# rizar/attention-lvcsr

Measured on AMD Instinct MI355X. Metric: encoder+attention+decoder training frames/sec (whole node), higher is better.
Workload: dtype f32; 1 GPU; wsj_base: B=16 utterances x T=800 frames x F=40 fbank per GPU, L=100 labels; 256x256x256x256 BiGRU subsample [1, 1, 2, 2], content_and_conv attention, 256-unit GRU decoder; global_batch=16, per_gpu_batch=16, ragged=False, parallelism=dp1, optimizer=clip100+adadelta+maxnorm1, hip_graph=True, priming_steps=2, encoder_kernels=persistent clusters, full=False

## Files before the change

attention-lvcsr_amd/csrc/encoder_persist.hip:

```cpp
#include "common.h"
#include "graph_cache.h"
#include "lvsr_hip.h"
#include "persist.h"

typedef lvsr_bigru_fwd_args EncFwd;
typedef lvsr_bigru_bwd_args EncBwd0;

template <int NG, bool PRIV, int NTH = 256>
struct Sweep {
    static constexpr int NT = PRIV ? 64 : NTH;
    static constexpr int N = (NG + NT - 1) / NT;
    u64 w[N];
    __device__ __forceinline__ void issue(const u64* g, unsigned epoch) {
        const int tid = PRIV ? (int)(threadIdx.x & 63) : (int)threadIdx.x;
#pragma unroll
        for (int i = 0; i < N; ++i) {
            const int idx = tid + NT * i;
            if (NG % NT == 0 || idx < NG) w[i] = __hip_atomic_load(g + idx, __ATOMIC_RELAXED, __HIP_MEMORY_SCOPE_AGENT);
            else w[i] = (u64)epoch << 32;
        }
    }
    __device__ __forceinline__ bool complete(unsigned epoch) const {
        bool ok = true;
#pragma unroll
// ... 353 lines not shown
        const size_t jo = (size_t)b0 * 2 * H + dir * H + min(jj, H - 1);
        const long long row = (long long)B * 2 * H, sgn = dir == 0 ? -1 : 1;
        const float* p0 = (hi ? a.c : a.u) + jo;
        const float* p1 = (hi ? a.y : a.r) + jo;
        const float h0v = a.h0[dir][min(jj, H - 1)];
        const float* p2 = hi ? a.dy + (size_t)b0 * 2 * H + dir * H + min(jj, H - 1) : (a.mask ? a.mask + b0 : a.h0[dir]);
        const long long row2 = hi ? row : (a.mask ? (long long)B : 0);
        auto issue = [&](int ns, float (&dst)[3]) {
            const int nsc = min(ns, T - 1), t = dir == 0 ? T - 1 - nsc : nsc, tp = t + (int)sgn, tpc = min(max(tp, 0), T - 1);
            const bool edge = tp != tpc, dy_here = !edge && (tp % a.sub) == 0;
            const float v0 = p0[(long long)t * row];
            const float v1 = p1[(long long)(hi ? tpc : t) * row];
            const float v2 = p2[(long long)(hi ? tpc / a.sub : t) * row2];
            dst[0] = live ? v0 : 0.f;
            dst[1] = live ? ((hi && edge) ? h0v : v1) : 0.f;
            dst[2] = hi ? ((live && dy_here) ? v2 : 0.f) : ((live && a.mask) ? v2 : 1.f);
        };
        float pa[3], pb[3];
        auto hand = [&](int n, const float (&v)[3]) {
            if (n + 1 < T) { opnd9[lane] = v[0]; opnd9[64 + lane] = v[1]; opnd9[128 + lane] = v[2]; }
            __syncthreads();
            __syncthreads();
        };
        issue(1, pa);
        for (int n = 0; n < T; n += 2) {
            issue(n + 2, pb);
            hand(n, pa);
            if (n + 1 < T) {
                issue(n + 3, pa);
                hand(n + 1, pb);
            }
        }
        return;
    }
    const int tid = threadIdx.x, q = tid % KSPLIT, j = p * UNITS + tid / KSPLIT, k0 = q * KS;
    const bool junit = j < H;
    f32x2 wa[KS / 2], wbu[KS / 2], wbr[KS / 2];
    {
        const float* Whg = a.WhgT_p[dir];
        const float* Whh = a.WhhT_p[dir];
        const size_t jc = (size_t)min(j, H - 1);
#pragma unroll
        for (int x = 0; x < KS / 2; ++x) {
            float v[6];
#pragma unroll
            for (int e = 0; e < 2; ++e) {
                const int k = k0 + 2 * x + e;
                const float keep = (junit && k < H) ? 1.f : 0.f;
                const size_t kc = (size_t)min(k, H - 1);
                v[e] = Whh[jc * H + kc] * keep;
                v[2 + e] = Whg[jc * 2 * H + kc] * keep;
                v[4 + e] = Whg[jc * 2 * H + H + kc] * keep;
            }
            wa[x] = (f32x2){v[0], v[1]}; wbu[x] = (f32x2){v[2], v[3]}; wbr[x] = (f32x2){v[4], v[5]};
        }
    }
    u64* gc = planes + (size_t)cl * 4 * NG;
    u64* gu = gc + NG;
    u64* gr = gc + 2 * NG;
    const int t_first = dir == 0 ? T - 1 : 0;
    float dh[NR], n_u[NR], n_c[NR], n_r[NR], n_hp[NR], n_m[NR], n_dy[NR];
    bool rvalid[NR];
    auto prefetch = [&](int t, int i) {
        const int b = b0 + q + i * KSPLIT;
        const int tp = dir == 0 ? t - 1 : t + 1;
        const size_t o = ((size_t)t * B + b) * 2 * H + dir * H + j;
        n_u[i] = a.u[o]; n_c[i] = a.c[o]; n_r[i] = a.r[o];
        n_hp[i] = (tp < 0 || tp >= T) ? a.h0[dir][j] : a.y[((size_t)tp * B + b) * 2 * H + dir * H + j];
        n_m[i] = a.mask ? a.mask[(size_t)t * B + b] : 1.f;
        n_dy[i] = pb_dy_at(a, tp, b, dir, j);
    };
#pragma unroll
    for (int i = 0; i < NR; ++i) {
        const int r = q + i * KSPLIT;
        rvalid[i] = junit && r < RB && b0 + r < B;
        dh[i] = rvalid[i] ? pb_dy_at(a, t_first, b0 + r, dir, j) : 0.f;
        n_u[i] = n_c[i] = n_r[i] = n_hp[i] = n_dy[i] = 0.f; n_m[i] = 1.f;
        if (rvalid[i]) prefetch(t_first, i);
    }
    for (int n = 0; n < T; ++n) {
        const int t = dir == 0 ? T - 1 - n : n;
        float uu[NR], cc[NR], rr[NR], hp[NR], part[NR];
#pragma unroll
        for (int i = 0; i < NR; ++i) {
            const int r = q + i * KSPLIT;
            uu[i] = n_u[i]; cc[i] = n_c[i]; rr[i] = n_r[i]; hp[i] = n_hp[i];
            if (r < RB) {
                const float dhn = n_m[i] * dh[i];
                const float dpc = rvalid[i] ? dhn * uu[i] * (1.f - cc[i] * cc[i]) : 0.f;
                const float dpu = rvalid[i] ? dhn * (cc[i] - hp[i]) * uu[i] * (1.f - uu[i]) : 0.f;
                if (P == 1) {
                    lds_publish<KS, LDH, KSPLIT>(vbuf[0], r, j, dpc);
                    lds_publish<KS, LDH, KSPLIT>(vbuf[1], r, j, dpu);
                } else {
                    granule_store(gc + (size_t)r * HP + j, (unsigned)(n + 1), dpc, plain);
                    granule_store(gu + (size_t)r * HP + j, (unsigned)(n + 1), dpu, plain);
                }
                part[i] = dhn * (1.f - uu[i]) + (1.f - n_m[i]) * dh[i] + n_dy[i];
                if (rvalid[i] && save) {
                    float* dx = a.dxg + ((size_t)t * B + b0 + r) * 6 * H + dir * 3 * H;
                    dx[j] = dpc; dx[H + j] = dpu;
                }
            }
        }
        if (!LD9 && n + 1 < T && !(flags & PF_NOPREFETCH)) {
#pragma unroll
            for (int i = 0; i < NR; ++i)
                if (rvalid[i]) prefetch(dir == 0 ? t - 1 : t + 1, i);
        }
        if (P > 1 && !gather_plane<NG, HP, KS, LDH, KSPLIT, PRIV, 2, NBUF * RB * KSPLIT * LDH, NTH>(gc, (unsigned)(n + 1), vbuf[0], abort_word)) return;
        gather_fence<PRIV>();
        if (LD9 && n + 1 < T && rvalid[0]) {
            const int ju = tid / KSPLIT;
            n_u[0] = opnd9[ju]; n_c[0] = opnd9[32 + ju]; n_r[0] = opnd9[64 + ju]; n_hp[0] = opnd9[96 + ju];
            n_m[0] = opnd9[128 + ju]; n_dy[0] = opnd9[160 + ju];
        }
        float s[RB], vu[RB];
        slice_dot<KS, RB, LDH, KSPLIT>(wa, vbuf[0], q, s);
#pragma unroll
        for (int i = 0; i < NR; ++i) {
            const int r = q + i * KSPLIT;
            if (r < RB) {
                const float drh = pick_row<RB, KSPLIT>(s, q, i);
                const float dpr = rvalid[i] ? drh * hp[i] * rr[i] * (1.f - rr[i]) : 0.f;
                if (P == 1) lds_publish<KS, LDH, KSPLIT>(vbuf[2], r, j, dpr);
                else granule_store(gr + (size_t)r * HP + j, (unsigned)(n + 1), dpr, plain);
                part[i] += drh * rr[i];
                if (rvalid[i] && save) a.dxg[((size_t)t * B + b0 + r) * 6 * H + dir * 3 * H + 2 * H + j] = dpr;
            }
        }
        slice_dot<KS, RB, LDH, KSPLIT>(wbu, vbuf[1], q, vu);
        if (P > 1 && !gather_plane<NG, HP, KS, LDH, KSPLIT, PRIV, 1, 0, NTH>(gr, (unsigned)(n + 1), vbuf[2], abort_word)) return;
        gather_fence<PRIV>();
        slice_dot<KS, RB, LDH, KSPLIT>(wbr, vbuf[2], q, s);
#pragma unroll
        for (int i = 0; i < NR; ++i) {
            const int r = q + i * KSPLIT;
            if (r < RB) dh[i] = rvalid[i] ? part[i] + pick_row<RB, KSPLIT>(vu, q, i) + pick_row<RB, KSPLIT>(s, q, i) : 0.f;
        }
    }
#pragma unroll
    for (int i = 0; i < NR; ++i)
        if (rvalid[i]) dh_out[((size_t)dir * Bp + b0 + q + i * KSPLIT) * H + j] = dh[i];
}

__global__ __launch_bounds__(256) void enc_pbwd_h0_kernel(const float* dh, int Bp, int B, int H, float* out_f, float* out_b) {
    const int dir = blockIdx.z;
    const int j = blockIdx.x * 256 + threadIdx.x;
    if (j >= H) return;
    float s = 0.f;
    for (int b = 0; b < B; ++b) s += dh[((size_t)dir * Bp + b) * H + j];
    (dir == 0 ? out_f : out_b)[j] = s;
}

template <int KS, int U>
__device__ __forceinline__ void ub_dot(const f32x2 (&w)[U][KS / 2], const float* buf, int q, float (&out)[U]) {
    const float4* hv = (const float4*)(buf + q * (KS + 4));
    f32x2 acc[U];
#pragma unroll
    for (int u = 0; u < U; ++u) acc[u] = (f32x2){0.f, 0.f};
#pragma unroll
    for (int x = 0; x < KS / 4; ++x) {
        const float4 h4 = hv[x];
        const f32x2 lo = {h4.x, h4.y}, hi = {h4.z, h4.w};
#pragma unroll
        for (int u = 0; u < U; ++u) {
            acc[u] = w[u][2 * x] * lo + acc[u];
            acc[u] = w[u][2 * x + 1] * hi + acc[u];
        }
    }
#pragma unroll
    for (int u = 0; u < U; ++u) out[u] = acc[u].x + acc[u].y;
}
template <int U>
__device__ __forceinline__ float ub_fold(const float (&v)[U], int q) {
    float r;
    if (U == 4) {
        const bool up = (q & 32) != 0;
        const float a0 = (up ? v[2] : v[0]) + __shfl_xor(up ? v[0] : v[2], 32, 64);
        const float a1 = (up ? v[3] : v[1]) + __shfl_xor(up ? v[1] : v[3], 32, 64);
        const bool up2 = (q & 16) != 0;
        r = (up2 ? a1 : a0) + __shfl_xor(up2 ? a0 : a1, 16, 64);
    } else if (U == 2) {
        const bool up = (q & 16) != 0;
        r = (up ? v[1] : v[0]) + __shfl_xor(up ? v[0] : v[1], 16, 64);
    } else {
        r = v[0];
    }
    return group_sum<16>(r);
}

template <int KS, int U, int NTH>
__global__ __launch_bounds__(NTH) void enc_pfwd_ub_kernel(EncFwd a, u64* planes, u64* hello, int* abort_word, int flags) {
    constexpr int G = 16 * U, HP = KS * G, UNITS = NTH / G * U, P = HP / UNITS, LDH = KS + 4, NG = HP;
    __shared__ __attribute__((aligned(16))) float hbuf[2][G * LDH];
    const int H = a.H, B = a.B, T = a.T;
    int cl, p;
    if (!cluster_of_block(P, 2 * B, flags, cl, p)) return;
    const bool save = !(flags & PF_NOSAVE);
    const bool plain = cluster_shares_xcd(hello + (size_t)cl * P, P, p, abort_word) && !(flags & PF_SC1);
    const int dir = cl / B, b = cl % B;
    const int tid = threadIdx.x, q = tid % G, jb = p * UNITS + (tid / G) * U, k0 = q * KS;
    f32x2 wr[U][KS / 2], wu[U][KS / 2], wc[U][KS / 2];
    {
        const float* Whg = a.Whg_p[dir];
        const float* Whh = a.Whh_p[dir];
#pragma unroll
        for (int u = 0; u < U; ++u) {
            const int j = jb + u;
            const size_t jc = (size_t)min(j, H - 1);
#pragma unroll
            for (int x = 0; x < KS / 2; ++x) {
                float v[6];
#pragma unroll
                for (int e = 0; e < 2; ++e) {
                    const int k = k0 + 2 * x + e;
                    const float keep = (j < H && k < H) ? 1.f : 0.f;
                    const size_t kc = (size_t)min(k, H - 1);
                    v[e] = Whg[kc * 2 * H + jc] * keep;
                    v[2 + e] = Whg[kc * 2 * H + H + jc] * keep;
                    v[4 + e] = Whh[kc * H + jc] * keep;
                }
                wu[u][x] = (f32x2){v[0], v[1]}; wr[u][x] = (f32x2){v[2], v[3]}; wc[u][x] = (f32x2){v[4], v[5]};
            }
        }
    }
    u64* gh = planes + (size_t)cl * 2 * NG;
    u64* grh = gh + NG;
    const int j = jb + (q >> 4);
    const bool own = (q & 15) == 0 && j < H;
    float hown = own ? a.h0[dir][j] : 0.f, n_xin = 0.f, n_gu = 0.f, n_gr = 0.f, n_m = 1.f;
    auto fetch = [&](int t) {
        const size_t row = (size_t)t * B + b;
        const float* xr = a.xg + row * 6 * H + dir * 3 * H;
        n_xin = xr[j]; n_gu = xr[H + j]; n_gr = xr[2 * H + j];
        if (a.mask) n_m = a.mask[row];
    };
    if (own) fetch(dir == 0 ? 0 : T - 1);
    for (int k = tid; k < HP; k += NTH) hbuf[0][(k / KS) * LDH + (k % KS)] = k < H ? a.h0[dir][k] : 0.f;
    for (int n = 0; n < T; ++n) {
        const int t = dir == 0 ? n : T - 1 - n;
        const float xin = n_xin, gu = n_gu, gr = n_gr, m = n_m;
        if (n > 0 && !gather_plane<NG, HP, KS, LDH, G, false, 1, 0, NTH>(gh, (unsigned)n, hbuf[0], abort_word, flags)) return;
        __syncthreads();
        float s[U];
        ub_dot<KS, U>(wr, hbuf[0], q, s);
        const float rr = sigmoid_fast(ub_fold<U>(s, q) + gr);
        const float rh = own ? rr * hown : 0.f;
        if ((q & 15) == 0) granule_store(grh + min(j, HP - 1), (unsigned)(n + 1), rh, plain);
        if (own && save) {
            const size_t o = ((size_t)t * B + b) * 2 * H + dir * H + j;
            a.r[o] = rr; a.rh[o] = rh;
        }
        ub_dot<KS, U>(wu, hbuf[0], q, s);
        const float uu = sigmoid_fast(ub_fold<U>(s, q) + gu);
        if (own && save) a.u[((size_t)t * B + b) * 2 * H + dir * H + j] = uu;
        if (!gather_plane<NG, HP, KS, LDH, G, false, 1, 0, NTH>(grh, (unsigned)(n + 1), hbuf[1], abort_word, flags)) return;
        __syncthreads();
        ub_dot<KS, U>(wc, hbuf[1], q, s);
        const float cand = tanh_fast(ub_fold<U>(s, q) + xin);
        float hn = cand * uu + hown * (1.f - uu);
        hn = m * hn + (1.f - m) * hown;
        if (!own) hn = 0.f;
        if ((q & 15) == 0 && n + 1 < T) granule_store(gh + min(j, HP - 1), (unsigned)(n + 1), hn, plain);
        if (own) {
            const size_t o = ((size_t)t * B + b) * 2 * H + dir * H + j;
            if (save) a.c[o] = cand;
            a.y[o] = hn;
            if (a.ysub && (t % a.sub) == 0) a.ysub[((size_t)(t / a.sub) * B + b) * 2 * H + dir * H + j] = hn;
        }
        hown = hn;
        if (own && n + 1 < T && !(flags & PF_NOPREFETCH)) fetch(dir == 0 ? n + 1 : T - 2 - n);
    }
}

static int wide_cluster_capacity() {
    static int occ_cached = -1;
    if (occ_cached < 0) {
        int occ = 1 << 20, n = 0;
        const bool ok = hipOccupancyMaxActiveBlocksPerMultiprocessor(&n, enc_pfwd_kernel<16, 16, 1, false, 512>, 512, 0) == hipSuccess && (occ = min(occ, n)) >= 0 &&
                        hipOccupancyMaxActiveBlocksPerMultiprocessor(&n, enc_pfwd_kernel<16, 16, 2, false, 512>, 512, 0) == hipSuccess && (occ = min(occ, n)) >= 0 &&
                        hipOccupancyMaxActiveBlocksPerMultiprocessor(&n, enc_pbwd_kernel<16, 16, 1, false, 512>, 512, 0) == hipSuccess && (occ = min(occ, n)) >= 0 &&
                        hipOccupancyMaxActiveBlocksPerMultiprocessor(&n, enc_pbwd_kernel<16, 16, 2, false, 512>, 512, 0) == hipSuccess && (occ = min(occ, n)) >= 0;
        if (!ok) { (void)hipGetLastError(); occ = 0; }
        occ_cached = min(occ, 2);
    }
    return occ_cached * lvsr_max_cluster_wgs();
}

static int persist_flags() { return lvsr_knob(LVSR_KNOB_PERSIST_FLAGS); }

extern "C" int lvsr_bigru_persist_rows(int B, int H) {
    PersistGeom g;
    if (B <= 0 || H <= 0 || !persist_geom(B, H, g)) return 0;
    return g.RB;
}

extern "C" long long lvsr_bigru_persist_ws_bytes(int B, int H) {
    PersistGeom g;
    if (B <= 0 || H <= 0) return 0;
    if (!persist_geom(B, H, g)) return 0;
    const long long hello = (long long)cluster_grid(2 * B, 16, 0) * 8;
    return 256 + (long long)2 * (B + 16) * 4 * g.HP * 8 + (hello > 8 * 1024 ? hello : 8 * 1024);
}

template <int KS, int KSPLIT>
static void launch_fwd(hipStream_t s, const EncFwd& a, const PersistGeom& g, u64* planes, u64* hello, int* ab, int flags) {
    if (g.NTH == 512 && g.RB == 1 && g.HP == 512 && !(flags & PF_NOUB)) {
        hipLaunchKernelGGL((enc_pfwd_ub_kernel<8, 4, 512>), dim3(g.grid), dim3(512), 0, s, a, planes, hello, ab, flags);
        return;
    }
    if (g.NTH == 512) {
        if (g.P == 8 && g.KS == 16 && g.RB == 1 && !(flags & (PF_NOLD9F | PF_NOSTAGE)) && g.grid <= lvsr_max_cluster_wgs())
            hipLaunchKernelGGL((enc_pfwd_kernel<16, 16, 1, false, 512, true>), dim3(g.grid), dim3(576), 0, s, a, planes, hello, ab, flags);
        else if (g.P == 8 && g.KS == 16 && g.RB == 1) hipLaunchKernelGGL((enc_pfwd_kernel<16, 16, 1, false, 512>), dim3(g.grid), dim3(512), 0, s, a, planes, hello, ab, flags);
        else if (g.P == 8 && g.KS == 16) hipLaunchKernelGGL((enc_pfwd_kernel<16, 16, 2, false, 512>), dim3(g.grid), dim3(512), 0, s, a, planes, hello, ab, flags);
        else if (g.RB == 1) hipLaunchKernelGGL((enc_pfwd_kernel<KS / 2, KSPLIT * 2, 1, false, 512>), dim3(g.grid), dim3(512), 0, s, a, planes, hello, ab, flags);
        else hipLaunchKernelGGL((enc_pfwd_kernel<KS / 2, KSPLIT * 2, 2, false, 512>), dim3(g.grid), dim3(512), 0, s, a, planes, hello, ab, flags);
        return;
    }
    switch (g.RB) {
        case 1:
            if (!(flags & PF_PRIVATE)) hipLaunchKernelGGL((enc_pfwd_kernel<KS, KSPLIT, 1, false>), dim3(g.grid), dim3(256), 0, s, a, planes, hello, ab, flags);
            else hipLaunchKernelGGL((enc_pfwd_kernel<KS, KSPLIT, 1, true>), dim3(g.grid), dim3(256), 0, s, a, planes, hello, ab, flags);
            break;
        case 2: hipLaunchKernelGGL((enc_pfwd_kernel<KS, KSPLIT, 2, false>), dim3(g.grid), dim3(256), 0, s, a, planes, hello, ab, flags); break;
        case 4: hipLaunchKernelGGL((enc_pfwd_kernel<KS, KSPLIT, 4, false>), dim3(g.grid), dim3(256), 0, s, a, planes, hello, ab, flags); break;
        default: hipLaunchKernelGGL((enc_pfwd_kernel<KS, KSPLIT, 8, false>), dim3(g.grid), dim3(256), 0, s, a, planes, hello, ab, flags); break;
    }
}
template <int KS, int KSPLIT>
static void launch_bwd(hipStream_t s, const EncBwd0& a, const PersistGeom& g, u64* planes, u64* hello, int* ab, float* dh, int Bp, int flags) {
    if (g.NTH == 512) {
        if (g.P == 8 && g.KS == 16 && g.RB == 1 && !(flags & PF_NOLD9) && g.grid <= lvsr_max_cluster_wgs())
            hipLaunchKernelGGL((enc_pbwd_kernel<16, 16, 1, false, 512, true>), dim3(g.grid), dim3(576), 0, s, a, planes, hello, ab, dh, Bp, flags);
        else if (g.P == 8 && g.KS == 16 && g.RB == 1) hipLaunchKernelGGL((enc_pbwd_kernel<16, 16, 1, false, 512>), dim3(g.grid), dim3(512), 0, s, a, planes, hello, ab, dh, Bp, flags);
        else if (g.P == 8 && g.KS == 16) hipLaunchKernelGGL((enc_pbwd_kernel<16, 16, 2, false, 512>), dim3(g.grid), dim3(512), 0, s, a, planes, hello, ab, dh, Bp, flags);
        else if (g.RB == 1) {
            if constexpr (KSPLIT == 8) {
                if (!(flags & PF_NOLD9) && g.grid <= lvsr_max_cluster_wgs()) {
                    hipLaunchKernelGGL((enc_pbwd_kernel<KS / 2, KSPLIT * 2, 1, false, 512, true>), dim3(g.grid), dim3(576), 0, s, a, planes, hello, ab, dh, Bp, flags);
                    return;
                }
            }
            hipLaunchKernelGGL((enc_pbwd_kernel<KS / 2, KSPLIT * 2, 1, false, 512>), dim3(g.grid), dim3(512), 0, s, a, planes, hello, ab, dh, Bp, flags);
        }
        else hipLaunchKernelGGL((enc_pbwd_kernel<KS / 2, KSPLIT * 2, 2, false, 512>), dim3(g.grid), dim3(512), 0, s, a, planes, hello, ab, dh, Bp, flags);
        return;
    }
    switch (g.RB) {
        case 1:
            if (!(flags & PF_PRIVATE)) hipLaunchKernelGGL((enc_pbwd_kernel<KS, KSPLIT, 1, false>), dim3(g.grid), dim3(256), 0, s, a, planes, hello, ab, dh, Bp, flags);
            else hipLaunchKernelGGL((enc_pbwd_kernel<KS, KSPLIT, 1, true>), dim3(g.grid), dim3(256), 0, s, a, planes, hello, ab, dh, Bp, flags);
            break;
        case 2: hipLaunchKernelGGL((enc_pbwd_kernel<KS, KSPLIT, 2, false>), dim3(g.grid), dim3(256), 0, s, a, planes, hello, ab, dh, Bp, flags); break;
        case 4: hipLaunchKernelGGL((enc_pbwd_kernel<KS, KSPLIT, 4, false>), dim3(g.grid), dim3(256), 0, s, a, planes, hello, ab, dh, Bp, flags); break;
        default: hipLaunchKernelGGL((enc_pbwd_kernel<KS, KSPLIT, 8, false>), dim3(g.grid), dim3(256), 0, s, a, planes, hello, ab, dh, Bp, flags); break;
    }
}

int lvsr_bigru_fwd_persistent(hipStream_t s, const EncFwd& a0, int use_graph) {
    EncFwd a = a0;
    PersistGeom g;
    LVSR_REQUIRE(persist_geom(a.B, a.H, g) && a.sync_ws, "lvsr_bigru_fwd: persistent mode not available for B=%d H=%d", a.B, a.H);
    int* ab = (int*)a.sync_ws;
    u64* planes = (u64*)((char*)a.sync_ws + 256);
    u64* hello = planes + (size_t)2 * g.rt * 2 * g.plane;
    const size_t bytes = (size_t)2 * g.rt * 2 * g.plane * 8 + (size_t)g.grid * 8;
    if (a.sub == 1) a.ysub = nullptr;
    const int flags = persist_flags();
    auto enqueue = [&]() {
        (void)hipMemsetAsync(planes, 0, bytes, s);
        switch (g.KSPLIT / (g.NTH / 256)) {
            case 2: launch_fwd<64, 2>(s, a, g, planes, hello, ab, flags); break;
            case 4: launch_fwd<64, 4>(s, a, g, planes, hello, ab, flags); break;
            default: launch_fwd<64, 8>(s, a, g, planes, hello, ab, flags); break;
        }
    };
    GraphKey key("bigru_pfwd");
    key.add(&a, sizeof(a));
    key.add(&g.RB, sizeof(g.RB));
    key.add(&g.NTH, sizeof(g.NTH));
    key.add(&flags, sizeof(flags));
    return lvsr_run_graph(s, use_graph, key, enqueue, "lvsr_bigru_fwd(persistent)");
}

int lvsr_bigru_bwd_persistent(hipStream_t s, const EncBwd0& a, int use_graph) {
    PersistGeom g;
    LVSR_REQUIRE(persist_geom(a.B, a.H, g) && a.sync_ws, "lvsr_bigru_bwd: persistent mode not available for B=%d H=%d", a.B, a.H);
    int* ab = (int*)a.sync_ws;
    u64* planes = (u64*)((char*)a.sync_ws + 256);
    u64* hello = planes + (size_t)2 * g.rt * 4 * g.plane;
    const size_t bytes = (size_t)2 * g.rt * 4 * g.plane * 8 + (size_t)g.grid * 8;
    const int Bp = ((a.B + 15) / 16) * 16;
    float* dh = a.dh_ws;
    const int flags = persist_flags();
    auto enqueue = [&]() {
        (void)hipMemsetAsync(planes, 0, bytes, s);
        switch (g.KSPLIT / (g.NTH / 256)) {
            case 2: launch_bwd<64, 2>(s, a, g, planes, hello, ab, dh, Bp, flags); break;
            case 4: launch_bwd<64, 4>(s, a, g, planes, hello, ab, dh, Bp, flags); break;
            default: launch_bwd<64, 8>(s, a, g, planes, hello, ab, dh, Bp, flags); break;
        }
        hipLaunchKernelGGL(enc_pbwd_h0_kernel, dim3((a.H + 255) / 256, 1, 2), dim3(256), 0, s, dh, Bp, a.B, a.H, a.dh0[0], a.dh0[1]);
    };
    GraphKey key("bigru_pbwd");
    key.add(&a, sizeof(a));
    key.add(&g.RB, sizeof(g.RB));
    key.add(&g.NTH, sizeof(g.NTH));
    key.add(&flags, sizeof(flags));
    return lvsr_run_graph(s, use_graph, key, enqueue, "lvsr_bigru_bwd(persistent)");
}
```

attention-lvcsr_amd/csrc/gemm.hip:

```cpp
#include "common.h"
#include "lvsr_hip.h"
#include "graph_cache.h"
#include <algorithm>
#include <vector>

#define BM 64
#define BN 64
#define BK 16
#define LDS_LD (BM + 4)

struct GemmArgs {
    const float* A; const float* B; float* C; const float* bias;
    int M, N, K, lda, ldb, ldc, transA, transB;
    float alpha, beta;
    int ksplit;
    int kchunk;
    float* part;
    int batch;
    long long sA, sB, sC;
};

__global__ __launch_bounds__(256) void lvsr_sgemm_kernel(GemmArgs g) {
    __shared__ float As[BK][LDS_LD];
    __shared__ float Bs[BK][LDS_LD];
// ... 424 lines not shown
        if ((int)blockIdx.x >= pk.d[x].fold0) p = x;
    const GroupDesc& d = pk.d[p];
    const size_t total = (size_t)d.M * d.N;
    const float* part = pk.part + d.part_off;
    const size_t base = (size_t)((int)blockIdx.x - d.fold0) * FOLD_ELEMS;
    const bool vec = (d.N & 3) == 0 && (d.ldc & 3) == 0 && (((size_t)d.C) & 15) == 0 && (((size_t)part) & 15) == 0;
    size_t idx[4];
    float s[4] = {0.f, 0.f, 0.f, 0.f};
#pragma unroll
    for (int e = 0; e < 4; ++e) idx[e] = vec ? base + 4 * threadIdx.x + e : base + threadIdx.x + 256 * e;
    int z = 0;
    if (vec) {
        if (idx[0] >= total) return;
        const float* q = part + idx[0];
        for (; z + 4 <= d.ksplit; z += 4) {
            float4 v[4];
#pragma unroll
            for (int c = 0; c < 4; ++c) v[c] = *(const float4*)(q + (size_t)(z + c) * total);
#pragma unroll
            for (int c = 0; c < 4; ++c) { s[0] += v[c].x; s[1] += v[c].y; s[2] += v[c].z; s[3] += v[c].w; }
        }
        for (; z < d.ksplit; ++z) {
            const float4 v = *(const float4*)(q + (size_t)z * total);
            s[0] += v.x; s[1] += v.y; s[2] += v.z; s[3] += v.w;
        }
        float* c = d.C + (idx[0] / d.N) * d.ldc + idx[0] % d.N;
        if (d.beta != 0.f) {
            const float4 o = *(const float4*)c;
            s[0] += d.beta * o.x; s[1] += d.beta * o.y; s[2] += d.beta * o.z; s[3] += d.beta * o.w;
        }
        *(float4*)c = make_float4(s[0], s[1], s[2], s[3]);
        return;
    }
    for (; z + 4 <= d.ksplit; z += 4) {
        float v[4][4];
#pragma unroll
        for (int c = 0; c < 4; ++c)
#pragma unroll
            for (int e = 0; e < 4; ++e) v[c][e] = idx[e] < total ? part[(size_t)(z + c) * total + idx[e]] : 0.f;
#pragma unroll
        for (int c = 0; c < 4; ++c)
#pragma unroll
            for (int e = 0; e < 4; ++e) s[e] += v[c][e];
    }
    for (; z < d.ksplit; ++z)
#pragma unroll
        for (int e = 0; e < 4; ++e) s[e] += idx[e] < total ? part[(size_t)z * total + idx[e]] : 0.f;
#pragma unroll
    for (int e = 0; e < 4; ++e) {
        if (idx[e] >= total) continue;
        float* c = d.C + (idx[e] / d.N) * d.ldc + idx[e] % d.N;
        float r = s[e];
        if (d.beta != 0.f) r += d.beta * *c;
        *c = r;
    }
}

__global__ __launch_bounds__(256) void lvsr_sgemm_splitk_reduce(GemmArgs g) {
    const size_t total = (size_t)g.M * g.N;
    for (size_t idx = (size_t)blockIdx.x * blockDim.x + threadIdx.x; idx < total; idx += (size_t)gridDim.x * blockDim.x) {
        const int m = (int)(idx / g.N), n = (int)(idx % g.N);
        float s = 0.f;
        for (int z = 0; z < g.ksplit; ++z) s += g.part[(size_t)z * total + idx];
        float v = g.alpha * s;
        if (g.beta != 0.f) v += g.beta * g.C[(size_t)m * g.ldc + n];
        if (g.bias) v += g.bias[n];
        g.C[(size_t)m * g.ldc + n] = v;
    }
}

__global__ __launch_bounds__(256) void lvsr_colsum_kernel(const float* X, int M, int N, int ldx, float* out, float beta,
                                                          int rows_per, float* part) {
    __shared__ float red[4][64];
    const int n = blockIdx.x * 64 + (threadIdx.x & 63);
    const int g = threadIdx.x >> 6;
    const int m0 = blockIdx.y * rows_per, m1 = min(M, m0 + rows_per);
    float s0 = 0.f, s1 = 0.f, s2 = 0.f, s3 = 0.f;
    if (n < N) {
        int m = m0 + g;
        for (; m + 12 < m1; m += 16) {
            s0 += X[(size_t)m * ldx + n];
            s1 += X[(size_t)(m + 4) * ldx + n];
            s2 += X[(size_t)(m + 8) * ldx + n];
            s3 += X[(size_t)(m + 12) * ldx + n];
        }
        for (; m < m1; m += 4) s0 += X[(size_t)m * ldx + n];
    }
    red[g][threadIdx.x & 63] = (s0 + s1) + (s2 + s3);
    __syncthreads();
    if (g == 0 && n < N) {
        const int c = threadIdx.x & 63;
        const float v = ((red[0][c] + red[1][c]) + red[2][c]) + red[3][c];
        if (part) part[(size_t)blockIdx.y * N + n] = v;
        else out[n] = (beta != 0.f ? beta * out[n] : 0.f) + v;
    }
}

#define COLSUM_MANY_MAX 32
struct ColsumMember { const float* X; float* out; float* part; int M, N, ldx, S, rows_per, nx, block0, fin0; float beta; };
struct ColsumPack { ColsumMember m[COLSUM_MANY_MAX]; int n; };
__global__ __launch_bounds__(256) void lvsr_colsum_many_kernel(ColsumPack pk) {
    __shared__ float red[4][64];
    int p = 0;
    for (int i = 1; i < pk.n; ++i)
        if ((int)blockIdx.x >= pk.m[i].block0) p = i;
    const ColsumMember& c = pk.m[p];
    const int local = blockIdx.x - c.block0, bx = local % c.nx, by = local / c.nx;
    const int n = bx * 64 + (threadIdx.x & 63);
    const int g = threadIdx.x >> 6;
    const int m0 = by * c.rows_per, m1 = min(c.M, m0 + c.rows_per);
    const float* X = c.X;
    const int ldx = c.ldx;
    float s0 = 0.f, s1 = 0.f, s2 = 0.f, s3 = 0.f;
    if (n < c.N) {
        int m = m0 + g;
        for (; m + 12 < m1; m += 16) {
            s0 += X[(size_t)m * ldx + n];
            s1 += X[(size_t)(m + 4) * ldx + n];
            s2 += X[(size_t)(m + 8) * ldx + n];
            s3 += X[(size_t)(m + 12) * ldx + n];
        }
        for (; m < m1; m += 4) s0 += X[(size_t)m * ldx + n];
    }
    red[g][threadIdx.x & 63] = (s0 + s1) + (s2 + s3);
    __syncthreads();
    if (g == 0 && n < c.N) {
        const int col = threadIdx.x & 63;
        const float v = ((red[0][col] + red[1][col]) + red[2][col]) + red[3][col];
        if (c.S > 1) c.part[(size_t)by * c.N + n] = v;
        else c.out[n] = (c.beta != 0.f ? c.beta * c.out[n] : 0.f) + v;
    }
}
__global__ __launch_bounds__(256) void lvsr_colsum_many_finish(ColsumPack pk) {
    int p = 0;
    for (int i = 1; i < pk.n; ++i)
        if ((int)blockIdx.x >= pk.m[i].fin0) p = i;
    const ColsumMember& c = pk.m[p];
    if (c.S <= 1) return;
    const int n = ((int)blockIdx.x - c.fin0) * 256 + threadIdx.x;
    if (n >= c.N) return;
    float v = 0.f;
    for (int s = 0; s < c.S; ++s) v += c.part[(size_t)s * c.N + n];
    c.out[n] = (c.beta != 0.f ? c.beta * c.out[n] : 0.f) + v;
}

__global__ __launch_bounds__(256) void lvsr_colsum_finish(const float* part, int S, int N, float* out, float beta) {
    const int n = blockIdx.x * 256 + threadIdx.x;
    if (n >= N) return;
    float v = 0.f;
    for (int s = 0; s < S; ++s) v += part[(size_t)s * N + n];
    out[n] = (beta != 0.f ? beta * out[n] : 0.f) + v;
}

#define COPY_MANY_MAX 32
struct CopyPack { lvsr_copy_desc d[COPY_MANY_MAX]; int n; };
__global__ __launch_bounds__(256) void lvsr_copy2d_many_kernel(CopyPack pk) {
    const lvsr_copy_desc& d = pk.d[blockIdx.y];
    const bool vec = ((d.cols | d.lds | d.ldd) & 3) == 0 && ((((size_t)d.src) | ((size_t)d.dst)) & 15) == 0;
    if (d.rows == 1) {
        for (int c = blockIdx.x * 256 + threadIdx.x; c < d.cols; c += gridDim.x * 256)
            d.dst[c] = d.beta != 0.f ? d.src[c] + d.beta * d.dst[c] : d.src[c];
        return;
    }
    for (int r = blockIdx.x; r < d.rows; r += gridDim.x) {
        const float* s = d.src + (size_t)r * d.lds;
        float* o = d.dst + (size_t)r * d.ldd;
        if (d.beta != 0.f) {
            for (int c = threadIdx.x; c < d.cols; c += 256) o[c] = s[c] + d.beta * o[c];
        } else if (vec) {
            for (int c = threadIdx.x * 4; c < d.cols; c += 1024) *(float4*)(o + c) = *(const float4*)(s + c);
        } else {
            for (int c = threadIdx.x; c < d.cols; c += 256) o[c] = s[c];
        }
    }
}

__global__ __launch_bounds__(256) void lvsr_transpose_kernel(const float* in, int rows, int cols, float* out) {
    __shared__ float tile[32][33];
    const int tx = threadIdx.x & 31, ty = threadIdx.x >> 5;
    const int r0 = blockIdx.y * 32, c0 = blockIdx.x * 32;
    for (int j = ty; j < 32; j += 8) {
        const int r = r0 + j, c = c0 + tx;
        tile[j][tx] = (r < rows && c < cols) ? in[(size_t)r * cols + c] : 0.f;
    }
    __syncthreads();
    for (int j = ty; j < 32; j += 8) {
        const int c = c0 + j, r = r0 + tx;
        if (r < rows && c < cols) out[(size_t)c * rows + r] = tile[tx][j];
    }
}

__global__ __launch_bounds__(256) void lvsr_pack_b_kernel(const float* W, int ldw, int K, int N, int trans, float* P,
                                                          int Kw, int NQ, long long total) {
    for (long long idx = (long long)blockIdx.x * 256 + threadIdx.x; idx < total; idx += (long long)gridDim.x * 256) {
        const int r = (int)(idx & 3), lane = (int)((idx >> 2) & 63);
        const long long g = idx >> 8;
        const int q = (int)(g % NQ), wave = (int)((g / NQ) & 3), tile = (int)(g / NQ / 4);
        const int k = wave * Kw + (lane >> 4) * (Kw >> 2) + 4 * q + r, col = tile * 16 + (lane & 15);
        float v = 0.f;
        if (k < K && col < N) v = trans ? W[(size_t)col * ldw + k] : W[(size_t)k * ldw + col];
        P[idx] = v;
    }
}

static bool operands_aligned(const float* A, int lda, const float* B, int ldb) {
    return (lda & 3) == 0 && (ldb & 3) == 0 && (((size_t)A) & 15) == 0 && (((size_t)B) & 15) == 0;
}

static int colsum_split(int M, int N, bool have_ws, long long ws_bytes) {
    if (!have_ws || M < 512) return 1;
    const int nx = (N + 63) / 64;
    int S = (M + 255) / 256;
    const int want = (1024 + nx - 1) / nx;
    if (S > want) S = want;
    while (S > 1 && (long long)S * N * 4 > ws_bytes) --S;
    return S;
}

extern "C" {

static int sgemm_launch(void* stream, int transA, int transB, int M, int N, int K, float alpha, const float* A, int lda,
                        const float* B, int ldb, float beta, float* C, int ldc, const float* bias, float* ws,
                        long long ws_bytes, int batch, long long sA, long long sB, long long sC) {
    LVSR_REQUIRE(M >= 0 && N >= 0 && K >= 0 && batch >= 1, "lvsr_sgemm: negative dimension");
    if (M == 0 || N == 0) return LVSR_OK;
    GemmArgs g;
    g.batch = batch; g.sA = sA; g.sB = sB; g.sC = sC;
    if (batch > 1) ws = nullptr;
    g.A = A; g.B = B; g.C = C; g.bias = bias;
    g.M = M; g.N = N; g.K = K; g.lda = lda; g.ldb = ldb; g.ldc = ldc; g.transA = transA; g.transB = transB;
    g.alpha = alpha; g.beta = beta; g.ksplit = 1; g.kchunk = 0; g.part = nullptr;
    const bool big = (M >= 96 && N >= 96) || (min(M, N) >= 32 && max(M, N) >= 256 && K >= 2048);
    int tm = big ? GM : BM, tn = big ? GN : BN;
    const int tk = big ? GK : BK;
    int tiles = ((M + tm - 1) / tm) * ((N + tn - 1) / tn);
    const int mid_max = lvsr_knob(LVSR_KNOB_GEMM_MID_TILES) > 0 ? lvsr_knob(LVSR_KNOB_GEMM_MID_TILES) : 2048;
    const bool mid = big && batch == 1 && (tiles < 256 || (tiles < mid_max && K <= 2048));
    if (mid) { tm = 64; tn = 64; tiles = ((M + 63) / 64) * ((N + 63) / 64); }
    g.kchunk = ((K + tk - 1) / tk) * tk;
    if (g.kchunk == 0) g.kchunk = tk;
    const int slots = mid ? 1024 : 512;
    if (ws && 2 * tiles <= slots && K >= 1024) {
        int want = (slots + tiles - 1) / tiles;
        int maxk = K / 256;
        if (want > maxk) want = maxk;
        long long need = (long long)want * M * N * 4;
        while (want > 1 && need > ws_bytes) { --want; need = (long long)want * M * N * 4; }
        if (want > 1) {
            int chunk = (K + want - 1) / want;
            chunk = ((chunk + tk - 1) / tk) * tk;
            g.ksplit = (K + chunk - 1) / chunk;
            g.kchunk = chunk;
            g.part = ws;
        }
    }
    dim3 grid((N + tn - 1) / tn, (M + tm - 1) / tm, batch > 1 ? batch : g.ksplit);
    hipStream_t st = (hipStream_t)stream;
    if (!big) {
        hipLaunchKernelGGL(lvsr_sgemm_kernel, grid, dim3(256), 0, st, g);
    } else {
        const bool fast = operands_aligned(A, lda, B, ldb) && (batch == 1 || ((sA & 3) == 0 && (sB & 3) == 0));
        lvsr_dispatch<0, 1, 2, 3, 4, 5, 6, 7>((transA ? 4 : 0) | (transB ? 2 : 0) | (fast ? 1 : 0), [&](auto v) {
            constexpr bool TA = (decltype(v)::value & 4) != 0, TB = (decltype(v)::value & 2) != 0, FAST = (decltype(v)::value & 1) != 0;
            if (mid) hipLaunchKernelGGL((lvsr_sgemm64_kernel<TA, TB, FAST>), grid, dim3(256), 0, st, g);
            else hipLaunchKernelGGL((lvsr_sgemm128_kernel<TA, TB, FAST>), grid, dim3(256), 0, st, g);
        });
    }
    if (g.ksplit > 1) {
        int nb = (int)(((size_t)M * N + 255) / 256);
        if (nb > 2048) nb = 2048;
        hipLaunchKernelGGL(lvsr_sgemm_splitk_reduce, dim3(nb), dim3(256), 0, st, g);
    }
    return lvsr_check_launch("lvsr_sgemm");
}

int lvsr_sgemm(void* stream, int transA, int transB, int M, int N, int K, float alpha, const float* A, int lda,
               const float* B, int ldb, float beta, float* C, int ldc, const float* bias, float* ws,
               long long ws_bytes) {
    return sgemm_launch(stream, transA, transB, M, N, K, alpha, A, lda, B, ldb, beta, C, ldc, bias, ws, ws_bytes, 1, 0, 0, 0);
}

int lvsr_sgemm_batched(void* stream, int transA, int transB, int M, int N, int K, float alpha, const float* A, int lda,
                       long long strideA, const float* B, int ldb, long long strideB, float beta, float* C, int ldc,
                       long long strideC, int batch) {
    LVSR_REQUIRE(batch >= 0, "lvsr_sgemm_batched: negative batch");
    if (batch == 0) return LVSR_OK;
    return sgemm_launch(stream, transA, transB, M, N, K, alpha, A, lda, B, ldb, beta, C, ldc, nullptr, nullptr, 0, batch,
                        strideA, strideB, strideC);
}

static bool group_aligned(const lvsr_gemm_desc& s) { return operands_aligned(s.A, s.lda, s.B, s.ldb); }
static void group_cut(const lvsr_gemm_desc* s, int n, long long ws_bytes, int* ksplit, int* kchunk) {
    int target = 1024;
    if (ws_bytes > 0) {
        for (;; target += 512) {
            long long need = 0;
            bool splits = false;
            for (int i = 0; i < n; ++i) {
                const int want = (s[i].K + target - 1) / target;
                if (want > 1) { need += ((long long)want * s[i].M * s[i].N + 3) / 4 * 4; splits = true; }
            }
            if (!splits || need * 4 <= ws_bytes) break;
        }
    }
    for (int i = 0; i < n; ++i) {
        const int want = ws_bytes > 0 ? (s[i].K + target - 1) / target : 1;
        int chunk = (s[i].K + want - 1) / want;
        chunk = ((chunk + GK - 1) / GK) * GK;
        kchunk[i] = chunk;
        ksplit[i] = (s[i].K + chunk - 1) / chunk;
    }
}
static void group_order(const lvsr_gemm_desc* s, const int* kchunk, int n, int* order) {
    for (int i = 0; i < n; ++i) order[i] = i;
    auto cost = [&](int i) { return (kchunk[i] < s[i].K ? kchunk[i] : s[i].K) * (group_aligned(s[i]) ? 1 : 2); };
    std::stable_sort(order, order + n, [&](int a, int b) { return cost(a) > cost(b); });
}

int lvsr_sgemm_tn_grouped_plan(const lvsr_gemm_desc* descs, int n, long long ws_bytes, int* ksplit, int* kchunk) {
    LVSR_REQUIRE(n >= 0 && (n == 0 || (descs && ksplit && kchunk)), "lvsr_sgemm_tn_grouped_plan: bad arguments");
    for (int i = 0; i < n; ++i)
        LVSR_REQUIRE(descs[i].M > 0 && descs[i].N > 0 && descs[i].K > 0, "lvsr_sgemm_tn_grouped_plan: bad descriptor %d", i);
    group_cut(descs, n, ws_bytes, ksplit, kchunk);
    return LVSR_OK;
}

int lvsr_sgemm_tn_grouped(void* stream, const lvsr_gemm_desc* descs, int n, float* ws, long long ws_bytes) {
    LVSR_REQUIRE(n >= 0 && (n == 0 || descs), "lvsr_sgemm_tn_grouped: bad arguments");
    hipStream_t st = (hipStream_t)stream;
    for (int i = 0; i < n; ++i)
        LVSR_REQUIRE(descs[i].A && descs[i].B && descs[i].C && descs[i].M > 0 && descs[i].N > 0 && descs[i].K > 0,
                     "lvsr_sgemm_tn_grouped: bad descriptor %d", i);
    if (!ws || ws_bytes < 0) ws_bytes = 0;
    std::vector<int> ksplit(n), kchunk(n);
    group_cut(descs, n, ws_bytes, ksplit.data(), kchunk.data());
    long long off = 0;
    for (int i0 = 0; i0 < n; i0 += GROUP_MAX) {
        const int cnt = n - i0 < GROUP_MAX ? n - i0 : GROUP_MAX;
        int order[GROUP_MAX];
        group_order(descs + i0, kchunk.data() + i0, cnt, order);
        GroupPack pk;
        pk.n = cnt; pk.part = ws;
        int units = 0, nfold = 0;
        for (int o = 0; o < cnt; ++o) {
            const int i = i0 + order[o];
            const lvsr_gemm_desc& s = descs[i];
            GroupDesc& d = pk.d[o];
            d.A = s.A; d.B = s.B; d.C = s.C; d.M = s.M; d.N = s.N; d.K = s.K; d.lda = s.lda; d.ldb = s.ldb; d.ldc = s.ldc; d.beta = s.beta;
            d.gx = (s.N + GN - 1) / GN; d.gy = (s.M + GM - 1) / GM;
            d.ksplit = ksplit[i]; d.kchunk = kchunk[i];
            d.fast = group_aligned(s) ? 1 : 0;
            d.unit0 = units;
            units += d.gx * d.gy * d.ksplit;
            d.fold0 = nfold;
            d.part_off = off;
            if (d.ksplit > 1) {
                const long long mn = (long long)s.M * s.N;
                off += (d.ksplit * mn + 3) / 4 * 4;
                nfold += (int)((mn + FOLD_ELEMS - 1) / FOLD_ELEMS);
            }
        }
        LVSR_REQUIRE(off * 4 <= ws_bytes, "lvsr_sgemm_tn_grouped: partials exceed the workspace");
        pk.total = units;
        hipLaunchKernelGGL(lvsr_sgemm128_grouped_tn_kernel, dim3(units), dim3(256), 0, st, pk);
        if (nfold) hipLaunchKernelGGL(lvsr_sgemm_grouped_reduce, dim3(nfold), dim3(256), 0, st, pk);
    }
    return lvsr_check_launch("lvsr_sgemm_tn_grouped");
}

int lvsr_colsum(void* stream, const float* X, int M, int N, int ldx, float* out, float beta, float* ws,
                long long ws_bytes) {
    if (N <= 0) return LVSR_OK;
    const int nx = (N + 63) / 64;
    const int S = colsum_split(M, N, ws != nullptr, ws_bytes);
    const int rows_per = (M + S - 1) / S;
    hipLaunchKernelGGL(lvsr_colsum_kernel, dim3(nx, S), dim3(256), 0, (hipStream_t)stream, X, M, N, ldx, out, beta, rows_per,
                       S > 1 ? ws : nullptr);
    if (S > 1)
        hipLaunchKernelGGL(lvsr_colsum_finish, dim3((N + 255) / 256), dim3(256), 0, (hipStream_t)stream, ws, S, N, out, beta);
    return lvsr_check_launch("lvsr_colsum");
}

int lvsr_colsum_many(void* stream, const lvsr_colsum_desc* descs, int n, float* ws, long long ws_bytes, long long split_ws_bytes) {
    LVSR_REQUIRE(n >= 0 && (n == 0 || descs), "lvsr_colsum_many: bad arguments");
    for (int i = 0; i < n; ++i)
        LVSR_REQUIRE(descs[i].X && descs[i].out && descs[i].M >= 0 && descs[i].N > 0, "lvsr_colsum_many: bad descriptor %d", i);
    for (int i0 = 0; i0 < n; i0 += COLSUM_MANY_MAX) {
        ColsumPack pk;
        pk.n = n - i0 < COLSUM_MANY_MAX ? n - i0 : COLSUM_MANY_MAX;
        int blocks = 0, fin = 0;
        long long off = 0;
        bool any_split = false;
        for (int i = 0; i < pk.n; ++i) {
            const lvsr_colsum_desc& d = descs[i0 + i];
            ColsumMember& c = pk.m[i];
            c.X = d.X; c.out = d.out; c.M = d.M; c.N = d.N; c.ldx = d.ldx; c.beta = d.beta;
            c.nx = (d.N + 63) / 64;
            const int S = colsum_split(d.M, d.N, ws != nullptr, split_ws_bytes);
            c.S = S;
            c.rows_per = (d.M + S - 1) / S;
            c.part = ws ? ws + off : nullptr;
            if (S > 1) { off += (long long)S * d.N; any_split = true; }
            c.block0 = blocks; blocks += c.nx * S;
            c.fin0 = fin; fin += (d.N + 255) / 256;
        }
        LVSR_REQUIRE(off * 4 <= ws_bytes, "lvsr_colsum_many: workspace too small for the partial sums (%lld bytes needed)", off * 4);
        if (blocks > 0) hipLaunchKernelGGL(lvsr_colsum_many_kernel, dim3(blocks), dim3(256), 0, (hipStream_t)stream, pk);
        if (any_split) hipLaunchKernelGGL(lvsr_colsum_many_finish, dim3(fin), dim3(256), 0, (hipStream_t)stream, pk);
        LVSR_REQUIRE(i0 + COLSUM_MANY_MAX >= n || !any_split, "lvsr_colsum_many: more than %d members with row splits", COLSUM_MANY_MAX);
    }
    return lvsr_check_launch("lvsr_colsum_many");
}

int lvsr_copy2d_many(void* stream, const lvsr_copy_desc* descs, int n) {
    LVSR_REQUIRE(n >= 0 && (n == 0 || descs), "lvsr_copy2d_many: bad arguments");
    for (int i = 0; i < n; ++i)
        LVSR_REQUIRE(descs[i].rows >= 0 && descs[i].cols >= 0 && descs[i].src && descs[i].dst, "lvsr_copy2d_many: bad descriptor %d", i);
    for (int i0 = 0; i0 < n; i0 += COPY_MANY_MAX) {
        CopyPack pk;
        pk.n = n - i0 < COPY_MANY_MAX ? n - i0 : COPY_MANY_MAX;
        for (int i = 0; i < pk.n; ++i) pk.d[i] = descs[i0 + i];
        hipLaunchKernelGGL(lvsr_copy2d_many_kernel, dim3(128, pk.n), dim3(256), 0, (hipStream_t)stream, pk);
    }
    return lvsr_check_launch("lvsr_copy2d_many");
}

int lvsr_transpose(void* stream, const float* in, int rows, int cols, float* out) {
    if (rows <= 0 || cols <= 0) return LVSR_OK;
    hipLaunchKernelGGL(lvsr_transpose_kernel, dim3((cols + 31) / 32, (rows + 31) / 32), dim3(256), 0, (hipStream_t)stream,
                       in, rows, cols, out);
    return lvsr_check_launch("lvsr_transpose");
}

long long lvsr_pack_size(int K, int N) {
    if (K <= 0 || N <= 0) return 0;
    return (long long)((N + 15) / 16) * 16 * 4 * lvsr_pack_kw(K);
}

int lvsr_pack_b(void* stream, const float* W, int ldw, int K, int N, int trans, float* packed) {
    LVSR_REQUIRE(K > 0 && N > 0 && W && packed, "lvsr_pack_b: bad arguments K=%d N=%d", K, N);
    const int Kw = lvsr_pack_kw(K), NQ = Kw / 16;
    const long long total = lvsr_pack_size(K, N);
    int nb = (int)((total + 255) / 256);
    if (nb > 4096) nb = 4096;
    hipLaunchKernelGGL(lvsr_pack_b_kernel, dim3(nb), dim3(256), 0, (hipStream_t)stream, W, ldw, K, N, trans, packed, Kw,
                       NQ, total);
    return lvsr_check_launch("lvsr_pack_b");
}

int lvsr_pack_b_many(void* stream, const lvsr_pack_desc* descs, int n, int use_graph) {
    LVSR_REQUIRE(n >= 0 && (n == 0 || descs), "lvsr_pack_b_many: bad arguments");
    if (n == 0) return LVSR_OK;
    for (int i = 0; i < n; ++i)
        LVSR_REQUIRE(descs[i].K > 0 && descs[i].N > 0 && descs[i].W && descs[i].packed, "lvsr_pack_b_many: bad descriptor %d", i);
    hipStream_t s = (hipStream_t)stream;
    auto enqueue = [&]() {
        for (int i = 0; i < n; ++i) {
            const lvsr_pack_desc& d = descs[i];
            const int Kw = lvsr_pack_kw(d.K), NQ = Kw / 16;
            const long long total = lvsr_pack_size(d.K, d.N);
            int nb = (int)((total + 255) / 256);
            if (nb > 4096) nb = 4096;
            hipLaunchKernelGGL(lvsr_pack_b_kernel, dim3(nb), dim3(256), 0, s, d.W, d.ldw, d.K, d.N, d.trans, d.packed, Kw, NQ, total);
        }
    };
    GraphKey key("pack_many");
    key.add(descs, sizeof(lvsr_pack_desc) * (size_t)n);
    return lvsr_run_graph(s, use_graph, key, enqueue, "lvsr_pack_b_many");
}

}
```

attention-lvcsr_amd/csrc/optimizer.hip:

```cpp
#include "common.h"
#include "lvsr_hip.h"
#include <string.h>

typedef lvsr_opt_args Opt;

__device__ __forceinline__ float blk_sum256(float v, float* red) {
    v = wave_sum(v);
    __syncthreads();
    if ((threadIdx.x & 63) == 0) red[threadIdx.x >> 6] = v;
    __syncthreads();
    return (red[0] + red[1]) + (red[2] + red[3]);
}

__global__ __launch_bounds__(256) void opt_sqnorm_kernel(Opt o) {
    __shared__ float red[4];
    float s = 0.f;
    for (long long i = (long long)blockIdx.x * 256 + threadIdx.x; i < o.n; i += (long long)gridDim.x * 256) {
        const float g = o.grad[i] * o.grad_scale;
        s += g * g;
    }
    s = blk_sum256(s, red);
    if (threadIdx.x == 0) o.scratch[2 + blockIdx.x] = s;
}

__global__ __launch_bounds__(256) void opt_norm_kernel(Opt o, int nparts) {
    __shared__ float red[4];
    float s = 0.f;
    for (int i = threadIdx.x; i < nparts; i += 256) s += o.scratch[2 + i];
    s = blk_sum256(s, red);
    if (threadIdx.x == 0) {
        const float norm = sqrtf(s);
        const bool skip = o.guard && o.guard[0] != 0.f;
        o.scratch[3] = skip ? 1.f : 0.f;
        double* cs = skip ? nullptr : o.clip_state;
        const float thr = cs ? (float)cs[0] : o.clip_threshold;
        o.scratch[0] = norm;
        o.scratch[1] = (thr > 0.f && !(norm < thr)) ? thr / norm : 1.f;
        float burn = 0.f;
        if (cs) {
            if (cs[4] > 0.0) { burn = 1.f; cs[4] -= 1.0; }
            if (o.adaptive_clipping && norm > 0.f && norm - norm == 0.f) {
                const double d = (double)o.adaptive_decay, init = (double)o.clip_threshold, bp = (double)o.adaptive_burnin;
                const double ln = log((double)norm);
                cs[3] += 1.0;
                cs[1] = d * cs[1] + (1.0 - d) * ln;
                cs[2] = d * cs[2] + (1.0 - d) * ln * ln;
                const double var = cs[2] - cs[1] * cs[1];
                double t = exp(cs[1] + sqrt(var > 0.0 ? var : 0.0));
                const double conf = (cs[3] < bp ? cs[3] : bp) / bp;
                t = conf * t + (1.0 - conf) * init;
                cs[0] = t < 5.0 * init ? t : 5.0 * init;
            }
        }
        o.scratch[2] = burn;
    }
}

__global__ __launch_bounds__(256) void opt_rules_kernel(Opt o) {
    if (o.scratch[3] != 0.f) return;
    const float mult = o.scratch[1];
    if (blockIdx.x == 0)
        for (int sgi = threadIdx.x; sgi < o.nseg; sgi += 256) o.segflag[sgi] = 0;
    for (long long i = (long long)blockIdx.x * 256 + threadIdx.x; i < o.n; i += (long long)gridDim.x * 256) {
        float s = o.grad[i] * o.grad_scale * mult;
        if (o.use_momentum) {
            s = o.learning_rate * s;
            s = o.momentum * o.velocity[i] + s;
            o.velocity[i] = s;
        }
        if (o.use_adadelta) {
            const float ms = o.decay_rate * o.ms_step[i] + (1.f - o.decay_rate) * s * s;
            const float dx = sqrtf(o.ms_dx[i] + o.epsilon) / sqrtf(ms + o.epsilon) * s;
            o.ms_step[i] = ms;
            o.ms_dx[i] = o.decay_rate * o.ms_dx[i] + (1.f - o.decay_rate) * dx * dx;
            s = dx;
        }
        o.step[i] = s;
    }
}

#define MAXNORM_GROUPS 16
__global__ __launch_bounds__(64 * MAXNORM_GROUPS) void opt_maxnorm_kernel(Opt o) {
    __shared__ float red[MAXNORM_GROUPS][64];
    const long long* seg = o.segments + 4 * (long long)blockIdx.y;
    const long long off = seg[0], rows = seg[1], cols = seg[2], flags = seg[3];
    if (!(flags & 1) || o.scratch[3] != 0.f) return;
    const long long j = (long long)blockIdx.x * 64 + (threadIdx.x & 63);
    if ((long long)blockIdx.x * 64 >= cols) return;
    const int g = threadIdx.x >> 6;
    float s = 0.f;
    if (j < cols)
        for (long long r = g; r < rows; r += MAXNORM_GROUPS) {
            const float v = o.param[off + r * cols + j] - o.step[off + r * cols + j];
            s += v * v;
        }
    red[g][threadIdx.x & 63] = s;
    __syncthreads();
    const int c = threadIdx.x & 63;
    float tot = 0.f;
#pragma unroll
    for (int gg = 0; gg < MAXNORM_GROUPS; ++gg) tot += red[gg][c];
    const float norm = sqrtf(tot);
    if (j < cols && norm > o.max_norm) {
        const float k = o.max_norm / norm;
        for (long long r = g; r < rows; r += MAXNORM_GROUPS) {
            const long long x = off + r * cols + j;
            o.step[x] = o.param[x] - k * (o.param[x] - o.step[x]);
        }
    }
}

__global__ __launch_bounds__(256) void opt_finite_kernel(Opt o) {
    __shared__ float red[4];
    const long long* seg = o.segments + 4 * (long long)blockIdx.y;
    const long long off = seg[0], n = seg[1] * seg[2];
    if (o.scratch[3] != 0.f) return;
    float s = 0.f;
    for (long long i = (long long)blockIdx.x * 256 + threadIdx.x; i < n; i += (long long)gridDim.x * 256) s += o.step[off + i];
    s = blk_sum256(s, red);
    if (threadIdx.x == 0 && (s != s || s - s != 0.f)) o.segflag[blockIdx.y] = 1;
}

__global__ __launch_bounds__(256) void opt_apply_kernel(Opt o) {
    const long long* seg = o.segments + 4 * (long long)blockIdx.y;
    const long long off = seg[0], n = seg[1] * seg[2];
    const int bad = o.remove_not_finite ? o.segflag[blockIdx.y] : 0;
    if (o.scratch[3] != 0.f) return;
    if (o.clip_state && o.scratch[2] != 0.f) return;
    for (long long i = (long long)blockIdx.x * 256 + threadIdx.x; i < n; i += (long long)gridDim.x * 256) {
        const float p = o.param[off + i];
        const float s = bad ? (1.f - o.nonfinite_scaler) * p : o.step[off + i];
        o.param[off + i] = p - s;
    }
}

struct GuardPack { const int* w[64]; int n; };
__global__ void guard_collect_kernel(GuardPack pk, float* out) {
    if (threadIdx.x == 0) {
        int bad = 0;
        for (int i = 0; i < pk.n; ++i)
            if (pk.w[i] && __hip_atomic_load(pk.w[i], __ATOMIC_RELAXED, __HIP_MEMORY_SCOPE_AGENT) != 0) ++bad;
        out[0] = (float)bad;
    }
}

extern "C" int lvsr_guard_collect(void* stream, const int* const* words, int n, float* out) {
    LVSR_REQUIRE(n >= 0 && n <= 64 && out && (n == 0 || words), "lvsr_guard_collect: at most 64 words");
    GuardPack pk;
    pk.n = n;
    for (int i = 0; i < 64; ++i) pk.w[i] = i < n ? words[i] : nullptr;
    hipLaunchKernelGGL(guard_collect_kernel, dim3(1), dim3(64), 0, (hipStream_t)stream, pk, out);
    return lvsr_check_launch("lvsr_guard_collect");
}

extern "C" int lvsr_opt_step(void* stream, const lvsr_opt_args* args) {
    LVSR_REQUIRE(args != nullptr, "lvsr_opt_step: null args");
    Opt o;
    memcpy(&o, args, sizeof(o));
    LVSR_REQUIRE(o.n > 0 && o.nseg > 0 && o.param && o.grad && o.step && o.segments && o.scratch && o.segflag,
                 "lvsr_opt_step: missing buffers");
    LVSR_REQUIRE(!o.use_momentum || o.velocity, "lvsr_opt_step: momentum needs a velocity buffer");
    LVSR_REQUIRE(!o.use_adadelta || (o.ms_step && o.ms_dx), "lvsr_opt_step: AdaDelta needs its two accumulators");
    LVSR_REQUIRE(!o.adaptive_clipping || (o.clip_state && o.clip_threshold > 0.f && o.adaptive_burnin > 0),
                 "lvsr_opt_step: adaptive clipping needs clip_state, an initial threshold and a burn-in period");
    hipStream_t s = (hipStream_t)stream;
    const int nparts = 256;
    int nb = (int)((o.n + 255) / 256);
    if (nb > 2048) nb = 2048;
    hipLaunchKernelGGL(opt_sqnorm_kernel, dim3(nparts), dim3(256), 0, s, o);
    hipLaunchKernelGGL(opt_norm_kernel, dim3(1), dim3(256), 0, s, o, nparts);
    hipLaunchKernelGGL(opt_rules_kernel, dim3(nb), dim3(256), 0, s, o);
    if (o.max_norm > 0.f)
        hipLaunchKernelGGL(opt_maxnorm_kernel, dim3((o.max_cols + 63) / 64, o.nseg), dim3(64 * MAXNORM_GROUPS), 0, s, o);
    if (o.remove_not_finite)
        hipLaunchKernelGGL(opt_finite_kernel, dim3(16, o.nseg), dim3(256), 0, s, o);
    hipLaunchKernelGGL(opt_apply_kernel, dim3(16, o.nseg), dim3(256), 0, s, o);
    return lvsr_check_launch("lvsr_opt_step");
}
```

attention-lvcsr_amd/csrc/readout.hip:

```cpp
#include "common.h"
#include "lvsr_hip.h"

__global__ __launch_bounds__(256) void gather_rows_kernel(const float* table, int ldt, const long long* idx, int n,
                                                          int nrows, int width, const float* bias, float* out, int ldo) {
    const int r = blockIdx.y;
    const int c = blockIdx.x * 256 + threadIdx.x;
    if (r >= n || c >= width) return;
    long long v = idx[r];
    float x = 0.f;
    if (v >= 0 && v < nrows) x = table[(size_t)v * ldt + c];
    if (bias) x += bias[c];
    out[(size_t)r * ldo + c] = x;
}

#define SCATTER_CHUNK 2048
__global__ __launch_bounds__(256) void scatter_add_rows_kernel(const float* src, int lds, const long long* idx, int n,
                                                               int width, float* dst, int ldd, float beta) {
    __shared__ int hit[SCATTER_CHUNK];
    __shared__ int nhit;
    const int v = blockIdx.y;
    const int c = blockIdx.x * 256 + threadIdx.x;
    float s = 0.f;
    for (int r0 = 0; r0 < n; r0 += SCATTER_CHUNK) {
        const int m = min(SCATTER_CHUNK, n - r0);
        __syncthreads();
        if (threadIdx.x == 0) nhit = 0;
        const int per = (m + 255) / 256, x0 = min(m, (int)threadIdx.x * per), x1 = min(m, x0 + per);
        int mine = 0;
        for (int x = x0; x < x1; ++x) mine += idx[r0 + x] == v;
        __shared__ int cnt[256];
        cnt[threadIdx.x] = mine;
        __syncthreads();
        if (threadIdx.x == 0) {
            int run = 0;
            for (int t = 0; t < 256; ++t) { const int k = cnt[t]; cnt[t] = run; run += k; }
            nhit = run;
        }
        __syncthreads();
        int o = cnt[threadIdx.x];
        for (int x = x0; x < x1; ++x)
            if (idx[r0 + x] == v) hit[o++] = r0 + x;
        __syncthreads();
        if (c < width)
            for (int h = 0; h < nhit; ++h) s += src[(size_t)hit[h] * lds + c];
    }
    if (c < width) {
        float* d = dst + (size_t)v * ldd + c;
        *d = (beta != 0.f ? beta * *d : 0.f) + s;
    }
}

__global__ __launch_bounds__(256) void act_fwd_kernel(int kind, const float* x, int ldx, int n, int P, float* y, int ldy) {
    const int Pout = kind == 1 ? P / 2 : P;
    const size_t total = (size_t)n * Pout;
    for (size_t idx = (size_t)blockIdx.x * 256 + threadIdx.x; idx < total; idx += (size_t)gridDim.x * 256) {
        const int r = (int)(idx / Pout), j = (int)(idx % Pout);
        const float* xr = x + (size_t)r * ldx;
        float v;
        if (kind == 1) v = fmaxf(xr[2 * j], xr[2 * j + 1]);
        else if (kind == 2) v = xr[j] > 0.f ? xr[j] : 0.f;
        else if (kind == 3) v = tanhf(xr[j]);
        else v = xr[j];
        y[(size_t)r * ldy + j] = v;
    }
}

__global__ __launch_bounds__(256) void act_bwd_kernel(int kind, const float* x, int ldx, const float* dy, int lddy, int n,
                                                      int P, float* dx, int lddx) {
    const int Pout = kind == 1 ? P / 2 : P;
    const size_t total = (size_t)n * Pout;
    for (size_t idx = (size_t)blockIdx.x * 256 + threadIdx.x; idx < total; idx += (size_t)gridDim.x * 256) {
        const int r = (int)(idx / Pout), j = (int)(idx % Pout);
        const float* xr = x + (size_t)r * ldx;
        float* dr = dx + (size_t)r * lddx;
        const float g = dy[(size_t)r * lddy + j];
        if (kind == 1) {
            const float a = xr[2 * j], b = xr[2 * j + 1], m = fmaxf(a, b);
            dr[2 * j] = a == m ? g : 0.f;
            dr[2 * j + 1] = b == m ? g : 0.f;
        } else if (kind == 2) {
            dr[j] = xr[j] > 0.f ? g : 0.f;
        } else if (kind == 3) {
            const float t = tanhf(xr[j]);
            dr[j] = g * (1.f - t * t);
        } else {
            dr[j] = g;
        }
    }
}

__global__ __launch_bounds__(256) void softmax_nll_kernel(const float* logits, int ld, const long long* labels,
                                                          const float* mask, int n, int V, float* cost, float* dlogits,
                                                          int ldd, float scale, float* neglogp, int ldn) {
    const int r = blockIdx.x * 4 + (threadIdx.x >> 6), lane = threadIdx.x & 63;
    if (r >= n) return;
    const float* x = logits + (size_t)r * ld;
    float mx = -3.0e38f;
    for (int v = lane; v < V; v += 64) mx = fmaxf(mx, x[v]);
    mx = wave_max(mx);
    float s = 0.f;
    for (int v = lane; v < V; v += 64) s += expf(x[v] - mx);
    s = wave_sum(s);
    const float lse = logf(s);
    const float m = mask ? mask[r] : 1.f;
    const long long y = labels ? labels[r] : -1;
    if (cost && lane == 0) cost[r] = (y >= 0 && y < V) ? -((x[y] - mx) - lse) * m : 0.f;
    for (int v = lane; v < V; v += 64) {
        const float lp = (x[v] - mx) - lse;
        if (neglogp) neglogp[(size_t)r * ldn + v] = -lp;
        if (dlogits) dlogits[(size_t)r * ldd + v] = (expf(lp) - (v == y ? 1.f : 0.f)) * m * scale;
    }
}

__device__ __forceinline__ float row_lse(const float* x, int V, float scale, int lane) {
    float mx = -3.0e38f;
    for (int v = lane; v < V; v += 64) mx = fmaxf(mx, scale * x[v]);
    mx = wave_max(mx);
    float s = 0.f;
    for (int v = lane; v < V; v += 64) s += expf(scale * x[v] - mx);
    s = wave_sum(s);
    return mx + logf(s);
}
__global__ __launch_bounds__(256) void shallow_fusion_kernel(const float* am, int ld, const float* lm_add, int n, int V,
                                                             float am_beta, float lm_weight, int norm_am, int norm_lm,
                                                             int norm_tot, float out_scale, float* out) {
    const int r = blockIdx.x * 4 + (threadIdx.x >> 6), lane = threadIdx.x & 63;
    if (r >= n) return;
    const float* a = am + (size_t)r * ld;
    const float* l = lm_add + (size_t)r * V;
    float* o = out + (size_t)r * V;
    const float lse_a = norm_am ? row_lse(a, V, am_beta, lane) : 0.f;
    const float lse_l = norm_lm ? row_lse(l, V, -1.f, lane) : 0.f;
    float lse_t = 0.f;
    if (norm_tot) {
        float mx = -3.0e38f;
        for (int v = lane; v < V; v += 64) mx = fmaxf(mx, (am_beta * a[v] - lse_a) + lm_weight * (-l[v] - lse_l));
        mx = wave_max(mx);
        float s = 0.f;
        for (int v = lane; v < V; v += 64) s += expf(((am_beta * a[v] - lse_a) + lm_weight * (-l[v] - lse_l)) - mx);
        s = wave_sum(s);
        lse_t = mx + logf(s);
    }
    for (int v = lane; v < V; v += 64) o[v] = out_scale * (((am_beta * a[v] - lse_a) + lm_weight * (-l[v] - lse_l)) - lse_t);
}

__global__ __launch_bounds__(256) void select_cost_kernel(const float* x, int ld, const long long* labels, const float* mask, int n, int V,
                                                          float scale, float* cost) {
    const int r = blockIdx.x * 256 + threadIdx.x;
    if (r >= n) return;
    const long long y = labels[r];
    const float v = (y >= 0 && y < V) ? x[(size_t)r * ld + y] : 0.f;
    cost[r] = scale * v * (mask ? mask[r] : 1.f);
}

__device__ __forceinline__ float row_lse(const float* x, int V, float scale, int lane);
#define RS_MAX_IN 4096
#define RS_MAX_P 2048
#define RS_MAX_V 2048

__device__ void wg_matvec(const float* x, int K, const float* W, int N, const float* bias, float* out, float* part ) {
    const bool vec = (N % 4 == 0) && ((((size_t)W) & 15) == 0);
    const int cols = vec ? N / 4 : N;
    int CP = 1;
    while (CP < cols && CP < 256) CP <<= 1;
    const int G = 256 / CP, jl = threadIdx.x % CP, g = threadIdx.x / CP;
    const int per = (K + G - 1) / G, k0 = g * per, k1 = min(K, k0 + per);
    for (int j0 = 0; j0 < cols; j0 += CP) {
        const int j = j0 + jl;
        float a0 = 0.f, a1 = 0.f, a2 = 0.f, a3 = 0.f;
        if (j < cols) {
            if (vec) {
                const float4* w = (const float4*)W + j;
                const int N4 = N / 4;
                int k = k0;
                for (; k + 7 < k1; k += 8) {
                    float4 wv[8];
#pragma unroll
                    for (int u = 0; u < 8; ++u) wv[u] = w[(size_t)(k + u) * N4];
#pragma unroll
                    for (int u = 0; u < 8; ++u) {
                        const float xv = x[k + u];
                        a0 += xv * wv[u].x; a1 += xv * wv[u].y; a2 += xv * wv[u].z; a3 += xv * wv[u].w;
                    }
                }
                for (; k < k1; ++k) {
                    const float4 wv = w[(size_t)k * N4];
                    const float xv = x[k];
                    a0 += xv * wv.x; a1 += xv * wv.y; a2 += xv * wv.z; a3 += xv * wv.w;
                }
            } else {
                const float* w = W + j;
                int k = k0;
                for (; k + 3 < k1; k += 4) {
                    a0 += x[k] * w[(size_t)k * N];
                    a1 += x[k + 1] * w[(size_t)(k + 1) * N];
                    a2 += x[k + 2] * w[(size_t)(k + 2) * N];
                    a3 += x[k + 3] * w[(size_t)(k + 3) * N];
                }
                for (; k < k1; ++k) a0 += x[k] * w[(size_t)k * N];
            }
        }
        __syncthreads();
// ... 86 lines not shown
    if (a.emitter == 1) {
        if (w0) {
            float bv = -3.0e38f;
            int bi = V;
            for (int v = lane; v < V; v += 64) {
                const float x = logits[v];
                if (a.neglogp) a.neglogp[(size_t)r * V + v] = -x;
                if (bi == V || x > bv) { bv = x; bi = v; }
            }
#pragma unroll
            for (int o = 32; o > 0; o >>= 1) {
                const float ov = __shfl_xor(bv, o, 64);
                const int oi = __shfl_xor(bi, o, 64);
                if (oi < V && (bi == V || ov > bv || (ov == bv && oi < bi))) { bv = ov; bi = oi; }
            }
            if (a.outputs && lane == 0) {
                a.outputs[r] = bi;
                if (a.costs) a.costs[r] = bv;
            }
        }
        return;
    }
    if (w0) {
        float lse_a = 0.f, lse_l = 0.f, lse_t = 0.f, mx0 = 0.f;
        if (!l) {
            mx0 = -3.0e38f;
            for (int v = lane; v < V; v += 64) mx0 = fmaxf(mx0, logits[v]);
            mx0 = wave_max(mx0);
            float s0 = 0.f;
            for (int v = lane; v < V; v += 64) s0 += expf(logits[v] - mx0);
            lse_a = logf(wave_sum(s0));
        } else {
            lse_a = a.norm_am ? row_lse(logits, V, a.am_beta, lane) : 0.f;
            lse_l = a.norm_lm ? row_lse(l, V, -1.f, lane) : 0.f;
            if (a.norm_tot) {
                float mx = -3.0e38f;
                for (int v = lane; v < V; v += 64) mx = fmaxf(mx, (a.am_beta * logits[v] - lse_a) + a.lm_weight * (-l[v] - lse_l));
                mx = wave_max(mx);
                float s = 0.f;
                for (int v = lane; v < V; v += 64) s += expf(((a.am_beta * logits[v] - lse_a) + a.lm_weight * (-l[v] - lse_l)) - mx);
                s = wave_sum(s);
                lse_t = mx + logf(s);
            }
        }
        for (int v = lane; v < V; v += 64) {
            const float lp = l ? ((a.am_beta * logits[v] - lse_a) + a.lm_weight * (-l[v] - lse_l)) - lse_t : (logits[v] - mx0) - lse_a;
            xin[v] = lp;
            if (a.neglogp) a.neglogp[(size_t)r * V + v] = -lp;
        }
    }
    __syncthreads();
    if (a.uniforms && tid == 0) {
        const float u = a.uniforms[r];
        float cum = 0.f;
        int pick = 0;
        bool hit = false;
        for (int v = 0; v < V; ++v) {
            cum += expf(xin[v]);
            if (!hit && cum > u) { pick = v; hit = true; }
        }
        a.outputs[r] = pick;
        if (a.costs) a.costs[r] = -xin[pick];
    }
}

__global__ __launch_bounds__(256) void softmax_emit_kernel(const float* logits, int ld, const float* uniforms, int n, int V,
                                                           long long* outputs, float* costs) {
    const int r = blockIdx.x * 4 + (threadIdx.x >> 6), lane = threadIdx.x & 63;
    if (r >= n) return;
    const float* x = logits + (size_t)r * ld;
    float mx = -3.0e38f;
    for (int v = lane; v < V; v += 64) mx = fmaxf(mx, x[v]);
    mx = wave_max(mx);
    float s = 0.f;
    for (int v = lane; v < V; v += 64) s += expf(x[v] - mx);
    const float lse = logf(wave_sum(s));
    if (lane == 0) {
        const float u = uniforms[r];
        float cum = 0.f;
        int pick = 0;
        bool hit = false;
        for (int v = 0; v < V; ++v) {
            cum += expf((x[v] - mx) - lse);
            if (!hit && cum > u) { pick = v; hit = true; }
        }
        outputs[r] = pick;
        if (costs) costs[r] = -((x[pick] - mx) - lse);
    }
}

#define GRID_Y_MAX 65535

extern "C" {

int lvsr_softmax_emit(void* stream, const float* logits, int ld, const float* uniforms, int n, int V, long long* outputs,
                      float* costs) {
    LVSR_REQUIRE(logits && uniforms && outputs && V > 0, "lvsr_softmax_emit: bad arguments");
    if (n <= 0) return LVSR_OK;
    hipLaunchKernelGGL(softmax_emit_kernel, dim3((n + 3) / 4), dim3(256), 0, (hipStream_t)stream, logits, ld, uniforms, n, V, outputs,
                       costs);
    return lvsr_check_launch("lvsr_softmax_emit");
}

int lvsr_readout_step(void* stream, const lvsr_readout_step_args* args) {
    LVSR_REQUIRE(args != nullptr, "lvsr_readout_step: null args");
    const lvsr_readout_step_args& a = *args;
    LVSR_REQUIRE(a.n > 0 && a.E > 0 && a.P > 0 && a.V > 0 && a.WA && a.Wmw, "lvsr_readout_step: bad arguments");
    LVSR_REQUIRE(a.D + a.E <= RS_MAX_IN && a.P <= RS_MAX_P && a.V <= RS_MAX_V && (!a.Wms || a.P <= RS_MAX_V),
                 "lvsr_readout_step: sizes exceed the LDS budget (D+E <= %d, P <= %d, V <= %d)", RS_MAX_IN, RS_MAX_P, RS_MAX_V);
    LVSR_REQUIRE(a.Wout != nullptr || a.P == a.V, "lvsr_readout_step: without a post-merge layer the merge width must be V");
    LVSR_REQUIRE(a.act >= 0 && a.act <= 3 && (a.act != 1 || a.P % 2 == 0), "lvsr_readout_step: bad activation");
    LVSR_REQUIRE(!a.uniforms || a.outputs, "lvsr_readout_step: emit needs an output buffer");
    LVSR_REQUIRE(a.emitter == 0 || (a.emitter == 1 && !a.lm_add),
                 "lvsr_readout_step: emitter must be 0 (softmax) or 1 (reward regression, without a language model)");
    LVSR_REQUIRE(a.n_hidden >= 0 && a.n_hidden <= 3 && (a.n_hidden == 0 || (a.Wout && (a.act == 2 || a.act == 3))),
                 "lvsr_readout_step: further post-merge layers need a one-piece activation and an output layer");
    for (int h = 0; h < a.n_hidden; ++h)
        LVSR_REQUIRE(a.Wh[h] && a.bh[h] && a.dimh[h] > 0 && a.dimh[h] <= RS_MAX_P && a.dimh[h] <= RS_MAX_V,
                     "lvsr_readout_step: bad post-merge layer %d", h);
    hipLaunchKernelGGL(readout_step_kernel, dim3(a.n), dim3(256), 0, (hipStream_t)stream, a);
    return lvsr_check_launch("lvsr_readout_step");
}

int lvsr_readout_merge(void* stream, const float* S, int lds, const float* WA, int ldwa, int n, int D, int E, int P,
                       const float* Wms_p, const float* Wmw_p, const float* bias1, float* R1, int ldr1) {
    LVSR_REQUIRE(WA && Wmw_p && R1 && n > 0 && E > 0 && P > 0 && ldwa >= E && ldr1 >= P && (!Wms_p || (S && D > 0 && lds >= D)),
                 "lvsr_readout_merge: bad arguments");
    hipLaunchKernelGGL(readout_merge_kernel, dim3((P + 15) / 16, (n + 15) / 16), dim3(256), 0, (hipStream_t)stream, S, lds, WA, ldwa, n,
                       D, E, P, Wms_p, Wmw_p, bias1, R1, ldr1);
    return lvsr_check_launch("lvsr_readout_merge");
}

int lvsr_gather_rows(void* stream, const float* table, int ldt, const long long* idx, int n, int nrows, int width,
                     const float* bias, float* out, int ldo) {
    if (n <= 0 || width <= 0) return LVSR_OK;
    LVSR_REQUIRE(n <= GRID_Y_MAX, "lvsr_gather_rows: n = %d rows exceed the %d of one launch (one work-group row per output row)", n,
                 GRID_Y_MAX);
    hipLaunchKernelGGL(gather_rows_kernel, dim3((width + 255) / 256, n), dim3(256), 0, (hipStream_t)stream, table, ldt, idx, n,
                       nrows, width, bias, out, ldo);
    return lvsr_check_launch("lvsr_gather_rows");
}

int lvsr_scatter_add_rows(void* stream, const float* src, int lds, const long long* idx, int n, int nrows, int width,
                          float* dst, int ldd, float beta) {
    if (nrows <= 0 || width <= 0) return LVSR_OK;
    LVSR_REQUIRE(nrows <= GRID_Y_MAX,
                 "lvsr_scatter_add_rows: nrows = %d rows exceed the %d of one launch (one work-group row per destination row)", nrows,
                 GRID_Y_MAX);
    hipLaunchKernelGGL(scatter_add_rows_kernel, dim3((width + 255) / 256, nrows), dim3(256), 0, (hipStream_t)stream, src, lds,
                       idx, n, width, dst, ldd, beta);
    return lvsr_check_launch("lvsr_scatter_add_rows");
}

int lvsr_act_fwd(void* stream, int kind, const float* x, int ldx, int n, int P, float* y, int ldy) {
    LVSR_REQUIRE(kind >= 0 && kind <= 3 && (kind != 1 || P % 2 == 0), "lvsr_act_fwd: bad activation %d / P=%d", kind, P);
    if (n <= 0 || P <= 0) return LVSR_OK;
    size_t total = (size_t)n * P;
    int nb = (int)((total + 255) / 256);
    if (nb > 4096) nb = 4096;
    hipLaunchKernelGGL(act_fwd_kernel, dim3(nb), dim3(256), 0, (hipStream_t)stream, kind, x, ldx, n, P, y, ldy);
    return lvsr_check_launch("lvsr_act_fwd");
}

int lvsr_act_bwd(void* stream, int kind, const float* x, int ldx, const float* dy, int lddy, int n, int P, float* dx,
                 int lddx) {
    LVSR_REQUIRE(kind >= 0 && kind <= 3 && (kind != 1 || P % 2 == 0), "lvsr_act_bwd: bad activation %d / P=%d", kind, P);
    if (n <= 0 || P <= 0) return LVSR_OK;
    size_t total = (size_t)n * P;
    int nb = (int)((total + 255) / 256);
    if (nb > 4096) nb = 4096;
    hipLaunchKernelGGL(act_bwd_kernel, dim3(nb), dim3(256), 0, (hipStream_t)stream, kind, x, ldx, dy, lddy, n, P, dx, lddx);
    return lvsr_check_launch("lvsr_act_bwd");
}

int lvsr_softmax_nll(void* stream, const float* logits, int ld, const long long* labels, const float* mask, int n, int V,
                     float* cost, float* dlogits, int ldd, float scale, float* neglogp, int ldn) {
    if (n <= 0 || V <= 0) return LVSR_OK;
    hipLaunchKernelGGL(softmax_nll_kernel, dim3((n + 3) / 4), dim3(256), 0, (hipStream_t)stream, logits, ld, labels, mask, n, V,
                       cost, dlogits, ldd, scale, neglogp, ldn);
    return lvsr_check_launch("lvsr_softmax_nll");
}

int lvsr_select_cost(void* stream, const float* x, int ld, const long long* labels, const float* mask, int n, int V, float scale,
                     float* cost) {
    LVSR_REQUIRE(x && labels && cost, "lvsr_select_cost: null argument");
    if (n <= 0) return LVSR_OK;
    hipLaunchKernelGGL(select_cost_kernel, dim3((n + 255) / 256), dim3(256), 0, (hipStream_t)stream, x, ld, labels, mask, n, V, scale, cost);
    return lvsr_check_launch("lvsr_select_cost");
}

int lvsr_shallow_fusion(void* stream, const float* am, int ld, const float* lm_add, int n, int V, float am_beta,
                        float lm_weight, int norm_am, int norm_lm, int norm_tot, float out_scale, float* out) {
    if (n <= 0 || V <= 0) return LVSR_OK;
    hipLaunchKernelGGL(shallow_fusion_kernel, dim3((n + 3) / 4), dim3(256), 0, (hipStream_t)stream, am, ld, lm_add, n, V,
                       am_beta, lm_weight, norm_am, norm_lm, norm_tot, out_scale, out);
    return lvsr_check_launch("lvsr_shallow_fusion");
}

}
```

attention-lvcsr_amd/lvsr_amd/bricks/__init__.py:

```python
import contextlib

import torch


class SpeechBottom(object):
    ACT = {"identity": 0, "rectifier": 2, "tanh": 3}

    def __init__(self, dims, store, lib, workspace):
        self.d, self.store, self.lib, self.ws = dims, store, lib, workspace
        self._saved = None

    def apply(self, recordings, save_for_backward=True):
        d, p, lib, ws = self.d, self.store.p, self.lib, self.ws
        if not d.bottom_dims:
            return recordings
        T, B = int(recordings.shape[0]), int(recordings.shape[1])
        x = recordings.contiguous().view(T * B, d.F)
        saved = []
        for j, o in enumerate(d.bottom_dims):
            z = ws.get("bottom%d.z" % j, (T * B, o))
            lib.sgemm(x, p["/recognizer/bottom/bottom/linear_%d.W" % j], z, bias=p["/recognizer/bottom/bottom/linear_%d.b" % j])
            a = ws.get("bottom%d.a" % j, (T * B, o))
            lib.call("lvsr_act_fwd", lib.stream_for(a), self.ACT[d.bottom_act], native_ptr(z), o, T * B, o, native_ptr(a), o)
            saved.append((x, z))
            x = a
        if save_for_backward:
            self._saved = saved
        return x.view(T, B, d.bottom_dims[-1])

    def backward(self, d_out):
        d, p, g, lib, ws = self.d, self.store.p, self.store.g, self.lib, self.ws
        if not d.bottom_dims:
            return
        gws = ws.get("gemm_ws", (1 << 22,))
        da = d_out.contiguous().view(-1, d.bottom_dims[-1])
        n = int(da.shape[0])
        for j in reversed(range(len(d.bottom_dims))):
            x, z = self._saved[j]
            o = d.bottom_dims[j]
            dz = ws.get("bottom%d.dz" % j, (n, o))
            lib.call("lvsr_act_bwd", lib.stream_for(dz), self.ACT[d.bottom_act], native_ptr(z), o, native_ptr(da), o, n, o,
                     native_ptr(dz), o)
            W = "/recognizer/bottom/bottom/linear_%d.W" % j
            lib.sgemm(x, dz, g[W], transA=True, ws=gws)
            lib.colsum(dz, g["/recognizer/bottom/bottom/linear_%d.b" % j], ws=gws)
            if j > 0:
                dx = ws.get("bottom%d.dx" % j, (n, int(x.shape[1])))
                lib.sgemm(dz, p[W], dx, transB=True)
                da = dx


def native_ptr(t):
    from ..native import ptr
    return ptr(t)


class Encoder(object):
    PERSIST_MAX_ROWS = 2

    PASS_ROWS = 64

    def __init__(self, dims, store, lib, workspace, use_graph=True, use_persistent=None, pfx="enc"):
        can = not lib.is_emulator or lib.emulates_concurrency()
        self.persist_auto = use_persistent is None
        self.use_persistent = can and (not lib.is_emulator if use_persistent is None else bool(use_persistent))
        self.d = dims
        self.store = store
        self.lib = lib
        self.ws = workspace
        self.use_graph = use_graph
        self.pfx = pfx
        self._passes = []
        self.force_passes = False
        self._pass_cols = None
        self._saved = None
        self._packs = {}
        self._cats = {}
        self._pack_cache = {}
        self.overlap = False
        self._side = None
        self._side_pending = False

    def _n(self, i, what):
        return "%s%d.%s" % (self.pfx, i, what)

    def _names(self, i, direction):
        base = "/recognizer/encoder/bidir%d/%s" % (i, direction)
        return dict(Wi=base + "/fork/fork_inputs.W", bi=base + "/fork/fork_inputs.b",
                    Wg=base + "/fork/fork_gate_inputs.W", bg=base + "/fork/fork_gate_inputs.b",
                    Whh=base + "/gatedrecurrent.state_to_state", Whg=base + "/gatedrecurrent.state_to_gates",
                    h0=base + "/gatedrecurrent.initial_state")

    def _packed(self, i):
        if self._packs.get("version") != self.store.version or self.lib.capturing:
            p, lib, ws = self.store.p, self.lib, self.ws
            packs, jobs = dict(version=self.store.version), []
            for li in range(self.d.n_layers):
                H = self.d.Hs[li]
                ent = dict(Whh=[], Whg=[], WhhT=[], WhgT=[])
                for di, direction in enumerate(("forward", "backward")):
                    n = self._names(li, direction)
                    for key, W, trans in (("Whh", p[n["Whh"]], False), ("Whg", p[n["Whg"]], False), ("WhhT", p[n["Whh"]], True)):
                        K, N = (W.shape[1], W.shape[0]) if trans else (W.shape[0], W.shape[1])
                        buf = ws.get("enc%d.%d.%s_p" % (li, di, key), (lib.pack_size(K, N),))
                        jobs.append((W, buf, trans))
                        ent[key].append(buf)
                    sz = lib.pack_size(H, H)
                    buf = ws.get("enc%d.%d.WhgT_p" % (li, di), (2 * sz,))
                    Wg = p[n["Whg"]]
                    jobs.append((Wg[:, :H], buf[:sz], True))
                    jobs.append((Wg[:, H:], buf[sz:], True))
                    ent["WhgT"].append(buf)
                packs[li] = ent
            lib.pack_many(jobs, use_graph=self.use_graph, cache=self._pack_cache)
            self._packs = packs
        return self._packs[i]

    def _fork_cat(self, i):
        ent = self._cats.get(i)
        if ent is None or ent["version"] != self.store.version or self.lib.capturing:
            p, ws = self.store.p, self.ws
            H, I = self.d.Hs[i], self.d.layer_input_dim(i)
            W = ws.get("enc%d.Wcat" % i, (I, 6 * H))
            b = ws.get("enc%d.bcat" % i, (6 * H,))
            pairs = []
            for di, direction in enumerate(("forward", "backward")):
                n = self._names(i, direction)
                o = di * 3 * H
                pairs += [(p[n["Wi"]], W[:, o: o + H]), (p[n["Wg"]], W[:, o + H: o + 3 * H]),
                          (p[n["bi"]], b[o: o + H]), (p[n["bg"]], b[o + H: o + 3 * H])]
            self.lib.copy_many(pairs)
            ent = dict(version=self.store.version, W=W, b=b)
            self._cats[i] = ent
        return ent["W"], ent["b"]

    @contextlib.contextmanager
    def _side_stream(self):
        if not self.overlap or self.lib.is_emulator or not torch.cuda.is_available():
            yield self.ws.get("gemm_ws", (1 << 22,))
            return
        cur = torch.cuda.current_stream()
        if self._side is None:
            self._side = torch.cuda.Stream(cur.device)
        self._side.wait_stream(cur)
        with torch.cuda.stream(self._side):
            yield self.ws.get("gemm_ws.side", (1 << 22,))
        self._side_pending = True

    def join_side_stream(self):
        if self._side is not None and self._side_pending:
            torch.cuda.current_stream().wait_stream(self._side)
            self._side_pending = False

    def _sync_ws(self, i, B, H):
        if not self.use_persistent:
            return None
        nbytes = int(self.lib._lvsr_bigru_persist_ws_bytes(int(B), int(H)))
        if nbytes <= 0:
            return None
        if self.persist_auto and int(self.lib._lvsr_bigru_persist_rows(int(B), int(H))) > self.PERSIST_MAX_ROWS:
            return None
        return self.ws.get(self._n(i, "sync"), ((nbytes + 3) // 4,), torch.int32)

    def check_persistent(self):
        for k, t in self.ws._bufs.items():
            if k[0].startswith("enc") and k[0].endswith(".sync") and int(t[0]) != 0:
                t[:64].zero_()
                raise RuntimeError("persistent BiGRU kernel aborted (a work-group of the cluster was not scheduled); results since "
                                   "the last check are invalid")

    def _pass_columns(self, B):
        if B <= self.PASS_ROWS or self.pfx != "enc":
            return None
        if not self.force_passes:
            if not (self.persist_auto and self.use_persistent):
                return None
            H = max(self.d.Hs)
            if int(self.lib._lvsr_bigru_persist_ws_bytes(int(B), int(H))) > 0 and \
                    int(self.lib._lvsr_bigru_persist_rows(int(B), int(H))) <= self.PERSIST_MAX_ROWS:
                return None
        n = (B + self.PASS_ROWS - 1) // self.PASS_ROWS
        per = (B + n - 1) // n
        return [(lo, min(B, lo + per)) for lo in range(0, B, per)]

    def _pass_encoder(self, k):
        while len(self._passes) <= k:
            child = Encoder(self.d, self.store, self.lib, self.ws, use_graph=self.use_graph, use_persistent=None,
                            pfx="enc.p%d_" % len(self._passes))
            child._cats = self._cats
            self._passes.append(child)
        return self._passes[k]

    @staticmethod
    def _cols2d(t, lo, hi):
        T, B = int(t.shape[0]), int(t.shape[1])
        F = int(t.numel() // max(1, T * B))
        return t.view(T, B * F)[:, lo * F: hi * F]

    def _apply_in_passes(self, cols, input_, mask, save_for_backward):
        d, lib, ws = self.d, self.lib, self.ws
        T, B = int(input_.shape[0]), int(input_.shape[1])
        F = int(input_.shape[2])
        x = input_.contiguous()
        m = None if mask is None else mask.contiguous()
        enc = msk = None
        for k, (lo, hi) in enumerate(cols):
            child = self._pass_encoder(k)
            xk = ws.get(child.pfx + ".x", (T, hi - lo, F))
            pairs = [(self._cols2d(x, lo, hi), xk.view(T, (hi - lo) * F))]
            mk = None
            if m is not None:
                mk = ws.get(child.pfx + ".m", (T, hi - lo))
                pairs.append((self._cols2d(m, lo, hi), mk))
            lib.copy_many(pairs)
            ek, emk = child.apply(xk, mk, save_for_backward=save_for_backward)
            if enc is None:
                Te, E = int(ek.shape[0]), int(ek.shape[2])
                enc = ws.get("enc.passes.encoded", (Te, B, E))
                msk = ws.get("enc.passes.mask", (Te, B))
            lib.copy_many([(ek.view(Te, (hi - lo) * E), self._cols2d(enc, lo, hi)), (emk, self._cols2d(msk, lo, hi))])
        if save_for_backward:
            self._pass_cols = cols
            self._saved = None
        return enc, msk

    def _encoder_gradient_range(self):
        offs = self.store.offsets
        mine = [(o, n) for k, (o, n) in offs.items() if k.startswith("/recognizer/encoder/")]
        lo, hi = min(o for o, n in mine), max(o + (n + 3) // 4 * 4 for o, n in mine)
        assert all(k.startswith("/recognizer/encoder/") == (lo <= o < hi) for k, (o, n) in offs.items()), "encoder parameters are not one range"
        return lo, min(hi, self.store.grad.numel()) - lo

    def _backward_in_passes(self, cols, d_encoded, need_input_grad, group=None):
        d, lib, ws = self.d, self.lib, self.ws
        dy = d_encoded.contiguous()
        Te, B, E = int(dy.shape[0]), int(dy.shape[1]), int(dy.shape[2])
        first, count = self._encoder_gradient_range()
        genc = self.store.grad[first: first + count]
        acc = ws.get("enc.passes.gacc", (count,))
        dx = None
        if group is None:
            group = lib.group()
        for k, (lo, hi) in enumerate(cols):
            child = self._passes[k]
            dk = ws.get(child.pfx + ".dy", (Te, hi - lo, E))
            lib.copy_many([(self._cols2d(dy, lo, hi), dk.view(Te, (hi - lo) * E))])
            dxk = child.backward(dk, need_input_grad=need_input_grad, group=group)
            group.flush(ws.get("gemm_ws.grouped", (1 << 26,)))
            child.finish_backward()
            if need_input_grad:
                if dx is None:
                    dx = ws.get("enc.passes.dx", (int(dxk.shape[0]), B, int(dxk.shape[2])))
                lib.copy_many([(dxk.view(int(dxk.shape[0]), -1), self._cols2d(dx, lo, hi))])
            if k + 1 < len(cols):
                lib.copy_many([(genc, acc, 0.0 if k == 0 else 1.0)])
            else:
                lib.copy_many([(acc, genc, 1.0)])
        self._scatter = []
        return dx

    def apply(self, input_, mask=None, save_for_backward=True):
        d, p, lib, ws = self.d, self.store.p, self.lib, self.ws
        T, B = int(input_.shape[0]), int(input_.shape[1])
        cols = self._pass_columns(B)
        if cols is not None:
            return self._apply_in_passes(cols, input_, mask, save_for_backward)
        if save_for_backward:
            self._pass_cols = None
        x = input_.contiguous()
        m = None if mask is None else mask.contiguous()
        saved = []
        gemm_ws = ws.get("gemm_ws", (1 << 22,))
        for i, (H, s) in enumerate(zip(d.Hs, d.subsample)):
            I = d.layer_input_dim(i)
            Ts = (T + s - 1) // s
            xg = ws.get(self._n(i, "xg"), (T, B, 6 * H))
            y = ws.get(self._n(i, "y"), (T, B, 2 * H))
            ysub = y if s == 1 else ws.get(self._n(i, "ysub"), (Ts, B, 2 * H))
            u = ws.get(self._n(i, "u"), (T, B, 2 * H))
            r = ws.get(self._n(i, "r"), (T, B, 2 * H))
            c = ws.get(self._n(i, "c"), (T, B, 2 * H))
            rh = ws.get(self._n(i, "rh"), (T, B, 2 * H))
            x2, xg2 = x.view(T * B, I), xg.view(T * B, 6 * H)
            sync = self._sync_ws(i, B, H)
            pk = self._packed(i) if sync is None else None
            Wcat, bcat = self._fork_cat(i)
            lib.sgemm(x2, Wcat, xg2, bias=bcat)
            h0s = [p[self._names(i, direction)["h0"]] for direction in ("forward", "backward")]
            if sync is not None:
                nf, nb = self._names(i, "forward"), self._names(i, "backward")
                Whh, Whg = [p[nf["Whh"]], p[nb["Whh"]]], [p[nf["Whg"]], p[nb["Whg"]]]
            else:
                Whh, Whg = [pk["Whh"][0], pk["Whh"][1]], [pk["Whg"][0], pk["Whg"][1]]
            lib.run("lvsr_bigru_fwd", "lvsr_bigru_fwd_args", y, self.use_graph and sync is None, xg=xg, mask=m, Whh_p=Whh, Whg_p=Whg, h0=h0s,
                    y=y, ysub=(ysub if s > 1 else None), u=u, r=r, c=c, rh=rh, sub=s, T=T, B=B, H=H,
                    persistent=int(sync is not None), sync_ws=sync)
            saved.append(dict(x=x, mask=m, T=T, y=y, u=u, r=r, c=c, rh=rh))
            x = ysub
            if m is not None and s > 1:
                mm = ws.get(self._n(i, "msub"), (Ts, B))
                mm.copy_(m[::s])
                m = mm
            T = Ts
        if m is None:
            m = ws.get(self.pfx + ".ones_mask", (T, B))
            m.fill_(1.0)
        if save_for_backward:
            self._saved = saved
        return x, m

    def backward(self, d_encoded, need_input_grad=False, group=None):
        d, p, g, lib, ws = self.d, self.store.p, self.store.g, self.lib, self.ws
        if self._pass_cols is not None:
            return self._backward_in_passes(self._pass_cols, d_encoded, need_input_grad, group)
        assert self._saved is not None, "apply() must run first"
        gemm_ws = ws.get("gemm_ws", (1 << 22,))
        self._scatter = []
        dy = d_encoded.contiguous()
        B = int(dy.shape[1])
        for i in reversed(range(d.n_layers)):
            H, s, I = d.Hs[i], d.subsample[i], d.layer_input_dim(i)
            sv = self._saved[i]
            T = sv["T"]
            dxg = ws.get(self._n(i, "dxg"), (T, B, 6 * H))
            Bp = (B + 15) // 16 * 16
            dh_ws = ws.get(self._n(i, "dh"), (12 * Bp * H,))
            nf, nb = self._names(i, "forward"), self._names(i, "backward")
            sync = self._sync_ws(i, B, H)
            pk = self._packed(i) if sync is None else None
            if sync is not None:
                WhhT, WhgT = [p[nf["Whh"]], p[nb["Whh"]]], [p[nf["Whg"]], p[nb["Whg"]]]
            else:
                WhhT, WhgT = [pk["WhhT"][0], pk["WhhT"][1]], [pk["WhgT"][0], pk["WhgT"][1]]
            lib.run("lvsr_bigru_bwd", "lvsr_bigru_bwd_args", dxg, self.use_graph and sync is None, mask=sv["mask"], y=sv["y"],
                    u=sv["u"], r=sv["r"], c=sv["c"], WhhT_p=WhhT, WhgT_p=WhgT, h0=[p[nf["h0"]], p[nb["h0"]]], dy=dy,
                    dxg=dxg, dh_ws=dh_ws, dh0=[g[nf["h0"]], g[nb["h0"]]], sub=s, T=T, B=B, H=H,
                    persistent=int(sync is not None), sync_ws=sync)
            x2 = sv["x"].view(T * B, I)
            dxg2 = dxg.view(T * B, 6 * H)
            y2 = sv["y"].view(T * B, 2 * H)
            rh2 = sv["rh"].view(T * B, 2 * H)
            dx = None
            if i > 0 or need_input_grad:
                dx = ws.get(self._n(i, "dx"), (T, B, I))
            if dx is not None:
                lib.sgemm(dxg2, self._cats[i]["W"], dx.view(T * B, I), transB=True)
            with self._side_stream() as side_ws:
                wgrad, colsum = lib.weight_grad_calls(group, side_ws)
                for di, direction in enumerate(("forward", "backward")):
                    n = self._names(i, direction)
                    dc = dxg2[:, di * 3 * H: di * 3 * H + H]
                    dg = dxg2[:, di * 3 * H + H: di * 3 * H + 3 * H]
                    hcol = slice(di * H, (di + 1) * H)
                    wgrad(rh2[:, hcol], dc, g[n["Whh"]])
                    if T > 1:
                        if di == 0:
                            wgrad(y2[: (T - 1) * B, hcol], dg[B:], g[n["Whg"]])
                        else:
                            wgrad(y2[B:, hcol], dg[: (T - 1) * B], g[n["Whg"]])
                        beta = 1.0
                    else:
                        beta = 0.0
                    first = dg[:B] if di == 0 else dg[(T - 1) * B:]
                    if group is not None:
                        group.add_after(p[n["h0"]], first, g[n["Whg"]], beta=beta, M=H, K=B, lda=0)
                    else:
                        lib.sgemm(p[n["h0"]], first, g[n["Whg"]], transA=True, beta=beta, M=H, K=B, lda=0)
                gW = ws.get("enc%d.gWcat" % i, (I, 6 * H))
                gb = ws.get("enc%d.gbcat" % i, (6 * H,))
                lib.sgemm(x2, dxg2, gW, transA=True, ws=side_ws)
                colsum(dxg2, gb)
                for di, direction in enumerate(("forward", "backward")):
                    n = self._names(i, direction)
                    o = di * 3 * H
                    self._scatter += [(gW[:, o: o + H], g[n["Wi"]]), (gW[:, o + H: o + 3 * H], g[n["Wg"]]),
                                      (gb[o: o + H], g[n["bi"]]), (gb[o + H: o + 3 * H], g[n["bg"]])]
                if self.overlap and group is not None:
                    group.flush(ws.get("gemm_ws.grouped.side", (1 << 26,)))
            dy = dx
        self.join_side_stream()
        if group is None:
            self.finish_backward()
        return dy

    def finish_backward(self):
        self.lib.copy_many(self._scatter)
        self._scatter = []
```

attention-lvcsr_amd/lvsr_amd/bricks/generator.py:

```python
import ctypes

import numpy
import torch

from ..native import ptr
from .beam_state import BeamState

ACT_KIND = {"identity": 0, "maxout2": 1, "rectifier": 2, "tanh": 3}
NORMALIZER_KIND = {"softmax": 0, "logistic": 1, "relu": 2}
PRIOR_KIND = {"expanding": 0, "window_around_mean": 1, "window_around_median": 2}
ATT_MS = 32


def _f32(x):
    return float(numpy.float32(x))


class SequenceGenerator(object):
    language_model = None
    current_search = None

    def __init__(self, dims, store, lib, workspace, use_graph=True, use_persistent=None):
        self.d = dims
        self.store = store
# ... 8 lines not shown
        self.criterion = dims.cfg["criterion"]
        self.mse = self.criterion != "log_likelihood"
        self.min_reward = float(dims.cfg["min_reward"])
        g = "/recognizer/generator"
        att = g + "/att_trans/" + ("conv_att" if dims.conv else "cont_att")
        self.n = dict(
            Wpre=att + "/preprocess.W", bpre=att + "/preprocess.b", Ws=att + "/state_trans/transform_states.W",
            we=att + "/energy_comp/linear.W", eb=att + "/energy_comp/linear.b", filters=att + "/conv1d.filters", handler=att + "/handler.W",
            Wdi=g + "/att_trans/distribute/fork_inputs.W", Wdg=g + "/att_trans/distribute/fork_gate_inputs.W",
            Whh=g + "/att_trans/transition.state_to_state", Whg=g + "/att_trans/transition.state_to_gates",
            h0=g + "/att_trans/transition.initial_state",
            Wfi=g + "/fork/fork_inputs.W", bfi=g + "/fork/fork_inputs.b",
            Wfg=g + "/fork/fork_gate_inputs.W", bfg=g + "/fork/fork_gate_inputs.b",
            Wms=g + "/readout/merge/transform_states.W", Wmw=g + "/readout/merge/transform_weighted_averages.W",
            bpm=g + "/readout/post_merge/bias.b", Wout=g + "/readout/post_merge/mlp/linear_%d.W" % len(dims.pm_hidden),
            bout=g + "/readout/post_merge/mlp/linear_%d.b" % len(dims.pm_hidden), bro=g + "/readout/bias.b",
            table=g + "/readout/lookupfeedback/lookuptable.W")
        self.pm_hidden = [(g + "/readout/post_merge/mlp/linear_%d.W" % j, g + "/readout/post_merge/mlp/linear_%d.b" % j, w)
                          for j, w in enumerate(dims.pm_hidden)]

    def _state_width(self):
        return self.d.D

    def _merge_states_weight(self):
        return self.store.p[self.n["Wms"]]

    def _initial_state(self):
        return self.store.p[self.n["h0"]]

    def _AW(self, Tp, B):
        ld = (3 * self.d.D + 3) // 4 * 4
        return self.ws.get("gen.AW", (Tp * B, ld))[:, : 3 * self.d.D], ld

    def _merge_states_backward(self, S2, dR1, gws, group=None):
        d, p, g, n, lib, ws = self.d, self.store.p, self.store.g, self.n, self.lib, self.ws
        wgrad, _ = lib.weight_grad_calls(group, gws)
        wgrad(S2, dR1, g[n["Wms"]])
        dS_r = ws.get("gen.dS_r", (S2.shape[0], d.D))
        lib.sgemm(dR1, p[n["Wms"]], dS_r, transB=True)
        return dS_r

    def _packed(self, packs=True):
        if self._packs is not None and self._packs["version"] == self.store.version and not self.lib.capturing:
            if packs:
                self._ensure_packs(self._packs)
            return self._packs
        p, lib, ws, n, d = self.store.p, self.lib, self.ws, self.n, self.d
        ent = dict(version=self.store.version)
        jobs = []

        def pack(key, W, trans=False):
            K, N = (W.shape[1], W.shape[0]) if trans else (W.shape[0], W.shape[1])
            buf = ws.get("gen.%s_p" % key, (lib.pack_size(K, N),))
            jobs.append((W, buf, trans))
            ent[key] = buf
        pack("Ws", p[n["Ws"]]); pack("WsT", p[n["Ws"]], True)
        pack("Whg", p[n["Whg"]]); pack("WhgT", p[n["Whg"]], True)
        pack("Whh", p[n["Whh"]]); pack("WhhT", p[n["Whh"]], True)
        pack("Wdi", p[n["Wdi"]]); pack("Wdg", p[n["Wdg"]])
        wd = ws.get("gen.Wd_cat", (d.E, 3 * d.D))
        lib.copy_many([(p[n["Wdi"]], wd[:, : d.D]), (p[n["Wdg"]], wd[:, d.D:])])
        pack("WdT", wd, True)
        ent["_jobs"], ent["packed"] = jobs, False
        if packs:
            self._ensure_packs(ent)
        self._packs = ent
        return ent

    MERGE_ROWS = 64

    def _readout_packs(self):
        hit = getattr(self, "_ro_packs", None)
        if hit is not None and hit["version"] == self.store.version:
            return hit
        d, p, n, lib, ws = self.d, self.store.p, self.n, self.lib, self.ws
        ent = dict(version=self.store.version, Wms=None)
        Wmw = p[n["Wmw"]]
        ent["Wmw"] = ws.get("gen.Wmw_p", (lib.pack_size(int(Wmw.shape[0]), int(Wmw.shape[1])),))
        jobs = [(Wmw, ent["Wmw"], False)]
        if d.use_states_for_readout:
            Wms = self._merge_states_weight()
            ent["Wms"] = ws.get("gen.Wms_p", (lib.pack_size(int(Wms.shape[0]), int(Wms.shape[1])),))
            jobs.append((Wms.contiguous(), ent["Wms"], False))
        lib.pack_many(jobs)
        self._ro_packs = ent
        return ent

    def _ensure_packs(self, ent):
        if not ent.get("packed", True):
            self.lib.pack_many(ent["_jobs"], use_graph=self.use_graph, cache=self._pack_cache)
            ent["packed"] = True

    def _prior(self):
        pr = self.d.cfg["prior"]
        if not self.d.conv:
            return 0, (0.0, 0.0, 0.0, 0.0)
        kind = PRIOR_KIND.get(pr.get("type", "expanding"))
        if kind is None:
            raise Exception("Unknown prior type: %s" % pr.get("type"))
        if kind == 0:
            return 0, (float(pr["initial_begin"]), float(pr["initial_end"]), _f32(pr["min_speed"]), _f32(pr["max_speed"]))
        return kind, (float(pr["before"]), float(pr["after"]), 0.0, 0.0)

    def _pos_needed(self):
        return bool(self.d.conv and self._prior()[0] != 0)

    def _attdec_bufs(self, prefix, suffix, steps, rows, Tp=None, att=True, gru=True, ZB=False, **given):
        d, ws = self.d, self.ws
        D, Kc = d.D, max(d.K, 1)

        def get(slot, *shape):
            return given[slot] if slot in given else ws.get(prefix + slot + suffix, shape)
        b = dict(given)
        if att:
            b.update(S=get("S", steps + 1, rows, self._state_width()), W=get("W", steps + 1, rows, Tp),
                     pos=get("pos", steps + 1, rows) if self._pos_needed() else None,
                     WA=get("WA", steps, rows, d.E), EN=get("EN", steps, rows, Tp), ZB=get("ZB", steps, rows) if ZB else None,
                     sW=get("sW", steps, rows, d.M), CV=get("CV", steps, rows, Kc, Tp) if d.conv else None)
        if gru:
            b.update(U=get("U", steps, rows, D), R=get("R", steps, rows, D), C=get("C", steps, rows, D), RH=get("RH", steps, rows, D),
                     sg=get("sg", rows, 2 * D), xin=get("xin", rows, D))
        if att:
            b["ep"] = get("ep", rows, (d.M + ATT_MS - 1) // ATT_MS, Tp)
        return b

    def _strides(self, B, broadcast, groups=0, group_Tp=None):
        d = self.d
        if groups:
            return dict(A_ts=groups * d.E, A_bs=d.E, PA_ts=groups * d.M, PA_bs=d.M, Am_ts=groups, Am_bs=1,
                        group_rows=B // groups, step_stride=16, group_Tp=group_Tp)
        if broadcast:
            return dict(A_ts=d.E, A_bs=0, PA_ts=d.M, PA_bs=0, Am_ts=1, Am_bs=0)
        return dict(A_ts=B * d.E, A_bs=d.E, PA_ts=B * d.M, PA_bs=d.M, Am_ts=B, Am_bs=1)

    def _att_fields(self, A, PA, Am, L, B, D, bufs, phases, step0, broadcast, groups=0, group_Tp=None):
        d, p, n = self.d, self.store.p, self.n
        kind, pp = self._prior()
        f = dict(Tp=int(A.shape[0]), B=B, L=L, E=d.E, D=D, M=d.M, K=d.K, c=d.c, prior_type=kind, step0=step0, phases=phases,
                 p0=pp[0], p1=pp[1], p2=pp[2], p3=pp[3], A=A, PA=PA, Am=Am, w_e=p[n["we"]],
                 normalizer=NORMALIZER_KIND[d.normalizer], e_bias=p[n["eb"]] if d.energy_bias else None,
                 filters=p[n["filters"]] if d.conv else None, handler=p[n["handler"]] if d.conv else None)
        f.update(self._strides(B, broadcast, groups, group_Tp))
        f.update(bufs)
        return f

    def _gru_fields(self, pk, l=""):
        return dict(Whg_p=pk["Whg%s" % l], Whh_p=pk["Whh%s" % l], Wdi_p=pk["Wdi%s" % l], Wdg_p=pk["Wdg%s" % l])

    def _attdec_fields(self, pk, A, PA, Am, L, B, bufs, phases, step0, broadcast, groups=0, group_Tp=None):
        f = self._att_fields(A, PA, Am, L, B, self.d.D, bufs, phases, step0, broadcast, groups, group_Tp)
        f.update(self._gru_fields(pk), Ws_p=pk["Ws"])
        return f

    def _feedback_forks(self, labels_flat, nrows, layers, fb_buf=None):
        d, p, lib = self.d, self.store.p, self.lib
        st = lib.stream_for(layers[0][1])
        if d.embed:
            lib.call("lvsr_gather_rows", st, ptr(p[self.n["table"]]), d.FB, ptr(labels_flat), nrows, d.V + 1, d.FB,
                     None, ptr(fb_buf), d.FB)
        for n, xg in layers:
            if d.embed:
                lib.sgemm(fb_buf, p[n["Wfi"]], xg[:, : d.D], bias=p[n["bfi"]])
                lib.sgemm(fb_buf, p[n["Wfg"]], xg[:, d.D:], bias=p[n["bfg"]])
            else:
                lib.call("lvsr_gather_rows", st, ptr(p[n["Wfi"]]), d.D, ptr(labels_flat), nrows, d.FB, d.D,
                         ptr(p[n["bfi"]]), ptr(xg), 3 * d.D)
                lib.call("lvsr_gather_rows", st, ptr(p[n["Wfg"]]), 2 * d.D, ptr(labels_flat), nrows, d.FB, 2 * d.D,
                         ptr(p[n["bfg"]]), ptr(xg[:, d.D:]), 3 * d.D)

    def _feedback_forks_backward(self, l, n, sv, DXG, dfb, wgrad):
        d, p, g, lib = self.d, self.store.p, self.store.g, self.lib
        dpc, dg = DXG[:, : d.D], DXG[:, d.D:]
        nrows, st, labels_flat = int(DXG.shape[0]), lib.stream_for(DXG), sv["labels"].view(-1)
        if d.embed:
            wgrad(sv["fb"], dpc, g[n["Wfi"]])
            wgrad(sv["fb"], dg, g[n["Wfg"]])
            lib.sgemm(dpc, p[n["Wfi"]], dfb, transB=True, beta=0.0 if l == 0 else 1.0)
            lib.sgemm(dg, p[n["Wfg"]], dfb, transB=True, beta=1.0)
            if l == d.n_dec - 1:
                lib.call("lvsr_scatter_add_rows", st, ptr(dfb), d.FB, ptr(labels_flat), nrows, d.V + 1, d.FB,
                         ptr(g[self.n["table"]]), d.FB, 0.0)
        else:
            lib.call("lvsr_scatter_add_rows", st, ptr(dpc), 3 * d.D, ptr(labels_flat), nrows, d.FB, d.D,
                     ptr(g[n["Wfi"]]), d.D, 0.0)
            lib.call("lvsr_scatter_add_rows", st, ptr(dg), 3 * d.D, ptr(labels_flat), nrows, d.FB, 2 * d.D,
                     ptr(g[n["Wfg"]]), 2 * d.D, 0.0)

    def preprocess(self, attended):
        d, p, n = self.d, self.store.p, self.n
        Tp, B = int(attended.shape[0]), int(attended.shape[1])
        PA = self.ws.get("gen.PA", (Tp, B, d.M))
        self.lib.sgemm(attended.view(Tp * B, d.E), p[n["Wpre"]], PA.view(Tp * B, d.M), bias=p[n["bpre"]])
        return PA

    def _readout(self, S2, WA2, nrows, tag):
        d, p, n, lib, ws = self.d, self.store.p, self.n, self.lib, self.ws
        R1 = ws.get("gen.R1" + tag, (nrows, d.P))
        self._pm_acts = []
        bias = p[n["bpm"]] if d.post_merge else p[n["bro"]]
        lib.sgemm(WA2, p[n["Wmw"]], R1, bias=bias)
        if d.use_states_for_readout:
            lib.sgemm(S2, self._merge_states_weight(), R1, beta=1.0)
        if not d.post_merge:
            return R1, None, R1
        R2 = ws.get("gen.R2" + tag, (nrows, d.Pout))
        lib.call("lvsr_act_fwd", lib.stream_for(R2), ACT_KIND[d.act], ptr(R1), d.P, nrows, d.P, ptr(R2), d.Pout)
        for j, (wn, bn, width) in enumerate(self.pm_hidden):
            pre = ws.get("gen.pm_pre%d" % j + tag, (nrows, width))
            lib.sgemm(R2, p[wn], pre, bias=p[bn])
            post = ws.get("gen.pm_post%d" % j + tag, (nrows, width))
            lib.call("lvsr_act_fwd", lib.stream_for(post), ACT_KIND[d.act], ptr(pre), width, nrows, width, ptr(post), width)
            self._pm_acts.append((R2, pre))
            R2 = post
        logits = ws.get("gen.logits" + tag, (nrows, d.V))
        lib.sgemm(R2, p[n["Wout"]], logits, bias=p[n["bout"]])
        return R1, R2, logits

    def _persist_sync(self, query, args, name, emulated=True):
        nbytes = int(getattr(self.lib, "_" + query)(ctypes.byref(args)))
        if emulated and self.lib.is_emulator and not self.lib.emulates_concurrency():
            nbytes = 0
        return self.ws.get(name, ((nbytes + 3) // 4,), torch.int32) if nbytes else None

    def _persistent_ws(self, fields):
        if self.use_persistent is not None and not self.use_persistent:
            return None
        sync = self._persist_sync("lvsr_attdec_persist_ws_bytes", self.lib.make("lvsr_attdec_args", **fields), "gen.sync")
        if sync is None and self.use_persistent:
            raise ValueError("persistent decoder kernel requested but not available for this configuration")
        return sync

    def _persistent_bwd_ws(self, fwd_args):
        if self.use_persistent is False or self.use_persistent_bwd is False:
            return None
        return self._persist_sync("lvsr_attdec_bwd_persist_ws_bytes", fwd_args, "gen.sync_bwd")

    def _plain(self, n, AW, AW_ld):
        p = self.store.p
        return self.lib.make("lvsr_attdec_plain", Ws=p[n["Ws"]], Whg=p[n["Whg"]], Whh=p[n["Whh"]], AW=AW, AW_ld=AW_ld)

    def _cluster_partials(self, query, fwd_args, B):
        d, ws = self.d, self.ws
        P = int(getattr(self.lib, "_" + query)(ctypes.byref(fwd_args)))
        return (ws.get("gen.accH_p", (B * P, max(d.K, 1) * d.M)), ws.get("gen.accWe_p", (B * P, d.M)),
                ws.get("gen.accEb_p", (B * P, 1)))

    def _QR(self, sv, dWA_r):
        d, lib = self.d, self.lib
        L, B, Tp = sv["L"], sv["B"], sv["Tp"]
        QR = self.ws.get("gen.QR", (L, B, Tp))
        lib.call("lvsr_sgemm_batched", lib.stream_for(QR), 0, 1, L, Tp, d.E, 1.0, ptr(dWA_r), B * d.E, d.E,
                 ptr(sv["A"]), B * d.E, d.E, 0.0, ptr(QR), B * Tp, Tp, B)
        return QR

    def check_persistent(self):
        for k, buf in self.ws._bufs.items():
            if k[0] in ("gen.sync", "gen.sync_bwd") and int(buf[0]) != 0:
                buf[:16].zero_()
                raise RuntimeError("persistent decoder kernel aborted (a work-group of a cluster was not scheduled); results since "
                                   "the last check are invalid")

    def _check_emitter(self):
        if self.mse and self.language_model is not None:
            raise NotImplementedError("criterion %s with a language model is not built" % self.criterion)

    def reward_matrices(self, groundtruth, prediction, want_mask=False):
        d, lib, ws = self.d, self.lib, self.ws
        Lp, B = int(prediction.shape[0]), int(prediction.shape[1])
        gt, pred = groundtruth.contiguous(), prediction.contiguous()
        out = dict(rewards=ws.get("gen.reward_matrix", (Lp, B, d.V)), gains=ws.get("gen.gain_matrix", (Lp, B, d.V)),
                   mask=ws.get("gen.prediction_mask", (Lp, B)) if want_mask else None)
        lib.call("lvsr_reward_gain", lib.stream_for(out["rewards"]), ptr(gt), int(gt.shape[0]), ptr(pred), Lp, B, int(d.cfg["eos_label"]),
                 d.V, ptr(out["rewards"]), ptr(out["gains"]), ptr(out["mask"]))
        return out

    def cost_matrix(self, outputs, mask=None, attended=None, attended_mask=None, save_for_backward=True, groundtruth=None,
                    rewards=None):
        self._check_emitter()
        d, p, n, lib, ws = self.d, self.store.p, self.n, self.lib, self.ws
        L, B = int(outputs.shape[0]), int(outputs.shape[1])
        Tp = int(attended.shape[0])
        pk = self._packed(packs=False)
        A = attended.contiguous()
        Am = attended_mask.contiguous()
        labels = outputs.contiguous()
        ym = None if mask is None else mask.contiguous()
        PA = self.preprocess(A)
        rc = self._forward_recurrent(pk, A, PA, Am, labels, ym, L, B, Tp)
        bufs, S, W, WA = rc["bufs"], rc["bufs"]["S"], rc["bufs"]["W"], rc["bufs"]["WA"]
        SW = self._state_width()
        S2, WA2 = S[:L].view(L * B, SW), WA.view(L * B, d.E)
        R1, R2, logits = self._readout(S2, WA2, L * B, "")
        cost = ws.get("gen.cost", (L, B))
        dlogits = ws.get("gen.dlogits", (L * B, d.V))
        if self.mse:
            rw = rewards if rewards is not None else self.reward_matrices(labels if groundtruth is None else groundtruth, labels)
            lib.call("lvsr_reward_mse", lib.stream_for(cost), int(self.criterion == "mse_reward"), ptr(logits), d.V, ptr(rw["gains"]),
                     ptr(rw["rewards"]), ptr(labels), ptr(ym), L, B, d.V, self.min_reward, ptr(cost), ptr(dlogits), d.V)
        else:
            lib.call("lvsr_softmax_nll", lib.stream_for(cost), ptr(logits), d.V, ptr(labels), ptr(ym), L * B, d.V,
                     ptr(cost), ptr(dlogits), d.V, 1.0, None, 0)
        lm = self.language_model
        self._cost_has_lm = lm is not None
        if lm is not None:
            lm_add = self._lm_lookahead(lm, labels, ym, L, B)
            fused = ws.get("gen.fused", (L * B, d.V))
            lib.call("lvsr_shallow_fusion", lib.stream_for(cost), ptr(logits), d.V, ptr(lm_add), L * B, d.V, float(lm.am_beta),
                     float(lm.lm_weight), int(lm.norm[0]), int(lm.norm[1]), int(lm.norm[2]), 1.0, ptr(fused))
            lib.call("lvsr_select_cost", lib.stream_for(cost), ptr(fused), d.V, ptr(labels), ptr(ym), L * B, d.V, -1.0,
                     ptr(cost))
        self.last = dict(weights=W[1:], energies=bufs["EN"], states=S[:L], weighted_averages=WA, readouts=logits.view(L, B, d.V))
        if self.mse:
            self.last.update(gain_matrix=rw["gains"], reward_matrix=rw["rewards"])
        if save_for_backward:
            self._saved = dict(L=L, B=B, Tp=Tp, A=A, Am=Am, PA=PA, labels=labels, ym=ym, bufs=bufs,
                               R1=R1, R2=R2, dlogits=dlogits, pk=pk, pm_acts=list(self._pm_acts))
            self._saved.update(rc["saved"])
        return cost

    def _forward_recurrent(self, pk, A, PA, Am, labels, ym, L, B, Tp):
        d, p, n, lib, ws = self.d, self.store.p, self.n, self.lib, self.ws
        xg = ws.get("gen.xg", (L * B, 3 * d.D))
        fb = ws.get("gen.fb", (L * B, d.FB)) if d.embed else None
        self._feedback_forks(labels.view(-1), L * B, [(n, xg)], fb)
        bufs = self._attdec_bufs("gen.", "", L, B, Tp, ZB=True, xg=xg, ymask=ym)
        S, W = bufs["S"], bufs["W"]
        S[0].copy_(p[n["h0"]].unsqueeze(0).expand(B, d.D))
        W[0].zero_()
        if d.conv:
            W[0, :, 0] = 1.0
        fields = self._attdec_fields(pk, A, PA, Am, L, B, bufs, phases=3, step0=0, broadcast=False)
        sync = self._persistent_ws(fields)
        if sync is not None:
            fwd_args = lib.make("lvsr_attdec_args", **fields)
            wd = ws.get("gen.Wd_cat", (d.E, 3 * d.D))
            AW, AW_ld = self._AW(Tp, B)
            lib.sgemm(A.view(Tp * B, d.E), wd, AW)
            lib.call("lvsr_attdec_fwd_persistent", lib.stream_for(S), ctypes.byref(fwd_args), ctypes.byref(self._plain(n, AW, AW_ld)),
                     ptr(sync), 0)
            lib.call("lvsr_attdec_glimpses", lib.stream_for(S), ctypes.byref(fwd_args))
        else:
            self._ensure_packs(pk)
            fwd_args = lib.run("lvsr_attdec_fwd", "lvsr_attdec_args", S, self.use_graph, **fields)
        return dict(bufs=bufs, saved=dict(xg=xg, fb=fb, fields=fields, AW_valid=sync is not None))

    def _lm_lookahead(self, lm, labels, ym, L, B):
        dev = labels.device
        out = self.ws.get("gen.lm_add", (L, B, self.d.V))
        st = lm.initial_states(B)
        on_dev = lm.on_device
        lab = labels if on_dev else labels.cpu().numpy()
        msk = None if ym is None else (ym if on_dev else ym.cpu().numpy())
        for i in range(L):
            out[i].copy_(lm.stage(st, dev))
            if i + 1 == L:
                break
            new = lm.transition(st, lab[i])
            if msk is not None:
                if on_dev:
                    keep = msk[i] > 0
                    st = {k: torch.where(keep.view(-1, *([1] * (v.dim() - 1))), new[k], st[k]) for k, v in new.items()}
                else:
                    keep = msk[i] > 0
                    st = {k: numpy.where(keep.reshape((-1,) + (1,) * (v.ndim - 1)), new[k], st[k]) for k, v in new.items()}
            else:
                st = new
        return out.view(L * B, self.d.V)

    def backward(self, group=None):
        d, p, g, n, lib, ws = self.d, self.store.p, self.store.g, self.n, self.lib, self.ws
        sv = self._saved
        assert sv is not None, "cost_matrix() must run first"
        if getattr(self, "_cost_has_lm", False):
            lm = self.language_model
            if lm is None or tuple(lm.norm) != (True, False, False) or float(lm.am_beta) != 1.0:
                raise NotImplementedError("gradient through ShallowFusionReadout is built for normalize_am_weights only (am_beta = 1)")
        L, B, Tp = sv["L"], sv["B"], sv["Tp"]
        bufs, pk = sv["bufs"], sv["pk"]
        nrows = L * B
        gws = ws.get("gemm_ws", (1 << 22,))
        wgrad, colsum = lib.weight_grad_calls(group, gws)
        S2, WA2 = bufs["S"][:L].view(nrows, self._state_width()), bufs["WA"].view(nrows, d.E)
        dlogits, R1, R2 = sv["dlogits"], sv["R1"], sv["R2"]
        if d.post_merge:
            wgrad(R2, dlogits, g[n["Wout"]])
            colsum(dlogits, g[n["bout"]])
            dR2 = ws.get("gen.dR2", (nrows, R2.shape[1]))
            lib.sgemm(dlogits, p[n["Wout"]], dR2, transB=True)
            for j in range(len(self.pm_hidden) - 1, -1, -1):
                wn, bn, width = self.pm_hidden[j]
                xin, pre = sv["pm_acts"][j]
                dpre = ws.get("gen.pm_dpre%d" % j, (nrows, width))
                lib.call("lvsr_act_bwd", lib.stream_for(dpre), ACT_KIND[d.act], ptr(pre), width, ptr(dR2), width, nrows, width,
                         ptr(dpre), width)
                wgrad(xin, dpre, g[wn])
                colsum(dpre, g[bn])
                dR2 = ws.get("gen.pm_dx%d" % j, (nrows, xin.shape[1]))
                lib.sgemm(dpre, p[wn], dR2, transB=True)
            dR1 = ws.get("gen.dR1", (nrows, d.P))
            lib.call("lvsr_act_bwd", lib.stream_for(dR1), ACT_KIND[d.act], ptr(R1), d.P, ptr(dR2), d.Pout, nrows, d.P,
                     ptr(dR1), d.P)
            colsum(dR1, g[n["bpm"]])
        else:
            dR1 = dlogits
            colsum(dR1, g[n["bro"]])
        wgrad(WA2, dR1, g[n["Wmw"]])
        dWA_r = ws.get("gen.dWA_r", (nrows, d.E))
        lib.sgemm(dR1, p[n["Wmw"]], dWA_r, transB=True)
        dS_r = None
        if d.use_states_for_readout:
            dS_r = self._merge_states_backward(S2, dR1, gws, group)
        rb = self._backward_recurrent(sv, dWA_r, dS_r, gws, group)
        accH, accWe, accEb, DCV, dPA, DWA = rb["accH"], rb["accWe"], rb["accEb"], rb["DCV"], rb["dPA"], rb["DWA"]
        st = lib.stream_for(dPA)
        colsum(accWe, g[n["we"]].view(-1))
        if d.energy_bias:
            colsum(accEb, g[n["eb"]])
        if d.conv:
            colsum(accH, g[n["handler"]].view(-1))
            fws = ws.get("gen.filter_ws", (max(1 << 20, L * B * d.K * (2 * d.c + 1)),))
            lib.call("lvsr_attdec_filter_grad", st, ctypes.byref(rb["fwd_args"]), ptr(DCV), ptr(g[n["filters"]]), ptr(fws),
                     fws.numel() * 4)
        A2, dPA2 = sv["A"].view(Tp * B, d.E), dPA.view(Tp * B, d.M)
        wgrad(A2, dPA2, g[n["Wpre"]])
        colsum(dPA2, g[n["bpre"]])
        dA = ws.get("gen.dA", (Tp, B, d.E))
        lib.sgemm(dPA2, p[n["Wpre"]], dA.view(Tp * B, d.E), transB=True)
        W = bufs["W"]
        lib.call("lvsr_sgemm_batched", lib.stream_for(dA), 1, 0, Tp, d.E, L, 1.0, ptr(W[1:]), B * Tp, Tp,
                 ptr(DWA), B * d.E, d.E, 1.0, ptr(dA), B * d.E, d.E, B)
        return dA

    def _backward_recurrent(self, sv, dWA_r, dS_r, gws, group=None):
        d, p, g, n, lib, ws = self.d, self.store.p, self.store.g, self.n, self.lib, self.ws
        L, B, Tp = sv["L"], sv["B"], sv["Tp"]
        bufs, pk = sv["bufs"], sv["pk"]
        nrows = L * B
        S2, WA2 = bufs["S"][:L].view(nrows, d.D), bufs["WA"].view(nrows, d.E)
        nslice = (d.M + ATT_MS - 1) // ATT_MS
        ntile = (Tp + 63) // 64
        Kc = max(d.K, 1)
        wgrad, colsum = lib.weight_grad_calls(group, gws)
        DXG = ws.get("gen.DXG", (nrows, 3 * d.D))
        DWA = dWA_r.view(L, B, d.E)
        DSW = ws.get("gen.DSW", (nrows, d.M))
        DCV = ws.get("gen.DCV", (L, B, Kc, Tp)) if d.conv else None
        dPA = ws.get("gen.dPA", (Tp, B, d.M), zero=True)
        ds = ws.get("gen.ds", (B, d.D), zero=True)
        wd = ws.get("gen.Wd_cat", (d.E, 3 * d.D))
        AW, AW_ld = self._AW(Tp, B)
        if not sv.get("AW_valid"):
            lib.sgemm(sv["A"].view(Tp * B, d.E), wd, AW)
        QR = self._QR(sv, dWA_r)
        fwd_args = lib.make("lvsr_attdec_args", **sv["fields"])
        psync = self._persistent_bwd_ws(fwd_args)
        if psync is not None:
            accH, accWe, accEb = self._cluster_partials("lvsr_attdec_bwd_persist_clusters", fwd_args, B)
            bw = lib.make("lvsr_attdec_bwd_args", dS_r=dS_r, DXG=DXG, DSW=DSW, DCV=DCV, dPA=dPA, accH=accH, accWe=accWe, accEb=accEb,
                          ds=ds, AW=AW, QR=QR, AW_ld=AW_ld)
            bw.f = fwd_args
            lib.call("lvsr_attdec_bwd_persistent", lib.stream_for(ds), ctypes.byref(bw), ctypes.byref(self._plain(n, AW, AW_ld)), ptr(psync))
        else:
            self._ensure_packs(pk)
            accH = ws.get("gen.accH", (B * ntile, Kc * d.M), zero=True)
            accWe = ws.get("gen.accWe", (B * ntile, d.M), zero=True)
            accEb = ws.get("gen.accEb", (B * ntile, 1), zero=True)
            bw = lib.make("lvsr_attdec_bwd_args", WhhT_p=pk["WhhT"], WhgT_p=pk["WhgT"], WdT_p=pk["WdT"], WsT_p=pk["WsT"],
                          dWA_r=dWA_r, dS_r=dS_r, DXG=DXG, DWA=DWA, DSW=DSW, DCV=DCV, dPA=dPA, accH=accH, accWe=accWe, accEb=accEb,
                          ds=ds, dalp=ws.get("gen.dalp", (B, Kc, Tp), zero=True), dspart=ws.get("gen.dspart", (B, d.D)),
                          dsacc=ws.get("gen.dsacc", (B, d.D)), Q=ws.get("gen.Q", (B, Tp)),
                          dcvp=ws.get("gen.dcvp", (B, nslice, Kc, Tp)) if d.conv else None,
                          dswp=ws.get("gen.dswp", (B, ntile, d.M)), AW=AW, QR=QR, AW_ld=AW_ld)
            bw.f = fwd_args
            lib.call("lvsr_attdec_bwd", lib.stream_for(ds), ctypes.byref(bw), int(self.use_graph))
        lib.sgemm(DXG, wd, dWA_r, transB=True, beta=1.0)
        dpc, dg = DXG[:, : d.D], DXG[:, d.D:]
        RH2 = bufs["RH"].view(nrows, d.D)
        wgrad(RH2, dpc, g[n["Whh"]])
        wgrad(S2, dg, g[n["Whg"]])
        wgrad(WA2, dpc, g[n["Wdi"]])
        wgrad(WA2, dg, g[n["Wdg"]])
        wgrad(S2, DSW, g[n["Ws"]])
        colsum(ds, g[n["h0"]])
        colsum(dpc, g[n["bfi"]])
        colsum(dg, g[n["bfg"]])
        self._feedback_forks_backward(0, n, sv, DXG, ws.get("gen.dfb", (nrows, d.FB)) if d.embed else None, wgrad)
        return dict(accH=accH, accWe=accWe, accEb=accEb, DCV=DCV, dPA=dPA, DWA=DWA, fwd_args=fwd_args)

    def init_generation(self, attended, attended_mask):
        d = self.d
        Tp, N = int(attended.shape[0]), int(attended.shape[1])
        A = attended.contiguous()
        PA = self.preprocess(A)
        if N == 1:
            self._gen = dict(Tp=Tp, A=A.view(Tp, d.E), Am=attended_mask.contiguous().view(Tp), PA=PA.view(Tp, d.M))
        else:
            Am = attended_mask.contiguous()
            self._gen = dict(Tp=Tp, A=A, Am=Am, PA=PA, N=N, lengths=self.ws.get("gen.glen", (N,), torch.int32))
            self._gen["lengths"].copy_(Am.sum(dim=0).to(torch.int32))

    def initial_states(self, batch_size, attended=None, attended_mask=None):
        d = self.d
        h0 = self._initial_state()
        dev = h0.device
        B = int(batch_size)
        Tp = int(attended.shape[0]) if attended is not None else 0
        out = dict(states=h0.unsqueeze(0).expand(B, self._state_width()).clone(),
                   outputs=torch.full((B,), 0 if self.mse else d.V, dtype=torch.int64, device=dev),
                   weighted_averages=torch.zeros(B, d.E, device=dev), weights=torch.zeros(B, Tp, device=dev))
        if d.conv:
            if Tp:
                out["weights"][:, 0] = 1.0
            out["energies"] = out["weights"].clone()
            out["step"] = torch.zeros(B, dtype=torch.int64, device=dev)
        return out

    def emit(self, readouts, uniforms=None, seed=None):
        d, lib = self.d, self.lib
        x = readouts.contiguous()
        n = int(x.shape[0])
        u = self._uniforms((n,), uniforms, seed, x.device)
        out = torch.empty(n, dtype=torch.int64, device=x.device)
        cost = torch.empty(n, dtype=torch.float32, device=x.device)
        lib.call("lvsr_softmax_emit", lib.stream_for(x), ptr(x), int(x.stride(0)), ptr(u), n, int(x.shape[1]), ptr(out),
                 ptr(cost))
        return out, cost

    def _uniforms(self, shape, uniforms, seed, dev):
        if uniforms is not None:
            u = torch.as_tensor(numpy.ascontiguousarray(uniforms, dtype=numpy.float32)) if not torch.is_tensor(uniforms) else uniforms
            u = u.to(dev).to(torch.float32).contiguous()
            assert tuple(u.shape) == tuple(shape), "uniforms must have shape %s" % (tuple(shape),)
            return u
        if dev.type == "cuda":
            gen = torch.Generator(device=dev)
            gen.manual_seed(int(seed if seed is not None else 1))
            return torch.rand(shape, generator=gen, device=dev, dtype=torch.float32)
        gen = torch.Generator()
        gen.manual_seed(int(seed if seed is not None else 1))
        return torch.rand(shape, generator=gen, dtype=torch.float32)

    def generate(self, n_steps=None, batch_size=None, attended=None, attended_mask=None, uniforms=None, seed=None):
        d, p, n, lib, ws = self.d, self.store.p, self.n, self.lib, self.ws
        self._check_emitter()
        if self.language_model is not None:
            raise NotImplementedError("generate() with a language model: the reference's LMEmitter.emit returns zeros (not a "
                                      "sampling path); use beam_search, or cost / analyze for teacher-forced costs")
        N = int(n_steps)
        Tp, B = int(attended.shape[0]), int(attended.shape[1])
        assert batch_size is None or int(batch_size) == B
        pk = self._packed()
        A, Am = attended.contiguous(), attended_mask.contiguous()
        PA = self.preprocess(A)
        dev = A.device
        u = None if self.mse else self._uniforms((N, B), uniforms, seed, dev)
        pos_needed = self._pos_needed()
        S = ws.get("sg.S", (N + 1, B, d.D))
        W = ws.get("sg.W", (N + 1, B, Tp))
        S[0].copy_(self._initial_state().unsqueeze(0).expand(B, d.D))
        W[0].zero_()
        if d.conv:
            W[0, :, 0] = 1.0
        full = self._attdec_bufs("sg.", "", N, B, Tp, S=S, W=W, xg=ws.get("sg.xg", (N, B, 3 * d.D)), ymask=None)
        outputs = ws.get("sg.outputs", (N, B), torch.int64)
        costs = ws.get("sg.costs", (N, B))
        fb = ws.get("sg.fb", (B, d.FB)) if d.embed else None
        if pos_needed:
            full["pos"][0].zero_()
        st = lib.stream_for(S)
        for t in range(N):
            bufs = {k: v if v is None or k in ("sg", "xin", "ep") else v[t:] for k, v in full.items()}
            skip = 4 if pos_needed else 0
            fa = self._attdec_fields(pk, A, PA, Am, 1, B, bufs, phases=1 | skip, step0=t, broadcast=False)
            lib.call("lvsr_attdec_fwd", st, ctypes.byref(lib.make("lvsr_attdec_args", **fa)), 0)
            ra = self._readout_step_args(S[t], full["WA"][t], B, uniforms=None if u is None else u[t], outputs=outputs[t], costs=costs[t])
            lib.call("lvsr_readout_step", st, ctypes.byref(ra))
            self._feedback_forks(outputs[t], B, [(n, full["xg"][t])], fb)
            fg = self._attdec_fields(pk, A, PA, Am, 1, B, bufs, phases=2, step0=t, broadcast=False)
            lib.call("lvsr_attdec_fwd", st, ctypes.byref(lib.make("lvsr_attdec_args", **fg)), 0)
        return dict(states=S[1:], outputs=outputs, weighted_averages=full["WA"], weights=W[1:], energies=full["EN"], costs=costs)

    def beam_begin(self, K, eol, max_length, ignore_first_eol=False, char_discount=0.0, round_to_inf=1e9, stop_on="patience",
                   force_merge=False):
        self._check_emitter()
        self.current_search = BeamState(self, K, eol, max_length, ignore_first_eol, char_discount, round_to_inf, stop_on, force_merge)
        return self.current_search

    def _readout_step_args(self, S2, WA2, n, neglogp=None, lm_add=None, uniforms=None, outputs=None, costs=None, logits=None, R1=None):
        d, p, n_ = self.d, self.store.p, self.n
        lm = self.language_model
        return self.lib.make(
            "lvsr_readout_step_args", S=S2, WA=WA2, lds=int(S2.stride(0)), ldwa=int(WA2.stride(0)), n=n, D=self._state_width(), E=d.E,
            P=d.P, V=d.V, act=ACT_KIND[d.act] if d.post_merge else 0,
            Wms=self._merge_states_weight() if d.use_states_for_readout else None, Wmw=p[n_["Wmw"]],
            bias1=p[n_["bpm"]] if d.post_merge else p[n_["bro"]], Wout=p[n_["Wout"]] if d.post_merge else None,
            bout=p[n_["bout"]] if d.post_merge else None, lm_add=lm_add,
            am_beta=lm.am_beta if lm_add is not None else 1.0, lm_weight=lm.lm_weight if lm_add is not None else 0.0,
            norm_am=int(lm.norm[0]) if lm_add is not None else 1, norm_lm=int(lm.norm[1]) if lm_add is not None else 0,
            norm_tot=int(lm.norm[2]) if lm_add is not None else 0, neglogp=neglogp, logits=logits, uniforms=uniforms,
            R1=R1, ldr1=0 if R1 is None else int(R1.stride(0)), emitter=int(self.mse),
            outputs=outputs, costs=costs, n_hidden=len(self.pm_hidden), Wh=[p[w] for w, _, _ in self.pm_hidden],
            bh=[p[b] for _, b, _ in self.pm_hidden], dimh=[w for _, _, w in self.pm_hidden])
```

attention-lvcsr_amd/lvsr_amd/native.py:

```python
import ctypes
import functools
import os
import re

import torch

_HERE = os.path.dirname(os.path.abspath(__file__))
DEFAULT_LIB = os.path.join(_HERE, "liblvsr_hip.so")
HEADER = os.path.join(os.path.dirname(os.path.dirname(_HERE)), "include", "lvsr_hip.h")


_SCALARS = {"int": ctypes.c_int, "float": ctypes.c_float, "double": ctypes.c_double,
            "long long": ctypes.c_longlong, "char": ctypes.c_char}


class NativeError(RuntimeError):
    pass


def _strip_comments(src):
    src = re.sub(r"/\*.*?\*/", " ", src, flags=re.S)
    src = re.sub(r"//[^\n]*", " ", src)
    src = re.sub(r"^\s*#.*$", " ", src, flags=re.M)
    return src
# ... 54 lines not shown
                argnames.append(toks[-1])
                base = " ".join(toks[:-1])
                if nptr and base.replace("const", "").strip() in structs:
                    argtypes.append(ctypes.POINTER(structs[base.replace("const", "").strip()]))
                else:
                    argtypes.append(_ctype(base, nptr, structs))
        functions[name] = (restype, argtypes, argnames)
    return structs, functions


def ptr(t):
    if t is None:
        return None
    if isinstance(t, int):
        return ctypes.c_void_p(t)
    if t.dim() > 0 and t.numel() > 0:
        assert t.stride(-1) == 1, "last dimension must be contiguous"
    return ctypes.c_void_p(t.data_ptr())


def _addr(v):
    if v is None:
        return None
    if isinstance(v, int):
        return v
    if v.dim() > 0 and v.numel() > 0:
        assert v.stride(-1) == 1, "last dimension must be contiguous"
    return v.data_ptr()


class Lib(object):
    def __init__(self, path=DEFAULT_LIB, sync_after_graph=True, step_graph=True):
        self.sync_after_graph = bool(sync_after_graph)
        self.step_graph = bool(step_graph)
        if not os.path.exists(path):
            raise NativeError(
                "HIP extension %s not found: build it with `python __graft_entry__.py` "
                "(hipcc --offload-arch=gfx950). There is no fallback path." % path)
        self.path = path
        self._dll = ctypes.CDLL(path)
        self.is_emulator = hasattr(self._dll, "hipemu_set_concurrent")
        self._gstream = None
        self.capturing = False
        self.structs, self.functions = parse_header()
        self.knobs = {m.group(1): int(m.group(2)) for m in re.finditer(r"#define\s+LVSR_KNOB_(\w+)\s+(\d+)", open(HEADER).read())
                      if m.group(1) != "COUNT"}
        for name, (res, args, _) in self.functions.items():
            try:
                fn = getattr(self._dll, name)
            except AttributeError:
                raise NativeError("symbol %s (declared in include/lvsr_hip.h) missing from %s" % (name, path))
            fn.restype = res
            fn.argtypes = args
            setattr(self, "_" + name, fn)

    def emulates_concurrency(self):
        if not self.is_emulator or not hasattr(self._dll, "hipemu_get_concurrent"):
            return False
        return bool(self._dll.hipemu_get_concurrent())

    def stream_for(self, t):
        if t.is_cuda:
            return ctypes.c_void_p(torch.cuda.current_stream(t.device).cuda_stream)
        if not self.is_emulator:
            raise NativeError("CPU tensor passed to the HIP library; the hot path runs on cuda devices only")
        return ctypes.c_void_p(0)

    def make(self, struct_name, **kw):
        cls = self.structs[struct_name]
        s = cls()
        known = dict(cls._fields_)
        for k, v in kw.items():
            if k not in known:
                raise NativeError("%s has no field %s" % (struct_name, k))
            ft = known[k]
            if isinstance(v, (list, tuple)):
                arr = getattr(s, k)
                for i, e in enumerate(v):
                    arr[i] = _addr(e) if ft._type_ is ctypes.c_void_p else e
            elif ft is ctypes.c_void_p:
                setattr(s, k, _addr(v))
            else:
                setattr(s, k, v)
        return s

    def call(self, name, *args):
        rc = getattr(self, "_" + name)(*args)
        if rc != 0:
            raise NativeError("%s failed (%d): %s" % (name, rc, self._lvsr_last_error().decode()))

    def last_error(self):
        return self._lvsr_last_error().decode()

    def set_knob(self, name, value):
        self.call("lvsr_set_knob", name if isinstance(name, int) else self.knobs[name.upper()], int(value))

    def get_knob(self, name):
        return int(self._lvsr_get_knob(name if isinstance(name, int) else self.knobs[name.upper()]))

    def set_knobs(self, settings):
        if not isinstance(settings, dict):
            settings = dict((kv.split("=")[0], int(kv.split("=")[1])) for kv in settings)
        unknown = [k for k in settings if k.upper() not in self.knobs]
        if unknown:
            raise NativeError("unknown knob(s) %s (include/lvsr_hip.h LVSR_KNOB_*: %s)" % (unknown, sorted(k.lower() for k in self.knobs)))
        low = {k.upper(): int(v) for k, v in settings.items()}
        for name in self.knobs:
            self.set_knob(name, low.get(name, 0))

    def group(self):
        return GemmGroup(self)

    def weight_grad_calls(self, group, ws):
        if group is None:
            return functools.partial(self.sgemm, transA=True, ws=ws), functools.partial(self.colsum, ws=ws)
        return group.add, functools.partial(group.colsum, ws=ws)

    def sgemm(self, A, B, C, transA=False, transB=False, alpha=1.0, beta=0.0, bias=None, ws=None,
              M=None, N=None, K=None, lda=None, ldb=None, ldc=None):
        if M is None:
            M = A.shape[1] if transA else A.shape[0]
        if K is None:
            K = A.shape[0] if transA else A.shape[1]
        if N is None:
            N = B.shape[0] if transB else B.shape[1]
        lda = A.stride(0) if lda is None else lda
        ldb = B.stride(0) if ldb is None else ldb
        ldc = C.stride(0) if ldc is None else ldc
        self.call("lvsr_sgemm", self.stream_for(C), int(transA), int(transB), M, N, K, alpha, ptr(A), lda, ptr(B), ldb,
                  beta, ptr(C), ldc, ptr(bias), ptr(ws), (ws.numel() * 4 if ws is not None else 0))

    def colsum(self, X, out, beta=0.0, M=None, N=None, ldx=None, ws=None):
        M = X.shape[0] if M is None else M
        N = X.shape[1] if N is None else N
        ldx = X.stride(0) if ldx is None else ldx
        self.call("lvsr_colsum", self.stream_for(out), ptr(X), M, N, ldx, ptr(out), beta,
                  ptr(ws), (ws.numel() * 4 if ws is not None else 0))

    def copy_many(self, pairs):
        if not pairs:
            return
        cls = self.structs["lvsr_copy_desc"]
        arr = (cls * len(pairs))()
        for d, pair in zip(arr, pairs):
            src, dst = pair[0], pair[1]
            d.beta = float(pair[2]) if len(pair) > 2 else 0.0
            assert src.shape == dst.shape and src.dim() in (1, 2) and src.stride(-1) == 1 and dst.stride(-1) == 1
            rows, cols = (1, src.shape[0]) if src.dim() == 1 else (src.shape[0], src.shape[1])
            d.src, d.dst, d.rows, d.cols = src.data_ptr(), dst.data_ptr(), rows, cols
            d.lds = src.stride(0) if src.dim() == 2 else cols
            d.ldd = dst.stride(0) if dst.dim() == 2 else cols
        self.call("lvsr_copy2d_many", self.stream_for(pairs[0][1]), arr, len(pairs))

    def transpose(self, x, out):
        self.call("lvsr_transpose", self.stream_for(out), ptr(x), x.shape[0], x.shape[1], ptr(out))

    def pack_size(self, K, N):
        return int(self._lvsr_pack_size(K, N))

    def pack_b(self, W, packed, trans=False):
        K, N = (W.shape[1], W.shape[0]) if trans else (W.shape[0], W.shape[1])
        assert packed.numel() >= self.pack_size(K, N)
        self.call("lvsr_pack_b", self.stream_for(packed), ptr(W), W.stride(0), K, N, int(trans), ptr(packed))

    def pack_many(self, jobs, use_graph=False, cache=None):
        if not jobs:
            return
        sig = tuple((W.data_ptr(), W.stride(0), W.shape[0], W.shape[1], P.data_ptr(), int(t)) for W, P, t in jobs)
        arr = None if cache is None or cache.get("sig") != sig else cache.get("arr")
        if arr is None:
            cls = self.structs["lvsr_pack_desc"]
            arr = (cls * len(jobs))()
            for d, (W, P, t) in zip(arr, jobs):
                K, N = (W.shape[1], W.shape[0]) if t else (W.shape[0], W.shape[1])
                assert W.stride(1) == 1 and P.numel() >= self.pack_size(K, N)
                d.W, d.packed, d.ldw, d.K, d.N, d.trans = W.data_ptr(), P.data_ptr(), W.stride(0), K, N, int(t)
            if cache is not None:
                cache["sig"], cache["arr"] = sig, arr
        ref = jobs[0][1]
        self.call("lvsr_pack_b_many", self.stream_for(ref), arr, len(jobs), int(bool(use_graph) and ref.is_cuda))

    def run(self, fn, struct_name, ref_tensor, use_graph=None, **fields):
        a = self.make(struct_name, **fields)
        if use_graph is None:
            self.call(fn, self.stream_for(ref_tensor), ctypes.byref(a))
        else:
            self.call(fn, self.stream_for(ref_tensor), ctypes.byref(a), int(use_graph))
        if use_graph:
            self.after_graph(ref_tensor, max(fields.get("T", 0), fields.get("L", 0)))
        return a

    def after_graph(self, ref_tensor, steps):
        if self.sync_after_graph and ref_tensor.is_cuda and steps >= 16 and not self.capturing:
            torch.cuda.current_stream(ref_tensor.device).synchronize()

    def region(self, owner, key, ref_tensor, enabled=True, volatile=(), drain=True):
        return Region(self, owner, key, ref_tensor, enabled, volatile, drain)

    _uid = [0]

    @classmethod
    def unique_token(cls):
        cls._uid[0] += 1
        return cls._uid[0]


class GemmGroup(object):
    def __init__(self, lib):
        self.lib = lib
        self.first, self.after, self.colsums = [], [], []

    @staticmethod
    def _member(A, B, C, beta, M=None, N=None, K=None, lda=None, ldb=None, ldc=None):
        assert A.stride(-1) == 1 and B.stride(-1) == 1 and C.stride(-1) == 1, "grouped products need unit inner strides"
        dims = (A.shape[1] if M is None else M, B.shape[1] if N is None else N, A.shape[0] if K is None else K,
                A.stride(0) if lda is None else lda, B.stride(0) if ldb is None else ldb, C.stride(0) if ldc is None else ldc)
        return (A, B, C, float(beta)) + tuple(int(v) for v in dims)

    def add(self, A, B, C, beta=0.0):
        assert A.dim() == B.dim() == C.dim() == 2
        self.first.append(self._member(A, B, C, beta))

    def add_after(self, A, B, C, beta=0.0, **sizes):
        self.after.append(self._member(A, B, C, beta, **sizes))

    def colsum(self, X, out, beta=0.0, M=None, N=None, ldx=None, ws=None):
        self.colsums.append((X, out, float(beta), int(X.shape[0] if M is None else M), int(X.shape[1] if N is None else N),
                             int(X.stride(0) if ldx is None else ldx), (ws.numel() * 4 if ws is not None else 0)))

    @staticmethod
    def _independent(members):
        def span(t, rows, cols, ld):
            return t.data_ptr(), t.data_ptr() + 4 * ((rows - 1) * ld + cols if rows > 0 and cols > 0 else 0)
        spans = [(span(A, K, M, lda), span(B, K, N, ldb), span(C, M, N, ldc)) for A, B, C, _, M, N, K, lda, ldb, ldc in members]
        return not any(lo < c_hi and c_lo < hi
                       for i, mine in enumerate(spans) for j, (_, _, (c_lo, c_hi)) in enumerate(spans) if i != j
                       for lo, hi in mine)

    def _launch_grouped(self, members, ws):
        arr = (self.lib.structs["lvsr_gemm_desc"] * len(members))()
        for d, (A, B, C, beta, M, N, K, lda, ldb, ldc) in zip(arr, members):
            d.A, d.B, d.C = A.data_ptr(), B.data_ptr(), C.data_ptr()
            d.M, d.N, d.K, d.lda, d.ldb, d.ldc, d.beta = M, N, K, lda, ldb, ldc, beta
        self.lib.call("lvsr_sgemm_tn_grouped", self.lib.stream_for(members[0][2]), arr, len(members), ptr(ws),
                      ws.numel() * 4 if ws is not None else 0)

    def flush(self, ws):
        lib = self.lib
        first, after, colsums = self.first, self.after, self.colsums
        self.first, self.after, self.colsums = [], [], []
        if first:
            self._launch_grouped(first, ws)
        if len(after) > 1 and self._independent(after):
            self._launch_grouped(after, None)
        else:
            for A, B, C, beta, M, N, K, lda, ldb, ldc in after:
                lib.sgemm(A, B, C, transA=True, beta=beta, M=M, N=N, K=K, lda=lda, ldb=ldb, ldc=ldc)
        if not colsums:
            return
        split_ws = {c[6] for c in colsums}
        if len({c[1].data_ptr() for c in colsums}) != len(colsums) or len(split_ws) != 1 or len(colsums) > 32:
            for X, out, beta, M, N, ldx, wsb in colsums:
                lib.call("lvsr_colsum", lib.stream_for(out), ptr(X), M, N, ldx, ptr(out), beta, ptr(ws) if wsb else None, min(wsb, ws.numel() * 4))
            return
        arr = (lib.structs["lvsr_colsum_desc"] * len(colsums))()
        for d, (X, out, beta, M, N, ldx, wsb) in zip(arr, colsums):
            d.X, d.out, d.M, d.N, d.ldx, d.beta = X.data_ptr(), out.data_ptr(), M, N, ldx, beta
        wsb = split_ws.pop()
        lib.call("lvsr_colsum_many", lib.stream_for(colsums[0][1]), arr, len(colsums), ptr(ws) if wsb else None, ws.numel() * 4 if wsb else 0, wsb)


class Region(object):
    def __init__(self, lib, owner, key, ref, enabled, volatile=(), drain=True):
        self.lib, self.ref = lib, ref
        self.drain = drain
        if not hasattr(owner, "_region_token"):
            owner._region_token, owner._regions = lib.unique_token(), {}
        soft = repr((owner._region_token, key)).encode()
        self.kb = soft + b"|" + repr(volatile).encode()
        self.enabled = bool(enabled) and lib.step_graph and ref.is_cuda and not lib.is_emulator and not lib.capturing
        self.state = "eager"
        self.slot = owner._regions.setdefault(soft, dict(seen=0, result=None)) if self.enabled else dict(seen=0, result=None)

    @property
    def result(self):
        return self.slot["result"]

    @result.setter
    def result(self, v):
        self.slot["result"] = v

    def _alloc_count(self):
        return torch.cuda.memory_stats(self.ref.device).get("allocation.all.allocated", 0)

    def begin(self):
        if not self.enabled:
            return True
        self.slot["seen"] += 1
        if self.slot.get("bad"):
            return True
        if self.slot["seen"] == 1:
            self.state = "first"
            self.lib._lvsr_graph_suppress(1)
            return True
        lib = self.lib
        rc = lib._lvsr_region_begin(lib.stream_for(self.ref), self.kb, len(self.kb))
# ... 58 lines not shown
```

attention-lvcsr_amd/lvsr_amd/training.py:

```python
import ctypes
import logging
import os

import numpy
import torch

from .native import ptr


def _is_weight(name):
    return name.endswith(".W") or name.endswith("state_to_state") or name.endswith("state_to_gates")


logger = logging.getLogger(__name__)


def _is_sync_word(key):
    return key[0] in ("gen.sync", "gen.sync_bwd") or (key[0].startswith("enc") and key[0].endswith(".sync"))


class Trainer(object):
    RECOVER_RESERVE = 32
    REARM_STEPS = 200
    OVERLAP_RESERVE = 32

    def __init__(self, recognizer, gradient_threshold=None, rules=("momentum",), scale=0.1, momentum=0.0,
                 decay_rate=0.95, epsilon=1e-8, max_norm=0.0, max_norm_exclude_lookup=False, nonfinite_scaler=0.0,
                 burn_in_steps=0, adaptive_clipping=None, process_group=None, distributed=None, dp_region=True,
                 overlap_allreduce=False, adaptive_noise=None, num_examples=None, exploration="imitative", observables=None):
        if exploration == "mixed":
            raise NotImplementedError("exploration 'mixed' (a Bernoulli draw per utterance between prediction and labels) is not built")
        if exploration not in ("imitative", "greedy"):
            raise ValueError("unknown exploration %r" % (exploration,))
        if exploration == "greedy" and not recognizer.generator.mse:
            raise NotImplementedError("greedy exploration needs an mse criterion (net.criterion.name mse_gain / mse_reward)")
        if exploration == "greedy" and overlap_allreduce:
            raise NotImplementedError("greedy exploration with overlap_allreduce is not built")
        self.exploration = exploration
        from .weight_noise import settings as noise_settings
        noise_conf = noise_settings(adaptive_noise)
        from .observables import settings as observables_settings
        obs_conf = observables_settings(observables)
        if obs_conf is not None and obs_conf["parameter_stats"] and noise_conf is not None:
            raise NotImplementedError("observables.parameter_stats with adaptive_noise is not built (the rules run over [means | "
                                      "log-variances]; pass observables=dict(parameter_stats=False))")
        if noise_conf is not None and num_examples is None:
            raise ValueError("adaptive_noise needs num_examples (the number of examples of the training set, lvsr/main.py:434)")
        self.rec = recognizer
        self._token = recognizer.lib.unique_token()
        st = recognizer.store
        dev = st.device
        self.conf = dict(clip_threshold=float(gradient_threshold or 0.0), use_momentum=int("momentum" in rules),
                         use_adadelta=int("adadelta" in rules), learning_rate=float(scale), momentum=float(momentum),
                         decay_rate=float(decay_rate), epsilon=float(epsilon), max_norm=float(max_norm or 0.0),
                         remove_not_finite=1, nonfinite_scaler=float(nonfinite_scaler))
        total = st.flat.numel()
        n = 2 * total if noise_conf is not None else total
        z = lambda: torch.zeros(n, dtype=torch.float32, device=dev)
        self.velocity = z() if self.conf["use_momentum"] else None
        self.ms_step = z() if self.conf["use_adadelta"] else None
        self.ms_dx = z() if self.conf["use_adadelta"] else None
        self.step_buf = z()
        seg, max_cols = [], 1
        for name, (off, cnt) in st.offsets.items():
            shape = st.shapes[name]
            rows, cols = (int(shape[0]), int(numpy.prod(shape[1:]))) if len(shape) >= 2 else (1, int(cnt))
            flag = int(self.conf["max_norm"] > 0 and _is_weight(name) and len(shape) == 2
                       and not (max_norm_exclude_lookup and "lookuptable" in name))
            if flag:
                max_cols = max(max_cols, cols)
            seg.append([off, rows, cols, flag])
        if noise_conf is not None:
            seg += [[off + total, rows, cols, 0] for off, rows, cols, _ in list(seg)]
        self.max_cols = max_cols
        self.segments = torch.tensor(seg, dtype=torch.int64, device=dev)
        self.segflag = torch.zeros(len(seg), dtype=torch.int32, device=dev)
        self.noise = None
        if noise_conf is not None:
            from .weight_noise import WeightNoise
            self.noise = WeightNoise(recognizer, self.segments[: len(st.offsets)], num_examples, **noise_conf)
            recognizer.weight_noise = self.noise
        self.scratch = torch.zeros(2 + 256, dtype=torch.float32, device=dev)
        self.clip_state = None
        if adaptive_clipping or burn_in_steps:
            ac = dict(decay_rate=0.998, burnin_period=500)
            if isinstance(adaptive_clipping, dict):
                ac.update(adaptive_clipping)
            if adaptive_clipping and not self.conf["clip_threshold"] > 0:
                raise ValueError("adaptive clipping needs gradient_threshold (its initial threshold)")
            self.clip_state = torch.tensor([self.conf["clip_threshold"], 0.0, 0.0, 0.0, float(burn_in_steps or 0), 0, 0, 0],
                                           dtype=torch.float64, device=dev)
            self.conf.update(adaptive_clipping=int(bool(adaptive_clipping)), adaptive_burnin=int(ac["burnin_period"]),
                             adaptive_decay=float(ac["decay_rate"]))
        if distributed is None:
            distributed = torch.distributed.is_available() and torch.distributed.is_initialized()
        self.distributed = distributed
        self.group = process_group
        self.world = torch.distributed.get_world_size(process_group) if distributed else 1
        self.rank = torch.distributed.get_rank(process_group) if distributed else 0
        self.dp_region = bool(dp_region)
        self.overlap_allreduce = bool(overlap_allreduce)
        self._comm = None
        self._overlap_reserve_before = None
        if self.overlap_allreduce and self.world > 1 and recognizer.lib.get_knob("cluster_reserve") == 0:
            self._overlap_reserve_before = 0
            recognizer.lib.set_knob("cluster_reserve", self.OVERLAP_RESERVE)
        self._skip_host = torch.zeros(1, dtype=torch.float32).pin_memory() if dev.type == "cuda" else None
        self.aborts = 0
        self._fallback = None
        self._reserve_before = None
        self._last_abort_step = None
        self.steps_done = 0
        self.obs = None
        if obs_conf is not None:
            from .observables import Observables
            self.obs = Observables(self, **obs_conf)

    @classmethod
    def from_config(cls, recognizer, training, regularization=None, adaptive_clipping=True, num_examples=None, **kw):
        reg = regularization or {}
        if reg.get("adaptive_noise"):
            kw.update(adaptive_noise=reg["adaptive_noise"], num_examples=num_examples)
        return cls(recognizer, gradient_threshold=training.get("gradient_threshold"), rules=tuple(training.get("rules", ["momentum"])),
                   scale=training.get("scale", 0.1), momentum=training.get("momentum", 0.0),
                   decay_rate=training.get("decay_rate", 0.95), epsilon=training.get("epsilon", 1e-8),
                   max_norm=reg.get("max_norm", 0.0) or 0.0, max_norm_exclude_lookup=reg.get("max_norm_exclude_lookup", False),
                   burn_in_steps=training.get("burn_in_steps", 0), exploration=training.get("exploration", "imitative"),
                   adaptive_clipping=adaptive_clipping and bool(training.get("gradient_threshold")), **kw)

    def state_dict(self):
        out = {}
        for name in ("velocity", "ms_step", "ms_dx"):
            t = getattr(self, name)
            if t is not None:
                out[name] = t.detach().cpu().numpy()
        if self.clip_state is not None:
            out["clip_state"] = self.clip_state.detach().cpu().numpy()
        if self.noise is not None:
            out["noise_counter"] = self.noise.counter.detach().cpu().numpy()
        out["layout"] = numpy.array(self._layout())
        return out

    def _layout(self):
        layout = ["%s:%d:%d" % (n, o, c) for n, (o, c) in self.rec.store.offsets.items()]
        return layout + (["adaptive_noise:%d" % self.noise.n] if self.noise is not None else [])

    def load_state_dict(self, state):
        if "layout" in state and [str(x) for x in state["layout"]] != self._layout():
            raise ValueError("training state was saved for another parameter layout (or with adaptive noise %s)"
                             % ("off" if self.noise is not None else "on"))
        for name in ("velocity", "ms_step", "ms_dx", "clip_state"):
            t = getattr(self, name)
            if t is not None and name in state:
                t.copy_(torch.as_tensor(numpy.asarray(state[name])).to(t.dtype))
        if self.noise is not None and "noise_counter" in state:
            self.noise.counter.copy_(torch.as_tensor(numpy.asarray(state["noise_counter"])).to(torch.int64))

    def gradient_threshold(self):
        return float(self.clip_state[0]) if self.clip_state is not None else self.conf["clip_threshold"]

    def gradient_norm(self):
        return float(self.scratch[0])

    def noise_stats(self):
        if self.noise is None:
            raise ValueError("this trainer runs without adaptive noise")
        return self.noise.observables()

    def observables(self):
        if self.obs is None:
            raise ValueError("this trainer runs without observables")
# ... 201 lines not shown
```

include/lvsr_hip.h:

```cpp
#ifndef LVSR_HIP_H
#define LVSR_HIP_H

#ifdef __cplusplus
extern "C" {
#endif

const char* lvsr_last_error(void);
int lvsr_abi_version(void);
void lvsr_graph_clear(void);
int lvsr_graph_count(void);
void lvsr_graph_suppress(int on);
int lvsr_region_begin(void* stream, const char* key, long long key_bytes);
int lvsr_region_end(void* stream, int keep);
#define LVSR_KNOB_PERSIST_ROWS 0
#define LVSR_KNOB_PERSIST_FLAGS 1
#define LVSR_KNOB_PERSIST_THREADS 2
#define LVSR_KNOB_PHASE_CLOCK 3
#define LVSR_KNOB_MAX_CLUSTER_WGS 4
#define LVSR_KNOB_CLUSTER_RESERVE 5
#define LVSR_KNOB_GEMM_MID_TILES 6
#define LVSR_KNOB_DEC_CLUSTER 7
#define LVSR_KNOB_ENERGY_ROWS 8
#define LVSR_KNOB_COUNT 9
int lvsr_set_knob(int knob, int value);
int lvsr_get_knob(int knob);

int lvsr_sgemm(void* stream, int transA, int transB, int M, int N, int K, float alpha, const float* A, int lda,
               const float* B, int ldb, float beta, float* C, int ldc, const float* bias, float* ws,
               long long ws_bytes);
int lvsr_sgemm_batched(void* stream, int transA, int transB, int M, int N, int K, float alpha, const float* A, int lda,
                       long long strideA, const float* B, int ldb, long long strideB, float beta, float* C, int ldc,
                       long long strideC, int batch);
typedef struct lvsr_gemm_desc {
    const float* A; const float* B; float* C;
    int M, N, K, lda, ldb, ldc;
    float beta;
} lvsr_gemm_desc;
int lvsr_sgemm_tn_grouped(void* stream, const lvsr_gemm_desc* descs, int n, float* ws, long long ws_bytes);
int lvsr_sgemm_tn_grouped_plan(const lvsr_gemm_desc* descs, int n, long long ws_bytes, int* ksplit, int* kchunk);
typedef struct lvsr_copy_desc {
    const float* src; float* dst;
    int rows, cols, lds, ldd;
    float beta;
} lvsr_copy_desc;
int lvsr_copy2d_many(void* stream, const lvsr_copy_desc* descs, int n);
int lvsr_colsum(void* stream, const float* X, int M, int N, int ldx, float* out, float beta, float* ws,
                long long ws_bytes);
typedef struct lvsr_colsum_desc {
    const float* X; float* out;
    int M, N, ldx;
    float beta;
} lvsr_colsum_desc;
int lvsr_colsum_many(void* stream, const lvsr_colsum_desc* descs, int n, float* ws, long long ws_bytes, long long split_ws_bytes);
int lvsr_transpose(void* stream, const float* in, int rows, int cols, float* out);

long long lvsr_pack_size(int K, int N);
int lvsr_pack_b(void* stream, const float* W, int ldw, int K, int N, int trans, float* packed);
typedef struct lvsr_pack_desc {
    const float* W;
    float* packed;
    int ldw, K, N, trans;
} lvsr_pack_desc;
int lvsr_pack_b_many(void* stream, const lvsr_pack_desc* descs, int n, int use_graph);

typedef struct lvsr_bigru_fwd_args {
    const float* xg;
    const float* mask;
    const float* Whh_p[2];
    const float* Whg_p[2];
    const float* h0[2];
    float* y;
    float* ysub;
    float* u; float* r; float* c; float* rh;
    int sub, T, B, H;
    int kernel_mask;
    int persistent;
    void* sync_ws;
} lvsr_bigru_fwd_args;
int lvsr_bigru_fwd(void* stream, const lvsr_bigru_fwd_args* a, int use_graph);

typedef struct lvsr_bigru_bwd_args {
    const float* mask; const float* y; const float* u; const float* r; const float* c;
    const float* WhhT_p[2];
    const float* WhgT_p[2];
    const float* h0[2];
    const float* dy;
    float* dxg;
    float* dh_ws;
    float* dh0[2];
    int sub, T, B, H;
    int kernel_mask;
    int persistent;
    void* sync_ws;
} lvsr_bigru_bwd_args;
int lvsr_bigru_bwd(void* stream, const lvsr_bigru_bwd_args* a, int use_graph);
int lvsr_bigru_persist_rows(int B, int H);
long long lvsr_bigru_persist_ws_bytes(int B, int H);

typedef struct lvsr_attdec_args {
    int Tp, B, L, E, D, M, K, c;
    int prior_type;
    int step0;
    int phases;
    int normalizer;
    double p0, p1, p2, p3;
    const float* A; const float* PA; const float* Am;
    long long A_ts, A_bs, PA_ts, PA_bs, Am_ts, Am_bs;
    const float* Ws_p;
    const float* w_e;
    const float* e_bias;
    const float* filters;
    const float* handler;
    const float* Whg_p;
    const float* Whh_p;
    const float* Wdi_p;
    const float* Wdg_p;
    const float* xg;
    const float* ymask;
    float* S;
    float* W;
    float* pos;
    float* WA;
    float* EN;
    float* ZB;
    float* sW;
    float* CV;
    float* U; float* R; float* C; float* RH;
    float* sg;
    float* xin;
    float* ep;
    const int* step_dev;
    int S_ld;
    int label0;
    int group_rows, step_stride;
    const int* group_Tp;
    const int* skip; int skip_stride;
} lvsr_attdec_args;
int lvsr_attdec_fwd(void* stream, const lvsr_attdec_args* a, int use_graph);

typedef struct lvsr_attdec_plain {
    const float* Ws;
    const float* Whg;
    const float* Whh;
    const float* AW;
    int AW_ld;
} lvsr_attdec_plain;
long long lvsr_attdec_persist_ws_bytes(const lvsr_attdec_args* a);
int lvsr_attdec_fwd_persistent(void* stream, const lvsr_attdec_args* a, const lvsr_attdec_plain* w, void* ws, int use_graph);
typedef struct lvsr_attdec_stack2 {
    const float* Whg1; const float* Whh1;
    const float* Ws1;
    const float* F1;
    const float* AW1;
    const float* xg1;
    float* U1; float* R1; float* C1; float* RH1;
    int F1_ld, AW1_ld;
    float* DXG1;
} lvsr_attdec_stack2;
long long lvsr_attdec_stack2_persist_ws_bytes(const lvsr_attdec_args* a);
int lvsr_attdec_fwd_persistent_stack2(void* stream, const lvsr_attdec_args* a, const lvsr_attdec_plain* w,
                                      const lvsr_attdec_stack2* l1, void* ws, int use_graph);
int lvsr_attdec_glimpses(void* stream, const lvsr_attdec_args* a);

typedef struct lvsr_attdec_bwd_args {
    lvsr_attdec_args f;
    const float* WhhT_p;
    const float* WhgT_p;
    const float* WdT_p;
    const float* WsT_p;
    const float* dWA_r;
    const float* dS_r;
    float* DXG;
    float* DWA;
    float* DSW;
    float* DCV;
    float* dPA;
    float* accH;
    float* accWe;
    float* accEb;
    float* ds;
    float* dalp;
    float* dspart; float* dsacc;
    float* Q;
    float* dcvp;
    float* dswp;
    const float* AW;
    const float* QR;
    int AW_ld;
    int ds_ld;
    int parts;
} lvsr_attdec_bwd_args;
int lvsr_attdec_bwd(void* stream, const lvsr_attdec_bwd_args* a, int use_graph);
long long lvsr_attdec_bwd_persist_ws_bytes(const lvsr_attdec_args* a);
int lvsr_attdec_bwd_persist_clusters(const lvsr_attdec_args* a);
int lvsr_attdec_bwd_persistent(void* stream, const lvsr_attdec_bwd_args* a, const lvsr_attdec_plain* w, void* ws);
long long lvsr_attdec_stack2_bwd_persist_ws_bytes(const lvsr_attdec_args* a);
int lvsr_attdec_stack2_bwd_persist_clusters(const lvsr_attdec_args* a);
int lvsr_attdec_bwd_persistent_stack2(void* stream, const lvsr_attdec_bwd_args* a, const lvsr_attdec_plain* w,
                                      const lvsr_attdec_stack2* l1, void* ws);
int lvsr_attdec_filter_grad(void* stream, const lvsr_attdec_args* f, const float* DCV, float* dfilters, float* ws,
                            long long ws_bytes);

int lvsr_gather_rows(void* stream, const float* table, int ldt, const long long* idx, int n, int nrows, int width,
                     const float* bias, float* out, int ldo);
int lvsr_scatter_add_rows(void* stream, const float* src, int lds, const long long* idx, int n, int nrows, int width,
                          float* dst, int ldd, float beta);
int lvsr_act_fwd(void* stream, int kind, const float* x, int ldx, int n, int P, float* y, int ldy);
int lvsr_act_bwd(void* stream, int kind, const float* x, int ldx, const float* dy, int lddy, int n, int P, float* dx,
                 int lddx);
int lvsr_softmax_nll(void* stream, const float* logits, int ld, const long long* labels, const float* mask, int n, int V,
                     float* cost, float* dlogits, int ldd, float scale, float* neglogp, int ldn);

int lvsr_reward_gain(void* stream, const long long* groundtruth, int Lg, const long long* prediction, int Lp, int B, int eos, int V,
                     float* rewards, float* gains, float* prediction_mask);
int lvsr_reward_mse(void* stream, int mode, const float* readouts, int ld, const float* gains, const float* rewards,
                    const long long* labels, const float* mask, int L, int B, int V, float min_reward, float* cost, float* dlogits,
                    int ldd);

typedef struct lvsr_opt_args {
    float* param; const float* grad;
    float* velocity; float* ms_step; float* ms_dx;
    float* step;
    const long long* segments;
    int* segflag;
    float* scratch;
    long long n;
    int nseg, max_cols;
    int use_momentum, use_adadelta, remove_not_finite, pad0;
    float grad_scale, clip_threshold, learning_rate, momentum, decay_rate, epsilon, max_norm, nonfinite_scaler;
    double* clip_state;
    int adaptive_clipping, adaptive_burnin;
    float adaptive_decay, pad1;
    const float* guard;
} lvsr_opt_args;
int lvsr_opt_step(void* stream, const lvsr_opt_args* a);
int lvsr_guard_collect(void* stream, const int* const* words, int n, float* out);

typedef struct lvsr_wnoise_args {
    const float* mu; const float* ls2;
    float* noisy;
    const long long* segments;
    int nseg, pad0;
    long long n;
    long long seed;
    long long* counter;
    double* stats;
    const float* grad;
    float grad_scale, pad1;
    double coef;
    double num_examples;
    float* gtheta;
} lvsr_wnoise_args;
int lvsr_wnoise_sample(void* stream, const lvsr_wnoise_args* a);
int lvsr_wnoise_grad(void* stream, const lvsr_wnoise_args* a);
int lvsr_philox_normal(void* stream, long long seed, long long counter, long long first, long long nblocks, float* z, unsigned* raw);

int lvsr_alignment_stats(void* stream, const float* weights, long long ldw, int L, int B, int Tp, const float* mask,
                         double* partials, double* out, int accumulate);
int lvsr_utterance_stats(void* stream, const float* weights, long long ldw, int L, int B, int Tp, const float* mask,
                         const float* costs, const int* lengths, double* partials, double* out);
int lvsr_tensor_stats(void* stream, const float* x, long long n, int use_floor, float floor, double* partials, double* out);
typedef struct lvsr_segnorm_args {
    const float* param; const float* grad; const float* step;
    const long long* segments;
    const long long* items;
    const int* seg_first;
    int nseg, nitems;
    float grad_scale, nonfinite_scaler;
    int remove_not_finite, pad0;
    const int* segflag; const float* scratch; const double* clip_state;
    double* partials;
    double* segsums;
    float* out;
    double* total;
} lvsr_segnorm_args;
int lvsr_segment_norms(void* stream, const lvsr_segnorm_args* a, int phase);

typedef struct lvsr_readout_step_args {
    const float* S; const float* WA;
    int lds, ldwa, n, D, E, P, V, act;
    const float* Wms;
    const float* Wmw;
    const float* bias1;
    const float* Wout; const float* bout;
    const float* lm_add;
    float am_beta, lm_weight;
    int norm_am, norm_lm, norm_tot;
    float* neglogp;
    float* logits;
    const float* uniforms;
    long long* outputs; float* costs;
    int n_hidden; int dimh[3];
    const float* Wh[3]; const float* bh[3];
    const float* R1; int ldr1;
    int emitter;
} lvsr_readout_step_args;
int lvsr_readout_step(void* stream, const lvsr_readout_step_args* a);
int lvsr_readout_merge(void* stream, const float* S, int lds, const float* WA, int ldwa, int n, int D, int E, int P,
                       const float* Wms_p, const float* Wmw_p, const float* bias1, float* R1, int ldr1);
int lvsr_softmax_emit(void* stream, const float* logits, int ld, const float* uniforms, int n, int V, long long* outputs,
                      float* costs);

typedef struct lvsr_beam_args {
    int K, V, eol, ignore_first_eol;
    int stop_on;
    int max_length, fin_cap, D, Tp;
    float round_to_inf;
    double char_discount;
    int* ctl; float* fctl;
    const float* neglogp;
    float* running; int* live_col;
    int* hist_parent; int* hist_char; float* hist_cost;
    int* fin_pos; int* fin_col; float* fin_cost; float* fin_score;
    int* keep;
    long long* chars;
    int* parents;
    const float* S_live; const float* W_live; float* S_sel; float* W_sel;
    const long long* lm_states_live; const double* lm_weights_live;
    long long* lm_states_sel; double* lm_weights_sel;
    const float* pos_live; float* pos_sel;
    float* fork_xg; const float* fork_Wi; const float* fork_Wg; const float* fork_bi; const float* fork_bg; int fork_rows;
    const float* pos_new; float* pos_live_out;
    const float* S_new; const float* W_new; float* S_live_out; float* W_live_out;
    const long long* lm_states_new; const double* lm_weights_new; const float* lm_add_new;
    long long* lm_states_live_out; double* lm_weights_live_out; float* lm_add_live_out;
    int groups;
    const float* WA_live; float* WA_sel; const float* W1_live; float* W1_sel; const float* pos1_live; float* pos1_sel; int E;
} lvsr_beam_args;
int lvsr_beam_select(void* stream, const lvsr_beam_args* a);
int lvsr_beam_compact(void* stream, const lvsr_beam_args* a);
int lvsr_topk_smallest(void* stream, const float* costs, int n, int k, long long* idx, float* val);

int lvsr_shallow_fusion(void* stream, const float* am, int ld, const float* lm_add, int n, int V, float am_beta,
                        float lm_weight, int norm_am, int norm_lm, int norm_tot, float out_scale, float* out);
int lvsr_select_cost(void* stream, const float* x, int ld, const long long* labels, const float* mask, int n, int V, float scale,
                     float* cost);

typedef struct lvsr_fst {
    const int* arc_off;
    const int* arc_lab;
    const int* arc_dst;
    const double* arc_w;
    const int* eps_off;
    const int* eps_dst;
    const double* eps_w;
    const int* topo;
    const int* remap;
    int num_states, V;
    double no_transition_cost;
} lvsr_fst;
int lvsr_fst_lm_step(void* stream, const lvsr_fst* f, const long long* states, const double* weights,
                     const long long* outputs, int n, long long* new_states, double* new_weights, float* add, int* err);
int lvsr_fst_lm_step_groups(void* stream, const lvsr_fst* f, const long long* states, const double* weights,
                            const long long* outputs, int n, long long* new_states, double* new_weights, float* add, int* err,
                            const int* ctl, int group_rows);

typedef struct lvsr_fbank_cfg {
    int frame_length, frame_shift;
    int num_mel, use_energy, remove_dc, pad0;
// ... 32 lines not shown
```

Before: 1.048 million frames/s.

## Merge small launches: batched clears, h0 sums, paired gather/scatter, fused optimizer finite check

```diff
diff --git a/attention-lvcsr_amd/csrc/encoder_persist.hip b/attention-lvcsr_amd/csrc/encoder_persist.hip
--- a/attention-lvcsr_amd/csrc/encoder_persist.hip
+++ b/attention-lvcsr_amd/csrc/encoder_persist.hip
@@ -529,6 +529,17 @@
     for (int b = 0; b < B; ++b) s += dh[((size_t)dir * Bp + b) * H + j];
     (dir == 0 ? out_f : out_b)[j] = s;
 }
+#define H0_MANY_MAX 16
+struct H0Pack { lvsr_h0_desc d[H0_MANY_MAX]; };
+__global__ __launch_bounds__(256) void enc_pbwd_h0_many_kernel(H0Pack pk) {
+    const lvsr_h0_desc& d = pk.d[blockIdx.y];
+    const int dir = blockIdx.z;
+    const int j = blockIdx.x * 256 + threadIdx.x;
+    if (j >= d.H) return;
+    float s = 0.f;
+    for (int b = 0; b < d.B; ++b) s += d.dh[((size_t)dir * d.Bp + b) * d.H + j];
+    (dir == 0 ? d.out_f : d.out_b)[j] = s;
+}
 
 template <int KS, int U>
 __device__ __forceinline__ void ub_dot(const f32x2 (&w)[U][KS / 2], const float* buf, int q, float (&out)[U]) {
@@ -747,7 +758,7 @@
     if (a.sub == 1) a.ysub = nullptr;
     const int flags = persist_flags();
     auto enqueue = [&]() {
-        (void)hipMemsetAsync(planes, 0, bytes, s);
+        if (!(a.persistent & 4)) (void)hipMemsetAsync(planes, 0, bytes, s);
         switch (g.KSPLIT / (g.NTH / 256)) {
             case 2: launch_fwd<64, 2>(s, a, g, planes, hello, ab, flags); break;
             case 4: launch_fwd<64, 4>(s, a, g, planes, hello, ab, flags); break;
@@ -773,13 +784,14 @@
     float* dh = a.dh_ws;
     const int flags = persist_flags();
     auto enqueue = [&]() {
-        (void)hipMemsetAsync(planes, 0, bytes, s);
+        if (!(a.persistent & 4)) (void)hipMemsetAsync(planes, 0, bytes, s);
         switch (g.KSPLIT / (g.NTH / 256)) {
             case 2: launch_bwd<64, 2>(s, a, g, planes, hello, ab, dh, Bp, flags); break;
             case 4: launch_bwd<64, 4>(s, a, g, planes, hello, ab, dh, Bp, flags); break;
             default: launch_bwd<64, 8>(s, a, g, planes, hello, ab, dh, Bp, flags); break;
         }
-        hipLaunchKernelGGL(enc_pbwd_h0_kernel, dim3((a.H + 255) / 256, 1, 2), dim3(256), 0, s, dh, Bp, a.B, a.H, a.dh0[0], a.dh0[1]);
+        if (!(a.persistent & 2))
+            hipLaunchKernelGGL(enc_pbwd_h0_kernel, dim3((a.H + 255) / 256, 1, 2), dim3(256), 0, s, dh, Bp, a.B, a.H, a.dh0[0], a.dh0[1]);
     };
     GraphKey key("bigru_pbwd");
     key.add(&a, sizeof(a));
@@ -788,3 +800,21 @@
     key.add(&flags, sizeof(flags));
     return lvsr_run_graph(s, use_graph, key, enqueue, "lvsr_bigru_bwd(persistent)");
 }
+
+extern "C" int lvsr_bigru_h0_many(void* stream, const lvsr_h0_desc* descs, int n) {
+    LVSR_REQUIRE(n >= 0 && (n == 0 || descs), "lvsr_bigru_h0_many: bad arguments");
+    for (int i = 0; i < n; ++i)
+        LVSR_REQUIRE(descs[i].dh && descs[i].out_f && descs[i].out_b && descs[i].B > 0 && descs[i].H > 0 && descs[i].Bp >= descs[i].B,
+                     "lvsr_bigru_h0_many: bad descriptor %d", i);
+    for (int i0 = 0; i0 < n; i0 += H0_MANY_MAX) {
+        H0Pack pk;
+        const int m = n - i0 < H0_MANY_MAX ? n - i0 : H0_MANY_MAX;
+        int maxH = 0;
+        for (int i = 0; i < H0_MANY_MAX; ++i) {
+            pk.d[i] = descs[i0 + (i < m ? i : 0)];
+            if (i < m && pk.d[i].H > maxH) maxH = pk.d[i].H;
+        }
+        hipLaunchKernelGGL(enc_pbwd_h0_many_kernel, dim3((maxH + 255) / 256, m, 2), dim3(256), 0, (hipStream_t)stream, pk);
+    }
+    return lvsr_check_launch("lvsr_bigru_h0_many");
+}
diff --git a/attention-lvcsr_amd/csrc/gemm.hip b/attention-lvcsr_amd/csrc/gemm.hip
--- a/attention-lvcsr_amd/csrc/gemm.hip
+++ b/attention-lvcsr_amd/csrc/gemm.hip
@@ -600,7 +600,7 @@
     out[n] = (beta != 0.f ? beta * out[n] : 0.f) + v;
 }
 
-#define COPY_MANY_MAX 32
+#define COPY_MANY_MAX 64
 struct CopyPack { lvsr_copy_desc d[COPY_MANY_MAX]; int n; };
 __global__ __launch_bounds__(256) void lvsr_copy2d_many_kernel(CopyPack pk) {
     const lvsr_copy_desc& d = pk.d[blockIdx.y];
@@ -621,6 +621,23 @@
             for (int c = threadIdx.x; c < d.cols; c += 256) o[c] = s[c];
         }
     }
+}
+
+#define CLEAR_MANY_MAX 64
+struct ClearPack { lvsr_clear_desc d[CLEAR_MANY_MAX]; };
+__global__ __launch_bounds__(256) void lvsr_clear_many_kernel(ClearPack pk) {
+    char* p = (char*)pk.d[blockIdx.y].ptr;
+    const long long n = pk.d[blockIdx.y].bytes;
+    long long head = (long long)((16 - ((size_t)p & 15)) & 15);
+    if (head > n) head = n;
+    const long long body = (n - head) / 16, tail = head + body * 16;
+    if (blockIdx.x == 0) {
+        if ((long long)threadIdx.x < head) p[threadIdx.x] = 0;
+        if ((long long)threadIdx.x < n - tail) p[tail + threadIdx.x] = 0;
+    }
+    float4* q = (float4*)(p + head);
+    for (long long i = (long long)blockIdx.x * 256 + threadIdx.x; i < body; i += (long long)gridDim.x * 256)
+        q[i] = make_float4(0.f, 0.f, 0.f, 0.f);
 }
 
 __global__ __launch_bounds__(256) void lvsr_transpose_kernel(const float* in, int rows, int cols, float* out) {
@@ -683,7 +700,8 @@
     const int tk = big ? GK : BK;
     int tiles = ((M + tm - 1) / tm) * ((N + tn - 1) / tn);
     const int mid_max = lvsr_knob(LVSR_KNOB_GEMM_MID_TILES) > 0 ? lvsr_knob(LVSR_KNOB_GEMM_MID_TILES) : 2048;
-    const bool mid = big && batch == 1 && (tiles < 256 || (tiles < mid_max && K <= 2048));
+    const long long units = (long long)tiles * batch;
+    const bool mid = big && (units < 256 || (units < mid_max && K <= 2048));
     if (mid) { tm = 64; tn = 64; tiles = ((M + 63) / 64) * ((N + 63) / 64); }
     g.kchunk = ((K + tk - 1) / tk) * tk;
     if (g.kchunk == 0) g.kchunk = tk;
@@ -873,6 +891,25 @@
     return lvsr_check_launch("lvsr_copy2d_many");
 }
 
+int lvsr_clear_many(void* stream, const lvsr_clear_desc* descs, int n) {
+    LVSR_REQUIRE(n >= 0 && (n == 0 || descs), "lvsr_clear_many: bad arguments");
+    for (int i = 0; i < n; ++i)
+        LVSR_REQUIRE(descs[i].bytes >= 0 && (descs[i].bytes == 0 || descs[i].ptr), "lvsr_clear_many: bad descriptor %d", i);
+    for (int i0 = 0; i0 < n; i0 += CLEAR_MANY_MAX) {
+        ClearPack pk;
+        const int m = n - i0 < CLEAR_MANY_MAX ? n - i0 : CLEAR_MANY_MAX;
+        long long most = 0;
+        for (int i = 0; i < CLEAR_MANY_MAX; ++i) {
+            pk.d[i] = descs[i0 + (i < m ? i : 0)];
+            if (i < m && pk.d[i].bytes > most) most = pk.d[i].bytes;
+        }
+        long long gx = (most + 16383) / 16384;
+        gx = gx < 1 ? 1 : gx > 64 ? 64 : gx;
+        hipLaunchKernelGGL(lvsr_clear_many_kernel, dim3((unsigned)gx, m), dim3(256), 0, (hipStream_t)stream, pk);
+    }
+    return lvsr_check_launch("lvsr_clear_many");
+}
+
 int lvsr_transpose(void* stream, const float* in, int rows, int cols, float* out) {
     if (rows <= 0 || cols <= 0) return LVSR_OK;
     hipLaunchKernelGGL(lvsr_transpose_kernel, dim3((cols + 31) / 32, (rows + 31) / 32), dim3(256), 0, (hipStream_t)stream,
diff --git a/attention-lvcsr_amd/csrc/optimizer.hip b/attention-lvcsr_amd/csrc/optimizer.hip
--- a/attention-lvcsr_amd/csrc/optimizer.hip
+++ b/attention-lvcsr_amd/csrc/optimizer.hip
@@ -23,8 +23,9 @@
     if (threadIdx.x == 0) o.scratch[2 + blockIdx.x] = s;
 }
 
-__global__ __launch_bounds__(256) void opt_norm_kernel(Opt o, int nparts) {
+__global__ __launch_bounds__(256) void opt_norm_kernel(Opt o, int nparts, int clear_flags) {
     __shared__ float red[4];
+    __shared__ int skipped;
     float s = 0.f;
     for (int i = threadIdx.x; i < nparts; i += 256) s += o.scratch[2 + i];
     s = blk_sum256(s, red);
@@ -53,33 +54,55 @@
             }
         }
         o.scratch[2] = burn;
-    }
-}
-
+        skipped = skip ? 1 : 0;
+    }
+    if (clear_flags) {
+        __syncthreads();
+        if (!skipped)
+            for (int sgi = threadIdx.x; sgi < o.nseg; sgi += 256) o.segflag[sgi] = 0;
+    }
+}
+
+__device__ __forceinline__ float opt_rule_step(const Opt& o, long long i, float mult) {
+    float s = o.grad[i] * o.grad_scale * mult;
+    if (o.use_momentum) {
+        s = o.learning_rate * s;
+        s = o.momentum * o.velocity[i] + s;
+        o.velocity[i] = s;
+    }
+    if (o.use_adadelta) {
+        const float ms = o.decay_rate * o.ms_step[i] + (1.f - o.decay_rate) * s * s;
+        const float dx = sqrtf(o.ms_dx[i] + o.epsilon) / sqrtf(ms + o.epsilon) * s;
+        o.ms_step[i] = ms;
+        o.ms_dx[i] = o.decay_rate * o.ms_dx[i] + (1.f - o.decay_rate) * dx * dx;
+        s = dx;
+    }
+    return s;
+}
+
+__device__ __forceinline__ bool opt_not_finite(float s) { return s != s || s - s != 0.f; }
+__device__ void opt_raise(const Opt& o, long long i) {
+    for (int sg = 0; sg < o.nseg; ++sg) {
+        const long long* seg = o.segments + 4 * (long long)sg;
+        if (i >= seg[0] && i < seg[0] + seg[1] * seg[2]) o.segflag[sg] = 1;
+    }
+}
+
+template <bool RAISE>
 __global__ __launch_bounds__(256) void opt_rules_kernel(Opt o) {
     if (o.scratch[3] != 0.f) return;
     const float mult = o.scratch[1];
-    if (blockIdx.x == 0)
+    if (!RAISE && blockIdx.x == 0)
         for (int sgi = threadIdx.x; sgi < o.nseg; sgi += 256) o.segflag[sgi] = 0;
     for (long long i = (long long)blockIdx.x * 256 + threadIdx.x; i < o.n; i += (long long)gridDim.x * 256) {
-        float s = o.grad[i] * o.grad_scale * mult;
-        if (o.use_momentum) {
-            s = o.learning_rate * s;
-            s = o.momentum * o.velocity[i] + s;
-            o.velocity[i] = s;
-        }
-        if (o.use_adadelta) {
-            const float ms = o.decay_rate * o.ms_step[i] + (1.f - o.decay_rate) * s * s;
-            const float dx = sqrtf(o.ms_dx[i] + o.epsilon) / sqrtf(ms + o.epsilon) * s;
-            o.ms_step[i] = ms;
-            o.ms_dx[i] = o.decay_rate * o.ms_dx[i] + (1.f - o.decay_rate) * dx * dx;
-            s = dx;
-        }
+        const float s = opt_rule_step(o, i, mult);
         o.step[i] = s;
+        if (RAISE && o.remove_not_finite && opt_not_finite(s)) opt_raise(o, i);
     }
 }
 
 #define MAXNORM_GROUPS 16
+template <bool RAISE>
 __global__ __launch_bounds__(64 * MAXNORM_GROUPS) void opt_maxnorm_kernel(Opt o) {
     __shared__ float red[MAXNORM_GROUPS][64];
     const long long* seg = o.segments + 4 * (long long)blockIdx.y;
@@ -105,7 +128,9 @@
         const float k = o.max_norm / norm;
         for (long long r = g; r < rows; r += MAXNORM_GROUPS) {
             const long long x = off + r * cols + j;
-            o.step[x] = o.param[x] - k * (o.param[x] - o.step[x]);
+            const float st = o.param[x] - k * (o.param[x] - o.step[x]);
+            o.step[x] = st;
+            if (RAISE && o.remove_not_finite && opt_not_finite(st)) o.segflag[blockIdx.y] = 1;
         }
     }
 }
@@ -168,12 +193,17 @@
     int nb = (int)((o.n + 255) / 256);
     if (nb > 2048) nb = 2048;
     hipLaunchKernelGGL(opt_sqnorm_kernel, dim3(nparts), dim3(256), 0, s, o);
-    hipLaunchKernelGGL(opt_norm_kernel, dim3(1), dim3(256), 0, s, o, nparts);
-    hipLaunchKernelGGL(opt_rules_kernel, dim3(nb), dim3(256), 0, s, o);
-    if (o.max_norm > 0.f)
-        hipLaunchKernelGGL(opt_maxnorm_kernel, dim3((o.max_cols + 63) / 64, o.nseg), dim3(64 * MAXNORM_GROUPS), 0, s, o);
-    if (o.remove_not_finite)
-        hipLaunchKernelGGL(opt_finite_kernel, dim3(16, o.nseg), dim3(256), 0, s, o);
-    hipLaunchKernelGGL(opt_apply_kernel, dim3(16, o.nseg), dim3(256), 0, s, o);
+    const bool raise = !lvsr_knob(LVSR_KNOB_OPT_UNFUSED);
+    hipLaunchKernelGGL(opt_norm_kernel, dim3(1), dim3(256), 0, s, o, nparts, raise ? 1 : 0);
+    const dim3 mgrid((o.max_cols + 63) / 64, o.nseg);
+    if (raise) {
+        hipLaunchKernelGGL(opt_rules_kernel<true>, dim3(nb), dim3(256), 0, s, o);
+        if (o.max_norm > 0.f) hipLaunchKernelGGL(opt_maxnorm_kernel<true>, mgrid, dim3(64 * MAXNORM_GROUPS), 0, s, o);
+    } else {
+        hipLaunchKernelGGL(opt_rules_kernel<false>, dim3(nb), dim3(256), 0, s, o);
+        if (o.max_norm > 0.f) hipLaunchKernelGGL(opt_maxnorm_kernel<false>, mgrid, dim3(64 * MAXNORM_GROUPS), 0, s, o);
+        if (o.remove_not_finite) hipLaunchKernelGGL(opt_finite_kernel, dim3(16, o.nseg), dim3(256), 0, s, o);
+    }
+    hipLaunchKernelGGL(opt_apply_kernel, dim3(raise ? 64 : 16, o.nseg), dim3(256), 0, s, o);
     return lvsr_check_launch("lvsr_opt_step");
 }
diff --git a/attention-lvcsr_amd/csrc/readout.hip b/attention-lvcsr_amd/csrc/readout.hip
--- a/attention-lvcsr_amd/csrc/readout.hip
+++ b/attention-lvcsr_amd/csrc/readout.hip
@@ -1,10 +1,10 @@
 #include "common.h"
 #include "lvsr_hip.h"
 
-__global__ __launch_bounds__(256) void gather_rows_kernel(const float* table, int ldt, const long long* idx, int n,
-                                                          int nrows, int width, const float* bias, float* out, int ldo) {
+__device__ __forceinline__ void gather_rows_block(const float* table, int ldt, const long long* idx, int n, int nrows, int width,
+                                                  const float* bias, float* out, int ldo, int bx) {
     const int r = blockIdx.y;
-    const int c = blockIdx.x * 256 + threadIdx.x;
+    const int c = bx * 256 + threadIdx.x;
     if (r >= n || c >= width) return;
     long long v = idx[r];
     float x = 0.f;
@@ -12,14 +12,25 @@
     if (bias) x += bias[c];
     out[(size_t)r * ldo + c] = x;
 }
+__global__ __launch_bounds__(256) void gather_rows_kernel(const float* table, int ldt, const long long* idx, int n,
+                                                          int nrows, int width, const float* bias, float* out, int ldo) {
+    gather_rows_block(table, ldt, idx, n, nrows, width, bias, out, ldo, blockIdx.x);
+}
+struct GatherPart { const float* table; const float* bias; float* out; int ldt, width, ldo; };
+__global__ __launch_bounds__(256) void gather_rows_pair_kernel(GatherPart a, GatherPart b, const long long* idx, int n, int nrows) {
+    const int na = (a.width + 255) / 256;
+    const bool first = (int)blockIdx.x < na;
+    const GatherPart& g = first ? a : b;
+    gather_rows_block(g.table, g.ldt, idx, n, nrows, g.width, g.bias, g.out, g.ldo, first ? blockIdx.x : blockIdx.x - na);
+}
 
 #define SCATTER_CHUNK 2048
-__global__ __launch_bounds__(256) void scatter_add_rows_kernel(const float* src, int lds, const long long* idx, int n,
-                                                               int width, float* dst, int ldd, float beta) {
+__device__ __forceinline__ void scatter_add_rows_block(const float* src, int lds, const long long* idx, int n, int width, float* dst,
+                                                       int ldd, float beta, int bx) {
     __shared__ int hit[SCATTER_CHUNK];
     __shared__ int nhit;
     const int v = blockIdx.y;
-    const int c = blockIdx.x * 256 + threadIdx.x;
+    const int c = bx * 256 + threadIdx.x;
     float s = 0.f;
     for (int r0 = 0; r0 < n; r0 += SCATTER_CHUNK) {
         const int m = min(SCATTER_CHUNK, n - r0);
@@ -48,6 +59,17 @@
         float* d = dst + (size_t)v * ldd + c;
         *d = (beta != 0.f ? beta * *d : 0.f) + s;
     }
+}
+__global__ __launch_bounds__(256) void scatter_add_rows_kernel(const float* src, int lds, const long long* idx, int n,
+                                                               int width, float* dst, int ldd, float beta) {
+    scatter_add_rows_block(src, lds, idx, n, width, dst, ldd, beta, blockIdx.x);
+}
+struct ScatterPart { const float* src; float* dst; int lds, width, ldd; float beta; };
+__global__ __launch_bounds__(256) void scatter_add_rows_pair_kernel(ScatterPart a, ScatterPart b, const long long* idx, int n) {
+    const int na = (a.width + 255) / 256;
+    const bool first = (int)blockIdx.x < na;
+    const ScatterPart& g = first ? a : b;
+    scatter_add_rows_block(g.src, g.lds, idx, n, g.width, g.dst, g.ldd, g.beta, first ? blockIdx.x : blockIdx.x - na);
 }
 
 __global__ __launch_bounds__(256) void act_fwd_kernel(int kind, const float* x, int ldx, int n, int P, float* y, int ldy) {
@@ -440,6 +462,35 @@
     return lvsr_check_launch("lvsr_scatter_add_rows");
 }
 
+int lvsr_gather_rows_pair(void* stream, const long long* idx, int n, int nrows, const float* table_a, int ldt_a, int width_a,
+                          const float* bias_a, float* out_a, int ldo_a, const float* table_b, int ldt_b, int width_b,
+                          const float* bias_b, float* out_b, int ldo_b) {
+    if (n <= 0 || (width_a <= 0 && width_b <= 0)) return LVSR_OK;
+    LVSR_REQUIRE(width_a >= 0 && width_b >= 0 && idx && (width_a == 0 || (table_a && out_a)) && (width_b == 0 || (table_b && out_b)),
+                 "lvsr_gather_rows_pair: bad arguments");
+    LVSR_REQUIRE(n <= GRID_Y_MAX, "lvsr_gather_rows_pair: n = %d rows exceed the %d of one launch (one work-group row per output row)", n,
+                 GRID_Y_MAX);
+    const GatherPart a = {table_a, bias_a, out_a, ldt_a, width_a, ldo_a}, b = {table_b, bias_b, out_b, ldt_b, width_b, ldo_b};
+    hipLaunchKernelGGL(gather_rows_pair_kernel, dim3((width_a + 255) / 256 + (width_b + 255) / 256, n), dim3(256), 0,
+                       (hipStream_t)stream, a, b, idx, n, nrows);
+    return lvsr_check_launch("lvsr_gather_rows_pair");
+}
+
+int lvsr_scatter_add_rows_pair(void* stream, const long long* idx, int n, int nrows, const float* src_a, int lds_a, int width_a,
+                               float* dst_a, int ldd_a, float beta_a, const float* src_b, int lds_b, int width_b, float* dst_b,
+                               int ldd_b, float beta_b) {
+    if (nrows <= 0 || (width_a <= 0 && width_b <= 0)) return LVSR_OK;
+    LVSR_REQUIRE(width_a >= 0 && width_b >= 0 && (n <= 0 || idx) && (width_a == 0 || (src_a && dst_a)) &&
+                 (width_b == 0 || (src_b && dst_b)), "lvsr_scatter_add_rows_pair: bad arguments");
+    LVSR_REQUIRE(nrows <= GRID_Y_MAX,
+                 "lvsr_scatter_add_rows_pair: nrows = %d rows exceed the %d of one launch (one work-group row per destination row)", nrows,
+                 GRID_Y_MAX);
+    const ScatterPart a = {src_a, dst_a, lds_a, width_a, ldd_a, beta_a}, b = {src_b, dst_b, lds_b, width_b, ldd_b, beta_b};
+    hipLaunchKernelGGL(scatter_add_rows_pair_kernel, dim3((width_a + 255) / 256 + (width_b + 255) / 256, nrows), dim3(256), 0,
+                       (hipStream_t)stream, a, b, idx, n);
+    return lvsr_check_launch("lvsr_scatter_add_rows_pair");
+}
+
 int lvsr_act_fwd(void* stream, int kind, const float* x, int ldx, int n, int P, float* y, int ldy) {
     LVSR_REQUIRE(kind >= 0 && kind <= 3 && (kind != 1 || P % 2 == 0), "lvsr_act_fwd: bad activation %d / P=%d", kind, P);
     if (n <= 0 || P <= 0) return LVSR_OK;
diff --git a/attention-lvcsr_amd/lvsr_amd/bricks/__init__.py b/attention-lvcsr_amd/lvsr_amd/bricks/__init__.py
--- a/attention-lvcsr_amd/lvsr_amd/bricks/__init__.py
+++ b/attention-lvcsr_amd/lvsr_amd/bricks/__init__.py
@@ -78,6 +78,7 @@
         self._cats = {}
         self._pack_cache = {}
         self.overlap = False
+        self.preclear = True
         self._side = None
         self._side_pending = False
 
@@ -116,23 +117,45 @@
             self._packs = packs
         return self._packs[i]
 
+    def _fork_cat_pairs(self, i):
+        p, ws = self.store.p, self.ws
+        H, I = self.d.Hs[i], self.d.layer_input_dim(i)
+        W = ws.get("enc%d.Wcat" % i, (I, 6 * H))
+        b = ws.get("enc%d.bcat" % i, (6 * H,))
+        pairs = []
+        for di, direction in enumerate(("forward", "backward")):
+            n = self._names(i, direction)
+            o = di * 3 * H
+            pairs += [(p[n["Wi"]], W[:, o: o + H]), (p[n["Wg"]], W[:, o + H: o + 3 * H]),
+                      (p[n["bi"]], b[o: o + H]), (p[n["bg"]], b[o + H: o + 3 * H])]
+        return dict(version=self.store.version, W=W, b=b), pairs
+
     def _fork_cat(self, i):
         ent = self._cats.get(i)
         if ent is None or ent["version"] != self.store.version or self.lib.capturing:
-            p, ws = self.store.p, self.ws
-            H, I = self.d.Hs[i], self.d.layer_input_dim(i)
-            W = ws.get("enc%d.Wcat" % i, (I, 6 * H))
-            b = ws.get("enc%d.bcat" % i, (6 * H,))
-            pairs = []
-            for di, direction in enumerate(("forward", "backward")):
-                n = self._names(i, direction)
-                o = di * 3 * H
-                pairs += [(p[n["Wi"]], W[:, o: o + H]), (p[n["Wg"]], W[:, o + H: o + 3 * H]),
-                          (p[n["bi"]], b[o: o + H]), (p[n["bg"]], b[o + H: o + 3 * H])]
+            ent, pairs = self._fork_cat_pairs(i)
             self.lib.copy_many(pairs)
-            ent = dict(version=self.store.version, W=W, b=b)
             self._cats[i] = ent
         return ent["W"], ent["b"]
+
+    def _layer_inputs(self, m, T, B):
+        d, ws = self.d, self.ws
+        pairs = []
+        for i in range(d.n_layers):
+            ent = self._cats.get(i)
+            if ent is None or ent["version"] != self.store.version or self.lib.capturing:
+                self._cats[i], fresh = self._fork_cat_pairs(i)
+                pairs += fresh
+        masks, stride = [], 1
+        for i, s in enumerate(d.subsample):
+            T = (T + s - 1) // s
+            stride *= s
+            masks.append(None)
+            if m is not None and s > 1:
+                masks[i] = ws.get(self._n(i, "msub"), (T, B))
+                pairs.append((m[::stride], masks[i]))
+        self.lib.copy_many(pairs)
+        return masks
 
     @contextlib.contextmanager
     def _side_stream(self):
@@ -152,7 +175,7 @@
             torch.cuda.current_stream().wait_stream(self._side)
             self._side_pending = False
 
-    def _sync_ws(self, i, B, H):
+    def _sync_ws(self, i, B, H, bwd=False):
         if not self.use_persistent:
             return None
         nbytes = int(self.lib._lvsr_bigru_persist_ws_bytes(int(B), int(H)))
@@ -160,11 +183,22 @@
             return None
         if self.persist_auto and int(self.lib._lvsr_bigru_persist_rows(int(B), int(H))) > self.PERSIST_MAX_ROWS:
             return None
-        return self.ws.get(self._n(i, "sync"), ((nbytes + 3) // 4,), torch.int32)
+        return self.ws.get(self._n(i, "sync_bwd" if bwd else "sync"), ((nbytes + 3) // 4,), torch.int32)
+
+    def _clear_planes(self, B):
+        own, ranges = {}, []
+        for i, H in enumerate(self.d.Hs):
+            fwd = self._sync_ws(i, B, H)
+            if fwd is not None:
+                own[i] = self._sync_ws(i, B, H, bwd=True)
+                ranges += [(t.data_ptr() + 256, t.numel() * 4 - 256) for t in (fwd, own[i])]
+        if ranges:
+            self.lib.clear_many(ranges, own[min(own)])
+        return own
 
     def check_persistent(self):
         for k, t in self.ws._bufs.items():
-            if k[0].startswith("enc") and k[0].endswith(".sync") and int(t[0]) != 0:
+            if k[0].startswith("enc") and k[0].endswith((".sync", ".sync_bwd")) and int(t[0]) != 0:
                 t[:64].zero_()
                 raise RuntimeError("persistent BiGRU kernel aborted (a work-group of the cluster was not scheduled); results since "
                                    "the last check are invalid")
@@ -271,6 +305,8 @@
         m = None if mask is None else mask.contiguous()
         saved = []
         gemm_ws = ws.get("gemm_ws", (1 << 22,))
+        msubs = self._layer_inputs(m, T, B) if save_for_backward else None
+        cleared = self._clear_planes(B) if self.preclear and save_for_backward else {}
         for i, (H, s) in enumerate(zip(d.Hs, d.subsample)):
             I = d.layer_input_dim(i)
             Ts = (T + s - 1) // s
@@ -284,7 +320,7 @@
             x2, xg2 = x.view(T * B, I), xg.view(T * B, 6 * H)
             sync = self._sync_ws(i, B, H)
             pk = self._packed(i) if sync is None else None
-            Wcat, bcat = self._fork_cat(i)
+            Wcat, bcat = (self._cats[i]["W"], self._cats[i]["b"]) if msubs is not None else self._fork_cat(i)
             lib.sgemm(x2, Wcat, xg2, bias=bcat)
             h0s = [p[self._names(i, direction)["h0"]] for direction in ("forward", "backward")]
             if sync is not None:
@@ -294,13 +330,16 @@
                 Whh, Whg = [pk["Whh"][0], pk["Whh"][1]], [pk["Whg"][0], pk["Whg"][1]]
             lib.run("lvsr_bigru_fwd", "lvsr_bigru_fwd_args", y, self.use_graph and sync is None, xg=xg, mask=m, Whh_p=Whh, Whg_p=Whg, h0=h0s,
                     y=y, ysub=(ysub if s > 1 else None), u=u, r=r, c=c, rh=rh, sub=s, T=T, B=B, H=H,
-                    persistent=int(sync is not None), sync_ws=sync)
-            saved.append(dict(x=x, mask=m, T=T, y=y, u=u, r=r, c=c, rh=rh))
+                    persistent=(0 if sync is None else 5 if i in cleared else 1), sync_ws=sync)
+            saved.append(dict(x=x, mask=m, T=T, y=y, u=u, r=r, c=c, rh=rh, sync_bwd=cleared.get(i)))
             x = ysub
             if m is not None and s > 1:
-                mm = ws.get(self._n(i, "msub"), (Ts, B))
-                mm.copy_(m[::s])
-                m = mm
+                if msubs is not None:
+                    m = msubs[i]
+                else:
+                    mm = ws.get(self._n(i, "msub"), (Ts, B))
+                    mm.copy_(m[::s])
+                    m = mm
             T = Ts
         if m is None:
             m = ws.get(self.pfx + ".ones_mask", (T, B))
@@ -316,6 +355,7 @@
         assert self._saved is not None, "apply() must run first"
         gemm_ws = ws.get("gemm_ws", (1 << 22,))
         self._scatter = []
+        h0_sums = []
         dy = d_encoded.contiguous()
         B = int(dy.shape[1])
         for i in reversed(range(d.n_layers)):
@@ -327,6 +367,9 @@
             dh_ws = ws.get(self._n(i, "dh"), (12 * Bp * H,))
             nf, nb = self._names(i, "forward"), self._names(i, "backward")
             sync = self._sync_ws(i, B, H)
+            own = sv.pop("sync_bwd", None) if sync is not None else None
+            if own is not None:
+                sync = own
             pk = self._packed(i) if sync is None else None
             if sync is not None:
                 WhhT, WhgT = [p[nf["Whh"]], p[nb["Whh"]]], [p[nf["Whg"]], p[nb["Whg"]]]
@@ -335,7 +378,9 @@
             lib.run("lvsr_bigru_bwd", "lvsr_bigru_bwd_args", dxg, self.use_graph and sync is None, mask=sv["mask"], y=sv["y"],
                     u=sv["u"], r=sv["r"], c=sv["c"], WhhT_p=WhhT, WhgT_p=WhgT, h0=[p[nf["h0"]], p[nb["h0"]]], dy=dy,
                     dxg=dxg, dh_ws=dh_ws, dh0=[g[nf["h0"]], g[nb["h0"]]], sub=s, T=T, B=B, H=H,
-                    persistent=int(sync is not None), sync_ws=sync)
+                    persistent=(0 if sync is None else 7 if own is not None else 3), sync_ws=sync)
+            if sync is not None:
+                h0_sums.append((dh_ws, Bp, H, g[nf["h0"]], g[nb["h0"]]))
             x2 = sv["x"].view(T * B, I)
             dxg2 = dxg.view(T * B, 6 * H)
             y2 = sv["y"].view(T * B, 2 * H)
@@ -378,6 +423,11 @@
                 if self.overlap and group is not None:
                     group.flush(ws.get("gemm_ws.grouped.side", (1 << 26,)))
             dy = dx
+        if h0_sums:
+            arr = (lib.structs["lvsr_h0_desc"] * len(h0_sums))()
+            for e, (dh, Bp, H, out_f, out_b) in zip(arr, h0_sums):
+                e.dh, e.out_f, e.out_b, e.Bp, e.B, e.H = dh.data_ptr(), out_f.data_ptr(), out_b.data_ptr(), Bp, B, H
+            lib.call("lvsr_bigru_h0_many", lib.stream_for(h0_sums[0][0]), arr, len(h0_sums))
         self.join_side_stream()
         if group is None:
             self.finish_backward()
diff --git a/attention-lvcsr_amd/lvsr_amd/bricks/generator.py b/attention-lvcsr_amd/lvsr_amd/bricks/generator.py
--- a/attention-lvcsr_amd/lvsr_amd/bricks/generator.py
+++ b/attention-lvcsr_amd/lvsr_amd/bricks/generator.py
@@ -184,7 +184,7 @@
         f.update(self._gru_fields(pk), Ws_p=pk["Ws"])
         return f
 
-    def _feedback_forks(self, labels_flat, nrows, layers, fb_buf=None):
+    def _feedback_forks(self, labels_flat, nrows, layers, fb_buf=None, pair=False):
         d, p, lib = self.d, self.store.p, self.lib
         st = lib.stream_for(layers[0][1])
         if d.embed:
@@ -194,13 +194,17 @@
             if d.embed:
                 lib.sgemm(fb_buf, p[n["Wfi"]], xg[:, : d.D], bias=p[n["bfi"]])
                 lib.sgemm(fb_buf, p[n["Wfg"]], xg[:, d.D:], bias=p[n["bfg"]])
+            elif pair:
+                lib.call("lvsr_gather_rows_pair", st, ptr(labels_flat), nrows, d.FB,
+                         ptr(p[n["Wfi"]]), d.D, d.D, ptr(p[n["bfi"]]), ptr(xg), 3 * d.D,
+                         ptr(p[n["Wfg"]]), 2 * d.D, 2 * d.D, ptr(p[n["bfg"]]), ptr(xg[:, d.D:]), 3 * d.D)
             else:
                 lib.call("lvsr_gather_rows", st, ptr(p[n["Wfi"]]), d.D, ptr(labels_flat), nrows, d.FB, d.D,
                          ptr(p[n["bfi"]]), ptr(xg), 3 * d.D)
                 lib.call("lvsr_gather_rows", st, ptr(p[n["Wfg"]]), 2 * d.D, ptr(labels_flat), nrows, d.FB, 2 * d.D,
                          ptr(p[n["bfg"]]), ptr(xg[:, d.D:]), 3 * d.D)
 
-    def _feedback_forks_backward(self, l, n, sv, DXG, dfb, wgrad):
+    def _feedback_forks_backward(self, l, n, sv, DXG, dfb, wgrad, pair=False):
         d, p, g, lib = self.d, self.store.p, self.store.g, self.lib
         dpc, dg = DXG[:, : d.D], DXG[:, d.D:]
         nrows, st, labels_flat = int(DXG.shape[0]), lib.stream_for(DXG), sv["labels"].view(-1)
@@ -212,6 +216,10 @@
             if l == d.n_dec - 1:
                 lib.call("lvsr_scatter_add_rows", st, ptr(dfb), d.FB, ptr(labels_flat), nrows, d.V + 1, d.FB,
                          ptr(g[self.n["table"]]), d.FB, 0.0)
+        elif pair:
+            lib.call("lvsr_scatter_add_rows_pair", st, ptr(labels_flat), nrows, d.FB,
+                     ptr(dpc), 3 * d.D, d.D, ptr(g[n["Wfi"]]), d.D, 0.0,
+                     ptr(dg), 3 * d.D, 2 * d.D, ptr(g[n["Wfg"]]), 2 * d.D, 0.0)
         else:
             lib.call("lvsr_scatter_add_rows", st, ptr(dpc), 3 * d.D, ptr(labels_flat), nrows, d.FB, d.D,
                      ptr(g[n["Wfi"]]), d.D, 0.0)
@@ -313,6 +321,7 @@
         L, B = int(outputs.shape[0]), int(outputs.shape[1])
         Tp = int(attended.shape[0])
         pk = self._packed(packs=False)
+        self._merge_launches = bool(save_for_backward)
         A = attended.contiguous()
         Am = attended_mask.contiguous()
         labels = outputs.contiguous()
@@ -354,13 +363,11 @@
         d, p, n, lib, ws = self.d, self.store.p, self.n, self.lib, self.ws
         xg = ws.get("gen.xg", (L * B, 3 * d.D))
         fb = ws.get("gen.fb", (L * B, d.FB)) if d.embed else None
-        self._feedback_forks(labels.view(-1), L * B, [(n, xg)], fb)
+        merge = getattr(self, "_merge_launches", False)
+        self._feedback_forks(labels.view(-1), L * B, [(n, xg)], fb, pair=merge)
         bufs = self._attdec_bufs("gen.", "", L, B, Tp, ZB=True, xg=xg, ymask=ym)
         S, W = bufs["S"], bufs["W"]
-        S[0].copy_(p[n["h0"]].unsqueeze(0).expand(B, d.D))
-        W[0].zero_()
-        if d.conv:
-            W[0, :, 0] = 1.0
+        self._initial_slots(S, W, B, Tp, merge)
         fields = self._attdec_fields(pk, A, PA, Am, L, B, bufs, phases=3, step0=0, broadcast=False)
         sync = self._persistent_ws(fields)
         if sync is not None:
@@ -375,6 +382,23 @@
             self._ensure_packs(pk)
             fwd_args = lib.run("lvsr_attdec_fwd", "lvsr_attdec_args", S, self.use_graph, **fields)
         return dict(bufs=bufs, saved=dict(xg=xg, fb=fb, fields=fields, AW_valid=sync is not None))
+
+    def _initial_slots(self, S, W, B, Tp, merge):
+        d, p, n, lib, ws = self.d, self.store.p, self.n, self.lib, self.ws
+        row = ws.get("gen.W0_row", (Tp,)) if merge else None
+        if row is None or getattr(self, "_w0_row_ptr", None) != row.data_ptr():
+            if row is None or lib.capturing:
+                S[0].copy_(p[n["h0"]].unsqueeze(0).expand(B, d.D))
+                W[0].zero_()
+                if d.conv:
+                    W[0, :, 0] = 1.0
+                return
+            base = ws._bufs[("gen.W0_row", torch.float32)]
+            base.zero_()
+            if d.conv:
+                base[0] = 1.0
+            self._w0_row_ptr = row.data_ptr()
+        lib.copy_many([(p[n["h0"]].unsqueeze(0).expand(B, d.D), S[0]), (row.unsqueeze(0).expand(B, Tp), W[0])])
 
     def _lm_lookahead(self, lm, labels, ym, L, B):
         dev = labels.device
@@ -477,8 +501,9 @@
         DWA = dWA_r.view(L, B, d.E)
         DSW = ws.get("gen.DSW", (nrows, d.M))
         DCV = ws.get("gen.DCV", (L, B, Kc, Tp)) if d.conv else None
-        dPA = ws.get("gen.dPA", (Tp, B, d.M), zero=True)
-        ds = ws.get("gen.ds", (B, d.D), zero=True)
+        dPA = ws.get("gen.dPA", (Tp, B, d.M))
+        ds = ws.get("gen.ds", (B, d.D))
+        lib.clear_many([(dPA.data_ptr(), dPA.numel() * 4), (ds.data_ptr(), ds.numel() * 4)], ds)
         wd = ws.get("gen.Wd_cat", (d.E, 3 * d.D))
         AW, AW_ld = self._AW(Tp, B)
         if not sv.get("AW_valid"):
@@ -516,7 +541,7 @@
         colsum(ds, g[n["h0"]])
         colsum(dpc, g[n["bfi"]])
         colsum(dg, g[n["bfg"]])
-        self._feedback_forks_backward(0, n, sv, DXG, ws.get("gen.dfb", (nrows, d.FB)) if d.embed else None, wgrad)
+        self._feedback_forks_backward(0, n, sv, DXG, ws.get("gen.dfb", (nrows, d.FB)) if d.embed else None, wgrad, pair=True)
         return dict(accH=accH, accWe=accWe, accEb=accEb, DCV=DCV, dPA=dPA, DWA=DWA, fwd_args=fwd_args)
 
     def init_generation(self, attended, attended_mask):
diff --git a/attention-lvcsr_amd/lvsr_amd/native.py b/attention-lvcsr_amd/lvsr_amd/native.py
--- a/attention-lvcsr_amd/lvsr_amd/native.py
+++ b/attention-lvcsr_amd/lvsr_amd/native.py
@@ -230,6 +230,14 @@
             d.ldd = dst.stride(0) if dst.dim() == 2 else cols
         self.call("lvsr_copy2d_many", self.stream_for(pairs[0][1]), arr, len(pairs))
 
+    def clear_many(self, ranges, ref):
+        if not ranges:
+            return
+        arr = (self.structs["lvsr_clear_desc"] * len(ranges))()
+        for d, (address, nbytes) in zip(arr, ranges):
+            d.ptr, d.bytes = int(address), int(nbytes)
+        self.call("lvsr_clear_many", self.stream_for(ref), arr, len(ranges))
+
     def transpose(self, x, out):
         self.call("lvsr_transpose", self.stream_for(out), ptr(x), x.shape[0], x.shape[1], ptr(out))
 
diff --git a/attention-lvcsr_amd/lvsr_amd/training.py b/attention-lvcsr_amd/lvsr_amd/training.py
--- a/attention-lvcsr_amd/lvsr_amd/training.py
+++ b/attention-lvcsr_amd/lvsr_amd/training.py
@@ -16,7 +16,7 @@
 
 
 def _is_sync_word(key):
-    return key[0] in ("gen.sync", "gen.sync_bwd") or (key[0].startswith("enc") and key[0].endswith(".sync"))
+    return key[0] in ("gen.sync", "gen.sync_bwd") or (key[0].startswith("enc") and key[0].endswith((".sync", ".sync_bwd")))
 
 
 class Trainer(object):
diff --git a/include/lvsr_hip.h b/include/lvsr_hip.h
--- a/include/lvsr_hip.h
+++ b/include/lvsr_hip.h
@@ -21,7 +21,8 @@
 #define LVSR_KNOB_GEMM_MID_TILES 6
 #define LVSR_KNOB_DEC_CLUSTER 7
 #define LVSR_KNOB_ENERGY_ROWS 8
-#define LVSR_KNOB_COUNT 9
+#define LVSR_KNOB_OPT_UNFUSED 9
+#define LVSR_KNOB_COUNT 10
 int lvsr_set_knob(int knob, int value);
 int lvsr_get_knob(int knob);
 
@@ -44,6 +45,11 @@
     float beta;
 } lvsr_copy_desc;
 int lvsr_copy2d_many(void* stream, const lvsr_copy_desc* descs, int n);
+typedef struct lvsr_clear_desc {
+    void* ptr;
+    long long bytes;
+} lvsr_clear_desc;
+int lvsr_clear_many(void* stream, const lvsr_clear_desc* descs, int n);
 int lvsr_colsum(void* stream, const float* X, int M, int N, int ldx, float* out, float beta, float* ws,
                 long long ws_bytes);
 typedef struct lvsr_colsum_desc {
@@ -94,6 +100,11 @@
     void* sync_ws;
 } lvsr_bigru_bwd_args;
 int lvsr_bigru_bwd(void* stream, const lvsr_bigru_bwd_args* a, int use_graph);
+typedef struct lvsr_h0_desc {
+    const float* dh; float* out_f; float* out_b;
+    int Bp, B, H, pad0;
+} lvsr_h0_desc;
+int lvsr_bigru_h0_many(void* stream, const lvsr_h0_desc* descs, int n);
 int lvsr_bigru_persist_rows(int B, int H);
 long long lvsr_bigru_persist_ws_bytes(int B, int H);
 
@@ -205,6 +216,12 @@
                      const float* bias, float* out, int ldo);
 int lvsr_scatter_add_rows(void* stream, const float* src, int lds, const long long* idx, int n, int nrows, int width,
                           float* dst, int ldd, float beta);
+int lvsr_gather_rows_pair(void* stream, const long long* idx, int n, int nrows, const float* table_a, int ldt_a, int width_a,
+                          const float* bias_a, float* out_a, int ldo_a, const float* table_b, int ldt_b, int width_b,
+                          const float* bias_b, float* out_b, int ldo_b);
+int lvsr_scatter_add_rows_pair(void* stream, const long long* idx, int n, int nrows, const float* src_a, int lds_a, int width_a,
+                               float* dst_a, int ldd_a, float beta_a, const float* src_b, int lds_b, int width_b, float* dst_b,
+                               int ldd_b, float beta_b);
 int lvsr_act_fwd(void* stream, int kind, const float* x, int ldx, int n, int P, float* y, int ldy);
 int lvsr_act_bwd(void* stream, int kind, const float* x, int ldx, const float* dy, int lddy, int n, int P, float* dx,
                  int lddx);
```

Measured after the change: 1.061 million frames/s, median of 6. 1.3% higher.
